# facebook/facebook360_dep

Hardware: AMD Instinct MI355X
Metric: depth Mpix/s per GPU (full pyramid, 16-cam 2048^2 rig); % HBM-read roofline (higher is better)
Workload: dtype f32+f64; 1 GPU; BASELINE config 3: 16-camera 2048x2048 synthetic rig, 8-frame sequence, full 10-level pyramid per frame, per-level temporal filter (+-2 frames); the same sequence for every --gpus N (block partition, 8 frame(s) on this rank); rig=cfg2, cameras=16, frames=8, temporal_filter=True, halo_transport=local, parallelism=frames x1

## Files before the change

### facebook360_dep_amd/csrc/derp_capi.hip

```cpp
#include <hip/hip_runtime.h>

#include <algorithm>
#include <cfloat>
#include <cmath>
#include <cstdarg>
#include <cstdio>
#include <cstdlib>
#include <cstring>
#include <map>
#include <memory>
#include <string>
#include <vector>

#include <rocprim/device/device_radix_sort.hpp>

#include "../../include/derp_hip.h"
#include "derp_host.h"
#include "derp_kernels.h"
#include "derp_mesh.h"
#include "derp_points.h"
#include "derp_render.h"

using namespace derp;

// ... 3 lines not shown

struct Span {
  derp_ctx* c;
  int stage, level;
  hipEvent_t a = nullptr, b = nullptr;
  Span(derp_ctx* ctx, int st, int lv) : c(ctx), stage(st), level(lv) {
    if (c->profiling) {
      (void)hipEventCreate(&a);
      (void)hipEventCreate(&b);
      (void)hipEventRecord(a, c->stream);
    }
  }
  ~Span() {
    if (c->profiling && a) {
      (void)hipEventRecord(b, c->stream);
      c->spans.push_back({stage, level, a, b});
    }
  }
};

void drain_spans(derp_ctx* c) {
  for (auto& s : c->spans) {
    (void)hipEventSynchronize(s.b);
    float ms = 0;
    (void)hipEventElapsedTime(&ms, s.a, s.b);
    if (s.level >= 0 && s.level < kMaxLevels) {
      c->accMs[s.stage][s.level] += ms;
      c->accLaunch[s.stage][s.level] += 1;
    }
    (void)hipEventDestroy(s.a);
    (void)hipEventDestroy(s.b);
  }
  c->spans.clear();
}

size_t npx(const derp_ctx* c, int level) {
  return (size_t)c->LW[level] * c->LH[level];
}

unsigned long long* counter_slot(derp_ctx* c, int stage, int level) {
  return c->counters.as<unsigned long long>() + ((size_t)stage * kMaxLevels + level) * 4;
}

LevelView make_view(derp_ctx* c, int stage, int dst0, int nd) {
  LevelView V;
  const int L = c->cur;
  V.W = c->LW[L];
  V.H = c->LH[L];
  V.Wd = (double)V.W;
  V.Hd = (double)V.H;
  V.S = c->S;
  V.D = nd;
  V.level = L;
  V.numLevels = c->numLevels;
  V.dst0 = dst0;
  V.hasFg = c->opt.use_foreground_masks;
  const float scale = float(V.W) / c->heightFull;
  const float scaleVar = scale * scale;
  V.varNoiseFloor = std::max(c->opt.var_noise_floor * scaleVar, kMinVar);
  V.varHighThresh = c->opt.var_high_thresh;
  V.minDepthM = c->opt.min_depth_m;
  V.maxDepthM = c->opt.max_depth_m;
  V.randomProposals = c->opt.random_proposals;
  V.partialCoverage = c->opt.partial_coverage;
  V.xcdRotate = c->xcdRotate;
  V.camsSrc = c->camsSrc.as<Cam>();
  V.camsDst = c->camsDst.as<Cam>();
  V.dst2src = c->dst2src.as<int>();
  V.srcColor = c->frame().color[L].as<ushort4>();
  V.ownBias = c->w.ownBias.as<ushort4>();
  V.srcVar = c->w.srcVar.as<float>();
  V.srcFg = c->frame().fg[L].as<uint8_t>();
  V.rayDir = c->rayDir.as<double>();
  V.behind = c->behind.as<unsigned>();
  V.rayStride = (size_t)c->D * V.W * V.H;
  V.projWarp = c->projWarp.as<float2>();
  V.projColor = c->w.projColor.as<ushort4>();
  V.projBias = c->w.projBias.as<ushort4>();
  V.projColorT = c->w.projColorT.as<ushort4>();
  V.disparity = c->w.disparity.as<float>();
  V.cost = c->w.cost.as<float>();
  V.confidence = c->w.confidence.as<float>();
  V.bgDisp = c->frame().bg[L].as<float>();
  V.fovMask = c->w.fovMask.as<uint8_t>();
  V.pairCount = c->w.pairCount.as<uint8_t>();
  V.counters = counter_slot(c, stage, L);
#if DERP_BLOCK_TRACE
  V.blockTrace = nullptr;
#endif
  return V;
}
int block_trace_attach(derp_ctx* c, LevelView& V, int which, int gridX, int gridY) {
#if DERP_BLOCK_TRACE
  DevBuf& buf = c->blockTrace[which][V.level];
  const size_t bytes = (size_t)gridX * gridY * 2 * sizeof(unsigned long long);
  ALLOC(c, buf, bytes);
  HIPCHK(c, hipMemsetAsync(buf.as<unsigned long long>(), 0, bytes, c->stream));
  V.blockTrace = buf.as<unsigned long long>();
  c->blockTraceGrid[which][V.level][0] = gridX;
  c->blockTraceGrid[which][V.level][1] = gridY;
#else
  (void)c, (void)V, (void)which, (void)gridX, (void)gridY;
#endif
  return 0;
}

const dim3 kBlurBlk(64, 4, 1);
dim3 blur_grid(int ow, int oh, int planes) {
  return dim3((ow + 63) / 64, (oh + 4 * kBlurRows - 1) / (4 * kBlurRows), planes);
}

void lanczos_coeffs(float x, float* coeffs) {
  static const double s45 = 0.70710678118654752440084436210485;
  static const double cs[][2] = {{1, 0}, {-s45, -s45}, {0, 1}, {s45, -s45}, {-1, 0}, {s45, s45}, {0, -1}, {-s45, s45}};
  if (x < 1.1920928955078125e-07f) {
    for (int i = 0; i < 8; i++) {
      coeffs[i] = 0;
    }
    coeffs[3] = 1;
    return;
  }
  float sum = 0;
  const double y0 = -(x + 3) * M_PI * 0.25, s0 = std::sin(y0), c0 = std::cos(y0);
  for (int i = 0; i < 8; i++) {
    const double y = -(x + 3 - i) * M_PI * 0.25;
    coeffs[i] = (float)((cs[i][0] * s0 + cs[i][1] * c0) / (y * y));
    sum += coeffs[i];
  }
  sum = 1.f / sum;
  for (int i = 0; i < 8; i++) {
    coeffs[i] *= sum;
  }
}

int get_lanczos(derp_ctx* c, int ssize, int dsize, LanczosTab** out) {
  auto key = std::make_pair(ssize, dsize);
  auto it = c->lanczos.find(key);
  if (it != c->lanczos.end()) {
    *out = &it->second;
    return 0;
  }
  std::vector<int> ofs(dsize);
  std::vector<float> coef((size_t)dsize * 8);
  const double scale = (double)ssize / dsize;
  for (int d = 0; d < dsize; ++d) {
    float f = (float)((d + 0.5) * scale - 0.5);
    int s = (int)f;
    s -= (s > f);
    f -= s;
    ofs[d] = s;
    lanczos_coeffs(f, &coef[(size_t)d * 8]);
  }
  LanczosTab t;
  ALLOC(c, t.ofs, ofs.size() * sizeof(int));
  ALLOC(c, t.coef, coef.size() * sizeof(float));
  HIPCHK(c, hipMemcpyAsync(t.ofs.p, ofs.data(), ofs.size() * sizeof(int), hipMemcpyHostToDevice, c->stream));
  HIPCHK(c, hipMemcpyAsync(t.coef.p, coef.data(), coef.size() * sizeof(float), hipMemcpyHostToDevice, c->stream));
  HIPCHK(c, hipStreamSynchronize(c->stream));
  *out = &(c->lanczos[key] = std::move(t));
  return 0;
}

int get_area_tab(derp_ctx* c, int ssize, int dsize, AreaTabDev** out, bool forceTable = false) {
  auto key = std::make_pair(forceTable ? -ssize : ssize, dsize);
  auto it = c->areaTabs.find(key);
  if (it != c->areaTabs.end()) {
    *out = &it->second;
// ... 93 lines not shown
      locs.push_back(make_int2(x, y));
    }
    if (x == y || ((x < 0) && (x == -y)) || ((x > 0) && (x == 1 - y))) {
      t = dx;
      dx = -dy;
      dy = t;
    }
    x += dx;
    y += dy;
  }
  return locs;
}

int ensure_spiral(derp_ctx* c, int radius) {
  if (c->spiralRadius == radius) {
    return 0;
  }
  const std::vector<int2> s = make_spiral(radius * 2 + 1);
  ALLOC(c, c->spiral, s.size() * sizeof(int2));
  HIPCHK(c, hipMemcpy(c->spiral.p, s.data(), s.size() * sizeof(int2), hipMemcpyHostToDevice));
  c->spiralN = (int)s.size();
  c->spiralRadius = radius;
  return 0;
}

int upsample_lanczos_dev(derp_ctx* c, const float* in, int sw, int sh, float* out, int dw, int dh, int planes,
                         size_t inStride, size_t outStride) {
  if (sw == dw && sh == dh) {
    return fail(c, "upsample to identical size not supported");
  }
  LanczosTab *tx, *ty;
  TRY(get_lanczos(c, sw, dw, &tx));
  TRY(get_lanczos(c, sh, dh, &ty));
  const size_t tmpStride = (size_t)dw * sh;
  ALLOC(c, c->w.lanczosTmp, tmpStride * planes * sizeof(float));
  hipLaunchKernelGGL(k_lanczos_h, grid2d(dw, sh, planes, kBlk2d), kBlk2d, 0, c->stream, in, sw, sh, dw,
                     tx->ofs.as<int>(), tx->coef.as<float>(), c->w.lanczosTmp.as<float>(), inStride, tmpStride);
  KCHECK(c);
  hipLaunchKernelGGL(k_lanczos_v, grid2d(dw, dh, planes, kBlk2d), kBlk2d, 0, c->stream, c->w.lanczosTmp.as<float>(), sh,
                     dw, dh, ty->ofs.as<int>(), ty->coef.as<float>(), out, tmpStride, outStride);
  KCHECK(c);
  return 0;
}

int upsample_masked_dev(derp_ctx* c, const float* in, const uint8_t* mask, int sw, int sh, const uint8_t* maskUp,
                        const float* bgUp, float* out, int dw, int dh, int planes = 1) {
  const float scale = float(dw) / float(sw);
  const int radius = (int)(scale * scale + 1);
  TRY(ensure_spiral(c, radius));
  ALLOC(c, c->w.lanczosTmp, (size_t)dw * dh * planes * sizeof(float));
  hipLaunchKernelGGL(k_upsample_nearest_masked, grid2d(dw, dh, planes, kBlk2d), kBlk2d, 0, c->stream, in, mask, sw, sh,
                     maskUp, dw, dh, c->w.lanczosTmp.as<float>());
  KCHECK(c);
  hipLaunchKernelGGL(k_spiral_fill, grid2d(dw, dh, planes, kBlk2d), kBlk2d, 0, c->stream, c->w.lanczosTmp.as<float>(), bgUp,
                     maskUp, dw, dh, c->spiral.as<int2>(), c->spiralN, out);
  KCHECK(c);
  return 0;
}

bool batch_needs_inverse_warps(const derp_ctx* c, int dst0, int nd) {
  std::vector<char> covered(c->S, 0);
  for (int d = dst0; d < dst0 + nd; ++d) {
    covered[c->dst2srcH[d]] = 1;
  }
  for (int s = 0; s < c->S; ++s) {
    if (!covered[s]) {
      return true;
    }
  }
  return false;
}

size_t table_bytes_per_dst(const derp_ctx* c, int W, int H, bool withInverse) {
  const size_t wp = (size_t)(W + 2 * kPadW) * (H + 2 * kPadW), cp = (size_t)(W + 2 * kPadC) * (H + 2 * kPadC);
  return (size_t)(c->S - 1) * (wp * sizeof(float2) + 2 * cp * sizeof(ushort4) + (withInverse ? (size_t)W * H * sizeof(float2) : 0) +
                               (DERP_RANDOM_TILED ? tiled_plane(W, H) * sizeof(ushort4) : 0));
}

int compute_fov_and_masks(derp_ctx* c, int level) {
  const int W = c->LW[level], H = c->LH[level];
  const size_t n = (size_t)W * H;
  {
    Span sp(c, ST_FOV, level);
    hipLaunchKernelGGL(k_fov_mask, grid2d(W, H, c->D, kBlk2d), kBlk2d, 0, c->stream, c->camsDst.as<Cam>(), W, H,
                       c->w.fovMask.as<uint8_t>());
    KCHECK(c);
    hipLaunchKernelGGL(k_and_masks, dim3(flat_grid(n), c->D), dim3(256), 0, c->stream, c->w.fovMask.as<uint8_t>(),
                       c->frame().fg[level].as<uint8_t>(), c->dst2src.as<int>(), 0, n, c->w.maskAnd.as<uint8_t>());
    KCHECK(c);
  }
  return 0;
}

int build_warp(derp_ctx* c, int dst0, int nd) {
  const int L = c->cur;
  Span sp(c, ST_PROJ_WARP, L);
  {
    const size_t n = (size_t)c->LW[L] * c->LH[L];
    ALLOC(c, c->rayDir, 3 * n * c->D * sizeof(double));
    ALLOC(c, c->behind, n * c->D * sizeof(unsigned));
  }
  LevelView V = make_view(c, ST_PROJ_WARP, dst0, nd);
  hipLaunchKernelGGL(k_proj_warp, grid2d(V.W + 2 * kPadW, V.H + 2 * kPadW, c->S, kBlk2d), kBlk2d, 0, c->stream, V,
                     c->projWarp.as<float2>());
  KCHECK(c);
  hipLaunchKernelGGL(k_pixel_rays, grid2d(V.W, V.H, nd, kBlk2d), kBlk2d, 0, c->stream, V, c->rayDir.as<double>(),
                     c->behind.as<unsigned>());
  KCHECK(c);
  c->w.colorTablesCleanLevel = -1;
  if (batch_needs_inverse_warps(c, dst0, nd)) {
    hipLaunchKernelGGL(k_proj_warp_inv, grid2d(V.W, V.H, nd, kBlk2d), kBlk2d, 0, c->stream, V, c->projWarpInv.as<float2>());
    KCHECK(c);
  }
  return 0;
}

int build_color_tables(derp_ctx* c, int dst0, int nd) {
  const int L = c->cur;
  LevelView V = make_view(c, ST_REPROJECT, dst0, nd);
  Span sp(c, ST_REPROJECT, L);
  const dim3 grid((V.W + kRbTile - 1) / kRbTile, (V.H + kRbTile - 1) / kRbTile, nd * (c->S - 1));
  ALLOC(c, c->w.tileSeen, (size_t)grid.x * grid.y * grid.z);
  const int skipBlank = c->w.colorTablesCleanLevel == L && nd == c->D && !c->noBlankSkip;
  hipLaunchKernelGGL(k_reproject_bias, grid, dim3(256), 0, c->stream, V, c->projWarpInv.as<float2>(),
                     c->w.projColor.as<ushort4>(), c->w.projBias.as<ushort4>(), c->w.projColorT.as<ushort4>(),
                     c->w.tileSeen.as<uint8_t>(), skipBlank);
  KCHECK(c);
  c->w.colorTablesCleanLevel = nd == c->D ? L : -1;
  return 0;
}

int tiles_of(int W, int H, int& tilesX) {
  constexpr int B = kTileBlock;
  tilesX = ((W + 15) / 16 + B - 1) / B * B;
  const int tilesY = ((H + 15) / 16 + B - 1) / B * B;
  return tilesX * tilesY * (256 / kCostBlock);
}
constexpr size_t kCostLdsPerSrc = (size_t)kCostBlock * sizeof(SsdPair);
struct CostGrid {
  int blocks, bands, perBlock;
};
constexpr int kCostMaxBands = 4, kCostMaxTilesPerBlock = 4;
int cost_grid_blocks(int tiles, int bands, int perBlock) {
  const int items = (tiles + perBlock - 1) / perBlock, unit = 8 * bands;
  return (items + unit - 1) / unit * unit;
}
CostGrid cost_grid(const derp_ctx* c, int tiles, int tilesX, bool spread) {
  const auto pow2_floor = [](int v, int cap) {
    int p = 1;
    while (p * 2 <= std::min(v, cap)) {
      p *= 2;
    }
    return p;
  };
  CostGrid g;
  g.perBlock = c->costTilesPerBlock > 0 ? pow2_floor(c->costTilesPerBlock, kCostMaxTilesPerBlock) : 1;
  const int rowOfSquares = tilesX * (256 / kCostBlock) * kTileBlock;
  g.bands = c->xcdBands > 0 ? pow2_floor(c->xcdBands, kCostMaxBands)
                            : spread ? pow2_floor(std::max(1, tiles / (8 * rowOfSquares)), kCostMaxBands) : 1;
  g.blocks = cost_grid_blocks(tiles, g.bands, g.perBlock);
  return g;
}
size_t lds_for_waves(size_t needed, int waves, size_t ldsPerCu, size_t fixed) {
  if (waves <= 0 || waves >= 4) {
    return needed;
  }
  const size_t perBlock = ldsPerCu / (size_t)(4 * waves + 1) + 256;
  return std::max(needed, perBlock > fixed ? perBlock - fixed : needed);
}
constexpr size_t kCostLdsStatic = sizeof(PatchWin) * (kCostBlock / 64) + kAtanLutDoubles * sizeof(double);
bool cost_four_waves(const derp_ctx* c) {
  if (const char* e = getenv("DERP_COST_WAVES")) {
    return atoi(e) >= 4;
  }
  return 16 * (kCostLdsPerSrc * (size_t)c->S + kCostLdsStatic) <= c->ldsPerCu && c->S <= 16;
}

int run_brute_force(derp_ctx* c, int dst0, int nd) {
  const int L = c->cur;
  if (L != c->numLevels - 1) {
    return 0;
  }
  Span sp(c, ST_BRUTE, L);
  LevelView V = make_view(c, ST_BRUTE, dst0, nd);
  const size_t n = (size_t)V.W * V.H;
  ALLOC(c, c->w.bruteCost, (size_t)nd * kNumDepths * n * sizeof(float));
  ALLOC(c, c->w.bruteConf, (size_t)nd * kNumDepths * n * sizeof(float));
  const int tilesX = std::max(1, (V.W - 2 + 7) / 8), tilesY = std::max(1, (V.H - 2 + 7) / 8);
  const int tiles = tilesX * tilesY;
  const size_t lds = kCostLdsPerSrc * (size_t)(c->S);
  hipLaunchKernelGGL(k_brute_costs, dim3(tiles, kNumDepths, nd), dim3(kCostBlock), lds, c->stream, V,
                     c->w.bruteCost.as<float>(), c->w.bruteConf.as<float>(), tilesX, tiles);
  KCHECK(c);
  hipLaunchKernelGGL(k_brute_select, grid2d(V.W, V.H, nd, kBlk2d), kBlk2d, 0, c->stream, V, c->w.bruteCost.as<float>(),
                     c->w.bruteConf.as<float>());
  KCHECK(c);
  hipLaunchKernelGGL(k_brute_margin, grid2d(V.W, V.H, nd, kBlk2d), kBlk2d, 0, c->stream, V);
  KCHECK(c);
  return 0;
}

int run_random_proposals(derp_ctx* c, int dst0, int nd) {
  const int L = c->cur;
  if (c->opt.random_proposals <= 0 || L == c->numLevels - 1) {
    return 0;
  }
  Span sp(c, ST_RANDOM, L);
  c->randomRanThisLevel = true;
  LevelView V = make_view(c, ST_RANDOM, dst0, nd);
  if (V.H > 2 && V.W > 2) {
    hipLaunchKernelGGL(k_row_rank, dim3(V.H - 2, nd), dim3(256), 0, c->stream, V, c->w.rank.as<int>());
    KCHECK(c);
  }
  int tilesX;
  const int tiles = tiles_of(V.W, V.H, tilesX);
  const size_t lds = lds_for_waves(kCostLdsPerSrc * (size_t)(c->S), c->randomWaves, c->ldsPerCu, kCostLdsStatic);
  const CostGrid cg = cost_grid(c, tiles, tilesX, true);
  TRY(block_trace_attach(c, V, 0, cg.blocks, nd));
  const bool four = cost_four_waves(c);
  const auto kernel = cg.perBlock > 1 ? (four ? k_random_proposals_walk : k_random_proposals_walk_w3)
                                      : (four ? k_random_proposals : k_random_proposals_w3);
  hipLaunchKernelGGL(kernel, dim3(cg.blocks, nd), dim3(kCostBlock), lds, c->stream, V, c->w.rank.as<int>(), tilesX, cg.bands, cg.perBlock);
  KCHECK(c);
  return 0;
}

int run_ping_pong(derp_ctx* c, int dst0, int nd) {
  const int L = c->cur;
  if (L == c->numLevels - 1) {
    return 0;
  }
  Span sp(c, ST_PINGPONG, L);
  LevelView V = make_view(c, ST_PINGPONG, dst0, nd);
  const size_t n = (size_t)V.W * V.H;
  HIPCHK(c, hipMemsetAsync(c->w.changed.as<uint8_t>() + (size_t)dst0 * n, 1, n * nd, c->stream));
  int tilesX;
  const int tiles = tiles_of(V.W, V.H, tilesX);
  const size_t lds = lds_for_waves(kCostLdsPerSrc * (size_t)(c->S), c->ppWaves, c->ldsPerCu, kCostLdsStatic);
  const bool four = cost_four_waves(c);
  const CostGrid cg = cost_grid(c, tiles, tilesX, false);
  const auto kernel = cg.perBlock > 1
                          ? (c->ppCompact ? (four ? k_ping_pong_walk : k_ping_pong_walk_w3) : (four ? k_ping_pong_loop_walk : k_ping_pong_loop_walk_w3))
                          : (c->ppCompact ? (four ? k_ping_pong : k_ping_pong_w3) : (four ? k_ping_pong_loop : k_ping_pong_loop_w3));
  TRY(block_trace_attach(c, V, 1, cg.blocks, nd));
  for (int it = 1; it <= c->opt.ping_pong_iterations; ++it) {
    hipLaunchKernelGGL(kernel, dim3(cg.blocks, nd), dim3(kCostBlock), lds,
                       c->stream, V, c->w.changed.as<uint8_t>(), c->w.dispRes.as<float>(), c->w.costRes.as<float>(), tilesX,
                       (int)(it == 1 && c->randomRanThisLevel && !c->noMemo), cg.bands, cg.perBlock);
    KCHECK(c);
    hipLaunchKernelGGL(k_ping_pong_commit, dim3(flat_grid(n * nd)), dim3(256), 0, c->stream,
                       c->w.disparity.as<float>() + (size_t)dst0 * n, c->w.cost.as<float>() + (size_t)dst0 * n,
                       c->w.dispRes.as<float>() + (size_t)dst0 * n, c->w.costRes.as<float>() + (size_t)dst0 * n,
                       c->w.changed.as<uint8_t>() + (size_t)dst0 * n, n * nd);
    KCHECK(c);
  }
  if (dst0 + nd >= c->D) {
    c->randomRanThisLevel = false;
  }
  return 0;
}

int run_mismatches(derp_ctx* c) {
  const int L = c->cur;
  if (L > c->opt.mismatches_start_level || L == c->numLevels - 1) {
    return 0;
  }
  if (c->D != c->S) {
    return fail(c, "Check failed: rigDst.size() == rigSrc.size()  Mismatches only valid when considering all cameras");
  }
  for (int d = 0; d < c->D; ++d) {
    if (c->dst2srcH[d] != d) {
      return fail(c, "mismatch handling needs destinations in rig order (dst %d maps to src %d)", d, c->dst2srcH[d]);
    }
  }
  Span sp(c, ST_MISMATCH, L);
  c->randomRanThisLevel = false;
  LevelView V = make_view(c, ST_MISMATCH, 0, c->D);
  const size_t n = (size_t)V.W * V.H;
  hipLaunchKernelGGL(k_mismatch, dim3((V.W + 15) / 16, (V.H + 15) / 16, c->D), dim3(256), 256 * sizeof(float) * c->S,
                     c->stream, V, c->w.dispRes.as<float>(), c->w.mismatchMask.as<uint8_t>());
  KCHECK(c);
  HIPCHK(c, hipMemcpyAsync(c->w.disparity.p, c->w.dispRes.p, n * c->D * sizeof(float), hipMemcpyDeviceToDevice, c->stream));
  return 0;
}

int bilateral_radius(int level) {
  const float scale = std::pow(0.9f, level);
  return (int)std::max(std::ceil(5 * scale), float(1));
}

size_t bilateral_lds_bytes(int radius) {
  const size_t side = 16 + 2 * (size_t)radius;
  const size_t t = ((side + 15) & ~(size_t)15) * side;
  return t * 4 * sizeof(float) + ((t + 3) & ~(size_t)3);
}

constexpr size_t kBilateralMaxLds = 64 * 1024 - 256;

int run_bilateral(derp_ctx* c) {
  const int L = c->cur;
  Span sp(c, ST_BILATERAL, L);
  c->randomRanThisLevel = false;
  const int W = c->LW[L], H = c->LH[L];
  const size_t n = (size_t)W * H;
  const int radius = bilateral_radius(L);
  hipLaunchKernelGGL(k_joint_bilateral<true>, dim3((W + 15) / 16, (H + 15) / 16, c->D), dim3(256),
                     bilateral_lds_bytes(radius), c->stream, c->w.disparity.as<float>(),
                     (const void*)c->frame().color[L].as<ushort4>(), c->w.maskAnd.as<uint8_t>(), W, H, radius, 0.005f, 0.5f,
                     1.0f, 1.0f, c->w.tmpF.as<float>(), n, n, c->dst2src.as<int>());
  KCHECK(c);
  HIPCHK(c, hipMemcpyAsync(c->w.disparity.p, c->w.tmpF.p, n * c->D * sizeof(float), hipMemcpyDeviceToDevice, c->stream));
  return 0;
}

int run_median(derp_ctx* c, bool fuseMaskFov) {
  const int L = c->cur;
  Span sp(c, ST_MEDIAN, L);
  c->randomRanThisLevel = false;
  const int W = c->LW[L], H = c->LH[L];
  const size_t n = (size_t)W * H;
  hipLaunchKernelGGL(k_masked_median, grid2d(W, H, c->D, kBlk2d), kBlk2d, 0, c->stream, c->w.disparity.as<float>(),
                     c->opt.use_foreground_masks ? c->frame().bg[L].as<float>() : (const float*)nullptr,
                     c->w.maskAnd.as<uint8_t>(), W, H, 1, c->w.tmpF.as<float>(), n,
                     fuseMaskFov ? c->w.fovMask.as<uint8_t>() : (const uint8_t*)nullptr);
  KCHECK(c);
  HIPCHK(c, hipMemcpyAsync(c->w.disparity.p, c->w.tmpF.p, n * c->D * sizeof(float), hipMemcpyDeviceToDevice, c->stream));
  return 0;
}

int run_mask_fov(derp_ctx* c) {
  const int L = c->cur;
  Span sp(c, ST_MASKFOV, L);
  const size_t n = npx(c, L) * c->D;
  hipLaunchKernelGGL(k_mask_fov, dim3(flat_grid(n)), dim3(256), 0, c->stream, c->w.disparity.as<float>(),
                     c->w.fovMask.as<uint8_t>(), n);
  KCHECK(c);
  return 0;
}

int check_level(derp_ctx* c, int level) {
  if (!c || c->numLevels == 0) {
    return fail(c, "derp_set_pyramid has not been called");
  }
  if (level < 0 || level >= c->numLevels) {
    return fail(c, "level %d out of range [0, %d)", level, c->numLevels);
  }
  if (c->LW[level] <= 0 || c->LH[level] <= 0) {
    return fail(c, "level %d was declared absent in derp_set_pyramid", level);
  }
  return 0;
}

int level_begin(derp_ctx* c, int level, bool buildAllTables) {
  TRY(check_level(c, level));
  if (c->S - 1 > kMaxSrc) {
    return fail(c, "too many source cameras (%d > %d)", c->S, kMaxSrc + 1);
  }
  c->cur = level;
  const int W = c->LW[level], H = c->LH[level];
  const size_t n = (size_t)W * H;
  if (W < 3 || H < 3) {
    return fail(c, "level %d is too small (%dx%d)", level, W, H);
  }
  TRY(compute_fov_and_masks(c, level));
  {
    Span sp(c, ST_VARIANCE, level);
    hipLaunchKernelGGL(k_variance, grid2d(W, H, c->S, kBlk2d), kBlk2d, 0, c->stream, c->frame().color[level].as<ushort4>(),
                       W, H, c->w.srcVar.as<float>());
    KCHECK(c);
  }
  {
    Span sp(c, ST_OWN_BIAS, level);
    hipLaunchKernelGGL(k_blur3_u16, blur_grid(W, H, c->S), kBlurBlk, 0, c->stream,
                       c->frame().color[level].as<ushort4>(), 0, c->w.ownBias.as<ushort4>(), 0, W, H, n, n);
    KCHECK(c);
  }
  HIPCHK(c, hipMemsetAsync(c->w.cost.p, 0, n * c->D * sizeof(float), c->stream));
  HIPCHK(c, hipMemsetAsync(c->w.confidence.p, 0, n * c->D * sizeof(float), c->stream));
  HIPCHK(c, hipMemsetAsync(c->w.mismatchMask.p, 0, n * c->D, c->stream));
  if (level < c->numLevels - 1 && !c->frame().haveDisp[level + 1] && !buildAllTables) {
    return fail(c, "Missing disparity of level %d needed to start level %d", level + 1, level);
  }
  if (level < c->numLevels - 1 && c->frame().haveDisp[level + 1]) {
    Span sp(c, ST_UPSAMPLE, level);
    const int sw = c->LW[level + 1], sh = c->LH[level + 1];
    if (!c->opt.use_foreground_masks) {
      TRY(upsample_lanczos_dev(c, c->frame().disp[level + 1].as<float>(), sw, sh, c->w.disparity.as<float>(), W, H, c->D,
                               (size_t)sw * sh, n));
    } else {
      ALLOC(c, c->w.staging, (size_t)sw * sh * c->D);
      hipLaunchKernelGGL(k_fov_mask, grid2d(sw, sh, c->D, kBlk2d), kBlk2d, 0, c->stream, c->camsDst.as<Cam>(), sw, sh,
                         c->w.staging.as<uint8_t>());
      KCHECK(c);
      hipLaunchKernelGGL(k_and_masks, dim3(flat_grid((size_t)sw * sh), c->D), dim3(256), 0, c->stream,
                         c->w.staging.as<uint8_t>(), c->frame().fg[level + 1].as<uint8_t>(), c->dst2src.as<int>(), 0,
                         (size_t)sw * sh, c->w.staging.as<uint8_t>());
      KCHECK(c);
      TRY(upsample_masked_dev(c, c->frame().disp[level + 1].as<float>(), c->w.staging.as<uint8_t>(), sw, sh,
                              c->w.maskAnd.as<uint8_t>(), c->frame().bg[level].as<float>(), c->w.disparity.as<float>(), W, H, c->D));
    }
  } else {
    HIPCHK(c, hipMemsetAsync(c->w.disparity.p, 0, n * c->D * sizeof(float), c->stream));
  }
  const bool invAll = batch_needs_inverse_warps(c, 0, c->D);
  size_t per = table_bytes_per_dst(c, W, H, invAll);
  int DB = c->D;
  bool needInv = invAll;
  {
    const size_t wpAll = (size_t)(W + 2 * kPadW) * (H + 2 * kPadW) * (c->S - 1) * c->D * sizeof(float2);
    const size_t cpAll = (size_t)(W + 2 * kPadC) * (H + 2 * kPadC) * (c->S - 1) * c->D * sizeof(ushort4);
    const size_t ipAll = (size_t)W * H * (c->S - 1) * c->D * sizeof(float2);
    const bool resident = c->projWarp.bytes >= wpAll && c->w.projColor.bytes >= cpAll && c->w.projBias.bytes >= cpAll &&
        (!invAll || c->projWarpInv.bytes >= ipAll) && !getenv("DERP_TABLE_BUDGET_GB") &&
        (!DERP_RANDOM_TILED || c->w.projColorT.bytes >= tiled_plane(W, H) * (c->S - 1) * c->D * sizeof(ushort4));
    if (!resident) {
      size_t freeB = 0, totalB = 0;
      HIPCHK(c, hipMemGetInfo(&freeB, &totalB));
      size_t budget = freeB + c->projWarp.bytes + c->w.projColor.bytes + c->w.projBias.bytes + c->projWarpInv.bytes + c->w.projColorT.bytes;
      if (const char* e = getenv("DERP_TABLE_BUDGET_GB")) {
        budget = std::min<size_t>(budget, (size_t)(atof(e) * (1ull << 30)));
      } else {
        budget = (size_t)(budget * 0.85);
      }
      DB = (int)std::min<size_t>((size_t)c->D, budget / std::max<size_t>(per, 1));
      if (DB < c->D && !needInv) {
        needInv = true;
        per = table_bytes_per_dst(c, W, H, true);
        DB = (int)std::min<size_t>((size_t)c->D, budget / std::max<size_t>(per, 1));
      }
      if (DB < 1) {
        return fail(c, "projection tables for one destination (%zu bytes) exceed the table budget (%zu bytes)", per, budget);
      }
      const int batches = (c->D + DB - 1) / DB;
      DB = (c->D + batches - 1) / batches;
    }
  }
  c->DB = DB;
  const size_t wp = (size_t)(W + 2 * kPadW) * (H + 2 * kPadW), cp = (size_t)(W + 2 * kPadC) * (H + 2 * kPadC);
  ALLOC(c, c->projWarp, (size_t)DB * (c->S - 1) * wp * sizeof(float2));
  ALLOC(c, c->w.projColor, (size_t)DB * (c->S - 1) * cp * sizeof(ushort4));
  ALLOC(c, c->w.projBias, (size_t)DB * (c->S - 1) * cp * sizeof(ushort4));
  if (needInv) {
    ALLOC(c, c->projWarpInv, (size_t)DB * (c->S - 1) * n * sizeof(float2));
  }
  if (DERP_RANDOM_TILED) {
    ALLOC(c, c->w.projColorT, (size_t)DB * (c->S - 1) * tiled_plane(W, H) * sizeof(ushort4));
  }
  c->tablesValid = false;
  c->randomRanThisLevel = false;
  if (buildAllTables) {
    if (DB < c->D) {
      return fail(c, "stage-level API needs all destinations' tables resident (batch %d < %d)", DB, c->D);
    }
    if (c->opt.rebuild_warp_tables || c->warpCachedLevel != level) {
      TRY(build_warp(c, 0, c->D));
      c->warpCachedLevel = level;
    }
  }
  return 0;
}

int level_end(derp_ctx* c) {
  const int L = c->cur;
  HIPCHK(c, hipMemcpyAsync(c->frame().disp[L].p, c->w.disparity.p, npx(c, L) * c->D * sizeof(float),
                           hipMemcpyDeviceToDevice, c->stream));
  c->frame().haveDisp[L] = 1;
  return 0;
}

int process_level(derp_ctx* c, int level) {
  TRY(level_begin(c, level, false));
  for (int d0 = 0; d0 < c->D; d0 += c->DB) {
    const int nd = std::min(c->DB, c->D - d0);
    const bool single = (c->DB == c->D);
    if (!single || c->opt.rebuild_warp_tables || c->warpCachedLevel != level) {
      TRY(build_warp(c, d0, nd));
      c->warpCachedLevel = single ? level : -1;
    }
    TRY(build_color_tables(c, d0, nd));
    TRY(run_brute_force(c, d0, nd));
    TRY(run_random_proposals(c, d0, nd));
    TRY(run_ping_pong(c, d0, nd));
  }
  TRY(run_mismatches(c));
  if (c->opt.do_bilateral_filter) {
    TRY(run_bilateral(c));
  }
  if (c->opt.do_median_filter) {
    TRY(run_median(c, true));
  } else {
    TRY(run_mask_fov(c));
  }
  TRY(level_end(c));
  return 0;
}

int need_current(derp_ctx* c, bool tables) {
  if (!c || c->cur < 0) {
    return fail(c, "derp_level_begin has not been called");
  }
  if (tables && !c->tablesValid) {
    return fail(c, "derp_stage_reproject_colors must run before this stage");
  }
  return 0;
}

template <typename T>
int upload_tmp(derp_ctx* c, DevBuf& buf, const T* host, size_t count) {
  ALLOC(c, buf, count * sizeof(T));
  HIPCHK(c, hipMemcpyAsync(buf.p, host, count * sizeof(T), hipMemcpyHostToDevice, c->stream));
  return 0;
}

int alloc_pyramid(derp_ctx* c, FramePyramid& f) {
  const int num_levels = c->numLevels;
  f.color.resize(num_levels);
  f.fg.resize(num_levels);
  f.bg.resize(num_levels);
  f.disp.resize(num_levels);
  f.haveBg.assign(num_levels, 0);
  f.haveDisp.assign(num_levels, 0);
  for (int l = 0; l < num_levels; ++l) {
    const size_t n = npx(c, l);
    if (n == 0) {
      continue;
    }
    ALLOC(c, f.color[l], n * c->S * sizeof(ushort4));
    ALLOC(c, f.fg[l], n * c->S);
    ALLOC(c, f.bg[l], n * c->D * sizeof(float));
    ALLOC(c, f.disp[l], n * c->D * sizeof(float));
    HIPCHK(c, hipMemsetAsync(f.fg[l].p, 1, n * c->S, c->stream));
    HIPCHK(c, hipMemsetAsync(f.bg[l].p, 0, n * c->D * sizeof(float), c->stream));
  }
  return 0;
}

int alloc_work_set(derp_ctx* c, WorkSet& w, size_t n) {
  ALLOC(c, w.srcVar, n * c->S * sizeof(float));
  ALLOC(c, w.ownBias, n * c->S * sizeof(ushort4));
  ALLOC(c, w.fovMask, n * c->D);
  ALLOC(c, w.maskAnd, n * c->D);
  for (DevBuf* b : {&w.disparity, &w.cost, &w.confidence, &w.dispRes, &w.costRes, &w.tmpF, &w.rank}) {
    ALLOC(c, *b, n * c->D * sizeof(float));
  }
  ALLOC(c, w.changed, n * c->D);
  ALLOC(c, w.mismatchMask, n * c->D);
  ALLOC(c, w.pairCount, n * c->D);
  return 0;
}

int select_frame(derp_ctx* c, int slot) {
  if (slot < 0 || slot >= (int)c->frames.size()) {
    return fail(c, "frame slot %d out of range [0, %d)", slot, (int)c->frames.size());
  }
  if (slot != c->curSlot) {
    c->curSlot = slot;
    c->cur = -1;
  }
  return 0;
}

void lane_swap(derp_ctx* c, int i) {
  std::swap(c->stream, c->lanes[i]->stream);
  std::swap(c->w, c->lanes[i]->w);
}

int lanes_prepare(derp_ctx* c, int count, size_t n) {
  while ((int)c->lanes.size() < count) {
    c->lanes.emplace_back(new WorkLane);
    WorkLane& l = *c->lanes.back();
    if (hipStreamCreateWithFlags(&l.stream, hipStreamNonBlocking) != hipSuccess ||
        hipEventCreateWithFlags(&l.done, hipEventDisableTiming) != hipSuccess) {
      return fail(c, "work lane: hipStreamCreate / hipEventCreate failed");
    }
  }
  if (!c->laneReady) {
    HIPCHK(c, hipEventCreateWithFlags(&c->laneReady, hipEventDisableTiming));
  }
  for (int i = 0; i < count; ++i) {
    TRY(alloc_work_set(c, c->lanes[i]->w, n));
  }
  return 0;
}

int process_level_on_lane(derp_ctx* c, int i, int slot, int level) {
  if (i < 0) {
    TRY(select_frame(c, slot));
    return process_level(c, level);
  }
  HIPCHK(c, hipStreamWaitEvent(c->lanes[i]->stream, c->laneReady, 0));
  lane_swap(c, i);
  c->activeLane = i;
  int rc = select_frame(c, slot);
  if (!rc) {
    rc = process_level(c, level);
  }
  if (!rc && hipEventRecord(c->lanes[i]->done, c->stream) != hipSuccess) {
    rc = fail(c, "work lane: hipEventRecord failed");
  }
  lane_swap(c, i);
  c->activeLane = -1;
  c->cur = -1;
  return rc;
}

int temporal_launch(derp_ctx* c, const void* const* guides, const float* const* images, const uint8_t* const* masks, int n,
                    int centre, int W, int H, int planes, float sigma, int radius, float w0, float w1, float w2,
                    float* out, const int* dst2src) {
  if (n < 1 || centre < 0 || centre >= n) {
    return fail(c, "temporal window must hold at least the centre frame");
  }
  if (n > kMaxTemporalFrames) {
    ALLOC(c, c->temporalCarry, (size_t)planes * W * H * sizeof(float2));
  }
  for (int t0 = 0; t0 < n; t0 += kMaxTemporalFrames) {
    TemporalFrames F;
    F.n = std::min(kMaxTemporalFrames, n - t0);
    for (int t = 0; t < F.n; ++t) {
      F.guides[t] = reinterpret_cast<const ushort4*>(guides[t0 + t]);
      F.images[t] = images[t0 + t];
      F.masks[t] = masks[t0 + t];
    }
    F.refGuide = reinterpret_cast<const ushort4*>(guides[centre]);
    F.refImage = images[centre];
    F.refMask = masks[centre];
    F.carry = n > kMaxTemporalFrames ? c->temporalCarry.as<float2>() : nullptr;
    F.first = t0 == 0;
    F.last = t0 + F.n >= n;
    const size_t lds = 2 * ((((size_t)(32 + 2 * radius) * (8 + 2 * radius) * 9) + 15) & ~(size_t)15);
    if (radius >= 0 && lds <= 48 * 1024 && !c->noTemporalTile) {
      hipLaunchKernelGGL(k_temporal_tiled, grid2d(W, H, planes, kBlk2d), kBlk2d, lds, c->stream, F, W, H, sigma, radius, w0,
                         w1, w2, out, dst2src);
    } else {
      hipLaunchKernelGGL(k_temporal, grid2d(W, H, planes, kBlk2d), kBlk2d, 0, c->stream, F, W, H, sigma, radius, w0, w1, w2,
                         out, dst2src);
    }
    KCHECK(c);
  }
  return 0;
}

}

extern "C" {

void derp_options_default(derp_options* o) {
  o->min_depth_m = 0.5f;
  o->max_depth_m = 1e4f;
  o->var_noise_floor = 4e-5f;
  o->var_high_thresh = 1e-3f;
  o->random_proposals = 2;
  o->ping_pong_iterations = 1;
  o->mismatches_start_level = -1;
  o->do_bilateral_filter = 1;
  o->do_median_filter = 1;
  o->use_foreground_masks = 0;
  o->partial_coverage = 0;
  o->rebuild_warp_tables = 1;
}

int derp_create(derp_ctx** out, int device, const derp_camera_desc* src, int n_src, const derp_camera_desc* dst,
                int n_dst) {
  if (!out) {
    return 1;
  }
  *out = nullptr;
  std::unique_ptr<derp_ctx> owner(new derp_ctx);
  derp_ctx* c = owner.get();
  derp_options_default(&c->opt);
  if (n_src <= 0 || n_dst <= 0) {
    return create_fail("no source / destination cameras!");
  }
  hipDeviceProp_t prop;
  TRY(open_device(device, "the depth path", &prop));
  c->device = device;
  if (prop.maxSharedMemoryPerMultiProcessor > 0) {
    c->ldsPerCu = prop.maxSharedMemoryPerMultiProcessor;
  }
  if (const char* e = getenv("DERP_XCD_ROTATE")) {
    c->xcdRotate = atoi(e);
  }
  if (const char* e = getenv("DERP_XCD_BANDS")) {
    c->xcdBands = atoi(e);
  }
  if (const char* e = getenv("DERP_COST_TILES_PER_BLOCK")) {
    c->costTilesPerBlock = atoi(e);
  }
  c->noMemo = getenv("DERP_NO_MEMO") != nullptr;
  if (const char* e = getenv("DERP_PP_COMPACT")) {
    c->ppCompact = atoi(e) != 0;
  }
  if (const char* e = getenv("DERP_RANDOM_WAVES")) {
    c->randomWaves = atoi(e);
  }
  if (const char* e = getenv("DERP_PP_WAVES")) {
    c->ppWaves = atoi(e);
  }
  c->noTemporalTile = getenv("DERP_NO_TEMPORAL_TILE") != nullptr;
  c->noBlankSkip = getenv("DERP_NO_BLANK_SKIP") != nullptr;
  c->S = n_src;
  c->D = n_dst;
  c->frames.resize(1);
  c->camsSrcH.resize(n_src);
  c->camsDstH.resize(n_dst);
  for (int i = 0; i < n_src; ++i) {
    if (const char* m = host_prepare_camera(src[i], c->camsSrcH[i])) {
      return create_fail(std::string("camera ") + src[i].id + ": " + m);
    }
  }
  c->dst2srcH.assign(n_dst, 0);
  c->descDstH.assign(dst, dst + n_dst);
  for (int i = 0; i < n_dst; ++i) {
    if (const char* m = host_prepare_camera(dst[i], c->camsDstH[i])) {
      return create_fail(std::string("camera ") + dst[i].id + ": " + m);
    }
    bool found = false;
    for (int s = 0; s < n_src; ++s) {
      if (strncmp(dst[i].id, src[s].id, sizeof dst[i].id) == 0) {
        c->dst2srcH[i] = s;
        found = true;
        break;
      }
    }
    if (!found) {
      return create_fail(std::string("destination camera ") + dst[i].id + " is not a source camera");
    }
    if (memcmp(&c->camsDstH[i], &c->camsSrcH[c->dst2srcH[i]], sizeof(Cam)) != 0) {
      return create_fail(std::string("destination camera ") + dst[i].id + " differs from the source camera of the same id "
                  "(destinations must be cameras of the source rig, as filterDestinations makes them)");
    }
  }
  if (c->camsSrc.ensure(sizeof(Cam) * n_src) || c->camsDst.ensure(sizeof(Cam) * n_dst) ||
      c->dst2src.ensure(sizeof(int) * n_dst) || c->counters.ensure(sizeof(unsigned long long) * ST_COUNT * kMaxLevels * 4)) {
    return create_fail("out of device memory");
  }
  if (hipStreamCreateWithFlags(&c->stream, hipStreamNonBlocking) != hipSuccess) {
    return create_fail("hipStreamCreate failed");
  }
  if (hipStreamCreateWithFlags(&c->copyStream, hipStreamNonBlocking) != hipSuccess) {
    (void)hipStreamDestroy(c->stream);
    return create_fail("hipStreamCreate failed");
  }
  (void)hipMemcpy(c->camsSrc.p, c->camsSrcH.data(), sizeof(Cam) * n_src, hipMemcpyHostToDevice);
  (void)hipMemcpy(c->camsDst.p, c->camsDstH.data(), sizeof(Cam) * n_dst, hipMemcpyHostToDevice);
  (void)hipMemcpy(c->dst2src.p, c->dst2srcH.data(), sizeof(int) * n_dst, hipMemcpyHostToDevice);
  (void)hipMemset(c->counters.p, 0, c->counters.bytes);
  *out = owner.release();
  return 0;
}

void derp_destroy(derp_ctx* c) {
  if (!c) {
    return;
  }
  (void)hipSetDevice(c->device);
  (void)hipStreamSynchronize(c->stream);
  for (auto& l : c->lanes) {
    (void)hipStreamSynchronize(l->stream);
  }
  drain_spans(c);
  for (auto& l : c->lanes) {
    (void)hipStreamDestroy(l->stream);
    (void)hipEventDestroy(l->done);
  }
  if (c->laneReady) {
    (void)hipEventDestroy(c->laneReady);
  }
  (void)hipStreamDestroy(c->stream);
  (void)hipStreamDestroy(c->copyStream);
  delete c;
}

const char* derp_last_error(const derp_ctx* c) {
  return c ? c->err.c_str() : g_create_error.c_str();
}

int derp_set_options(derp_ctx* c, const derp_options* o) {
  if (!c || !o) {
    return 1;
  }
  if (o->random_proposals < 0) {
    return fail(c, "Check failed: random_proposals >= 0");
  }
  c->opt = *o;
  return 0;
}

int derp_set_pyramid(derp_ctx* c, int num_levels, const int* widths, const int* heights, int width_full,
                     int height_full) {
  if (!c) {
    return 1;
  }
  if (num_levels <= 0 || num_levels > kMaxLevels) {
    return fail(c, "num_levels %d out of range (1..%d)", num_levels, kMaxLevels);
  }
  HIPCHK(c, hipSetDevice(c->device));
  c->numLevels = num_levels;
  c->widthFull = width_full;
  c->heightFull = height_full;
  c->LW.assign(widths, widths + num_levels);
  c->LH.assign(heights, heights + num_levels);
  c->frames.clear();
  c->frames.resize(1);
  c->curSlot = 0;
  TRY(alloc_pyramid(c, c->frame()));
  size_t nmax = 0;
  for (int l = 0; l < num_levels; ++l) {
    nmax = std::max(nmax, npx(c, l));
  }
  TRY(alloc_work_set(c, c->w, nmax));
  c->cur = -1;
  c->warpCachedLevel = -1;
  HIPCHK(c, hipStreamSynchronize(c->stream));
  return 0;
}

int derp_set_frame_slots(derp_ctx* c, int n_slots) {
  if (!c || c->numLevels == 0) {
    return fail(c, "derp_set_pyramid has not been called");
  }
  if (n_slots < 1 || n_slots > 4096) {
    return fail(c, "n_slots %d out of range (1..4096)", n_slots);
  }
  HIPCHK(c, hipSetDevice(c->device));
  TRY(select_frame(c, 0));
  const int had = (int)c->frames.size();
  c->frames.resize(n_slots);
  for (int k = had; k < n_slots; ++k) {
    TRY(alloc_pyramid(c, c->frames[k]));
  }
  HIPCHK(c, hipStreamSynchronize(c->stream));
  return 0;
}

int derp_select_frame(derp_ctx* c, int slot) {
  if (!c || c->numLevels == 0) {
    return fail(c, "derp_set_pyramid has not been called");
  }
  return select_frame(c, slot);
}

int derp_frame_slots(const derp_ctx* c, int* n_slots, int* selected) {
  if (!c) {
    return 1;
  }
  if (n_slots) {
    *n_slots = (int)c->frames.size();
  }
  if (selected) {
    *selected = c->curSlot;
  }
  return 0;
}

int derp_bind_thread(derp_ctx* c) {
  return use_device(c);
}
void* derp_host_alloc(size_t bytes) {
  void* p = nullptr;
  if (bytes == 0 || hipHostMalloc(&p, bytes, hipHostMallocDefault) != hipSuccess) {
    (void)hipGetLastError();
    return nullptr;
  }
  return p;
}
void derp_host_free(void* p) {
  if (p) {
    (void)hipHostFree(p);
  }
}
int derp_host_register(void* p, size_t bytes) {
  if (!p || bytes == 0 || hipHostRegister(p, bytes, hipHostRegisterDefault) != hipSuccess) {
    (void)hipGetLastError();
    return 1;
  }
  return 0;
}
void derp_host_unregister(void* p) {
  if (p && hipHostUnregister(p) != hipSuccess) {
    (void)hipGetLastError();
  }
}

int derp_upload_color(derp_ctx* c, int level, int s, const uint16_t* bgr) {
  TRY(check_level(c, level));
  if (s < 0 || s >= c->S || !bgr) {
    return fail(c, "bad source index / null image");
  }
  HIPCHK(c, hipSetDevice(c->device));
  const size_t n = npx(c, level);
  TRY(upload_tmp(c, c->w.staging, bgr, n * 3));
  hipLaunchKernelGGL(k_bgr_to_bgrx, dim3(flat_grid(n)), dim3(256), 0, c->stream, c->w.staging.as<uint16_t>(),
                     c->frame().color[level].as<ushort4>() + (size_t)s * n, n);
  KCHECK(c);
  HIPCHK(c, hipStreamSynchronize(c->stream));
// ... 170 lines not shown
  int tilesX;
  const int tiles = tiles_of(V.W, V.H, tilesX);
  const size_t lds = kCostLdsPerSrc * (size_t)(c->S);
  hipLaunchKernelGGL(k_cost_map, dim3(tiles), dim3(kCostBlock), lds, c->stream, V, d, c->w.staging.as<float>(),
                     c->w.stagingB.as<float>(), c->w.stagingB.as<float>() + n, tilesX);
  KCHECK(c);
  HIPCHK(c, hipStreamSynchronize(c->stream));
  HIPCHK(c, hipMemcpy(cost, c->w.stagingB.p, n * sizeof(float), hipMemcpyDeviceToHost));
  HIPCHK(c, hipMemcpy(confidence, c->w.stagingB.as<float>() + n, n * sizeof(float), hipMemcpyDeviceToHost));
  return 0;
}

static int build_pyramid(derp_ctx* c, int kind, int index, int count, const void* host, size_t elem, int w, int h,
                         int threshold) {
  if (!c || c->numLevels == 0) {
    return fail(c, "derp_set_pyramid has not been called");
  }
  if (index < 0 || index >= count || !host || w <= 0 || h <= 0) {
    return fail(c, "bad camera index / null image");
  }
  HIPCHK(c, hipSetDevice(c->device));
  const size_t n = (size_t)w * h;
  ALLOC(c, c->fullFrame, n * elem);
  HIPCHK(c, hipMemcpyAsync(c->fullFrame.p, host, n * elem, hipMemcpyHostToDevice, c->stream));
  for (int l = 0; l < c->numLevels; ++l) {
    const size_t nl = npx(c, l);
    if (nl == 0) {
      continue;
    }
    void* dst = kind == 0 ? (void*)(c->frame().color[l].as<ushort4>() + (size_t)index * nl)
        : kind == 1       ? (void*)(c->frame().fg[l].as<uint8_t>() + (size_t)index * nl)
                          : (void*)(c->frame().bg[l].as<float>() + (size_t)index * nl);
    TRY(resize_area_dev(c, kind, c->fullFrame.p, w, h, dst, c->LW[l], c->LH[l], threshold));
    if (kind == 2) {
      c->frame().haveBg[l] = 1;
    }
  }
  HIPCHK(c, hipStreamSynchronize(c->stream));
  return 0;
}
int derp_build_pyramid_color(derp_ctx* c, int src, const uint16_t* bgr, int w, int h) {
  return build_pyramid(c, 0, src, c ? c->S : 0, bgr, 6, w, h, -1);
}
int derp_build_pyramid_foreground_mask(derp_ctx* c, int src, const uint8_t* mask, int w, int h, int threshold) {
  return build_pyramid(c, 1, src, c ? c->S : 0, mask, 1, w, h, threshold);
}
int derp_build_pyramid_background_disparity(derp_ctx* c, int dst, const float* disp, int w, int h) {
  return build_pyramid(c, 2, dst, c ? c->D : 0, disp, 4, w, h, -1);
}
int derp_download_level_color(derp_ctx* c, int level, int src, uint16_t* bgr) {
  TRY(check_level(c, level));
  if (src < 0 || src >= c->S || !bgr) {
    return fail(c, "bad source index / null output");
  }
  const size_t n = npx(c, level);
  ALLOC(c, c->w.staging, n * 6);
  hipLaunchKernelGGL(k_bgrx_to_bgr, dim3(flat_grid(n)), dim3(256), 0, c->stream,
                     c->frame().color[level].as<ushort4>() + (size_t)src * n, c->w.staging.as<uint16_t>(), n);
  KCHECK(c);
  return download_sync(c, bgr, c->w.staging.p, n * 6);
}
int derp_download_level_mask(derp_ctx* c, int level, int src, uint8_t* mask) {
  TRY(check_level(c, level));
  if (src < 0 || src >= c->S || !mask) {
    return fail(c, "bad source index / null output");
  }
  const size_t n = npx(c, level);
  return download_sync(c, mask, c->frame().fg[level].as<uint8_t>() + (size_t)src * n, n);
}
int derp_download_level_background(derp_ctx* c, int level, int dst, float* disp) {
  TRY(check_level(c, level));
  if (dst < 0 || dst >= c->D || !disp) {
    return fail(c, "bad destination index / null output");
  }
  const size_t n = npx(c, level);
  return download_sync(c, disp, c->frame().bg[level].as<float>() + (size_t)dst * n, n * 4);
}
int derp_download_mismatch_mask(derp_ctx* c, int d, uint8_t* out) {
  TRY(need_current(c, false));
  if (d < 0 || d >= c->D || !out) {
    return fail(c, "bad destination index / null output");
  }
  const size_t n = npx(c, c->cur);
  return download_sync(c, out, c->w.mismatchMask.as<uint8_t>() + (size_t)d * n, n);
}

}

#include "derp_render_api.h"
#include "derp_rephoto_api.h"
#include "derp_points_api.h"
#include "derp_mesh_api.h"
#include "derp_filters_api.h"
#include "derp_debug_api.h"
#include "derp_sequence.h"
#include "derp_isp.h"
#include "derp_sim.h"

derp_ctx::derp_ctx() = default;
derp_ctx::~derp_ctx() = default;
```

### facebook360_dep_amd/csrc/derp_ctx.h

```cpp
#pragma once

namespace {

enum Stage {
  ST_FOV = 0,
  ST_VARIANCE,
  ST_OWN_BIAS,
  ST_UPSAMPLE,
  ST_PROJ_WARP,
  ST_REPROJECT,
  ST_PROJ_BIAS,
  ST_BRUTE,
  ST_RANDOM,
  ST_PINGPONG,
  ST_MISMATCH,
  ST_BILATERAL,
  ST_MEDIAN,
  ST_MASKFOV,
  ST_TEMPORAL,
  ST_LANES,
  ST_COUNT
};
const char* kStageNames[ST_COUNT] = {"fov_mask",  "variance",    "own_bias",         "upsample",  "proj_warp",
                                     "reproject", "proj_bias",   "brute_force",      "random_proposals",
                                     "ping_pong", "mismatches",  "bilateral",        "median",    "mask_fov",
                                     "temporal",  "lanes_wall"};
constexpr int kMaxLevels = 24;

struct TimedSpan {
  int stage, level;
  hipEvent_t a, b;
};

struct LanczosTab {
  DevBuf ofs, coef;
};

struct AreaTabDev {
  DevBuf start, si, alpha;
  int iscale = 0;
};

struct WorkSet {
  DevBuf srcVar, ownBias, fovMask, maskAnd, disparity, cost, confidence, dispRes, costRes, changed, tmpF, rank, mismatchMask, pairCount;
  DevBuf tileSeen;
  DevBuf projColor, projBias;
  DevBuf projColorT;
  DevBuf bruteCost, bruteConf, lanczosTmp, staging, stagingB;
  int colorTablesCleanLevel = -1;
};

struct FramePyramid {
  std::vector<DevBuf> color, fg, bg, disp;
  std::vector<char> haveBg, haveDisp;
};

struct WorkLane {
  hipStream_t stream = nullptr;
  hipEvent_t done = nullptr;
  WorkSet w;
};

struct SmrState; struct RephotoState; struct PointsState; struct MeshState;

}

struct derp_ctx {
  derp_ctx();
  ~derp_ctx();
  int device = 0;
  hipStream_t stream = nullptr;
  hipStream_t copyStream = nullptr;
  DevBuf copyStaging;
  std::string err;
  std::string* errSink() {
    return &err;
  }
  derp_options opt;
  int S = 0, D = 0;
  std::vector<Cam> camsSrcH, camsDstH;
  std::vector<int> dst2srcH;
  std::vector<derp_camera_desc> descDstH;
  DevBuf camsSrc, camsDst, dst2src;

  int numLevels = 0, widthFull = 0, heightFull = 0;
  std::vector<int> LW, LH;
  std::vector<FramePyramid> frames;
  int curSlot = 0;
  FramePyramid& frame() {
    return frames[curSlot];
  }
  DevBuf fullFrame;
  DevBuf devMask;

  int cur = -1;
  int DB = 0;
  WorkSet w;
  DevBuf temporalCarry;
  DevBuf projWarp, projWarpInv;
  DevBuf rayDir, behind;
  int warpCachedLevel = -1;
  bool randomRanThisLevel = false;
  bool tablesValid = false;
  std::map<std::pair<int, int>, LanczosTab> lanczos;
  std::map<std::pair<int, int>, AreaTabDev> areaTabs;
  DevBuf spiral;
  int spiralN = 0, spiralRadius = -1;
  std::vector<std::unique_ptr<WorkLane>> lanes;
  hipEvent_t laneReady = nullptr;
  int activeLane = -1;

  DevBuf counters;
  bool profiling = false;
  std::vector<TimedSpan> spans;
  double accMs[ST_COUNT][kMaxLevels] = {};
  int accLaunch[ST_COUNT][kMaxLevels] = {};
  int xcdRotate = 1;
  int xcdBands = 0, costTilesPerBlock = 0;
  DevBuf blockTrace[2][kMaxLevels];
  int blockTraceGrid[2][kMaxLevels][2] = {};
  bool noMemo = false;
  bool ppCompact = true;
  int randomWaves = 0, ppWaves = 0;
  size_t ldsPerCu = 160 * 1024;
  bool noTemporalTile = false;
  bool noBlankSkip = false;
  std::unique_ptr<SmrState> smr;
  std::unique_ptr<RephotoState> rephoto;
  std::unique_ptr<PointsState> points;
  std::unique_ptr<MeshState> mesh;
};

namespace {

int fail(derp_ctx* c, const char* fmt, ...) {
  va_list ap;
  va_start(ap, fmt);
  vfail(c ? &c->err : nullptr, fmt, ap);
  va_end(ap);
  return 1;
}

int use_device(derp_ctx* c) {
  if (!c) {
    return 1;
  }
  HIPCHK(c, hipSetDevice(c->device));
  return 0;
}

int check_camera(derp_ctx* c, int cam) {
  if (cam < 0 || cam >= c->D) {
    return fail(c, "bad camera index %d (the context has %d)", cam, c->D);
  }
  return 0;
}

}
```

### facebook360_dep_amd/csrc/derp_debug_api.h

```cpp
#pragma once

namespace {
struct HostPairs {
  SsdPair* p;
  SsdPair get(int i) const {
    return p[i];
  }
  void set(int i, const SsdPair& v) {
    p[i] = v;
  }
};
int stage_index(const char* stage) {
  for (int i = 0; i < ST_COUNT; ++i) {
    if (strcmp(stage, kStageNames[i]) == 0) {
      return i;
    }
  }
  return -1;
}
}

int derp_debug_atan2_ypos(derp_ctx* c, const double* y, const double* x, double* out, size_t n) {
  if (!c || !y || !x || !out) {
    return fail(c, "bad arguments");
  }
  ALLOC(c, c->w.staging, 3 * n * sizeof(double));
  double* d = c->w.staging.as<double>();
  HIPCHK(c, hipMemcpyAsync(d, y, n * sizeof(double), hipMemcpyHostToDevice, c->stream));
  HIPCHK(c, hipMemcpyAsync(d + n, x, n * sizeof(double), hipMemcpyHostToDevice, c->stream));
  hipLaunchKernelGGL(k_debug_atan2_ypos, dim3(flat_grid(n)), dim3(256), 0, c->stream, d, d + n, d + 2 * n, n);
  KCHECK(c);
  HIPCHK(c, hipMemcpyAsync(out, d + 2 * n, n * sizeof(double), hipMemcpyDeviceToHost, c->stream));
  HIPCHK(c, hipStreamSynchronize(c->stream));
  return 0;
}

int derp_debug_fp64(derp_ctx* c, int op, const double* a, const double* b, double* out, size_t n) {
  if (!c || !a || !out || op < 0 || op > 3 || (op >= 2 && !b)) {
    return fail(c, "bad arguments");
  }
  if (n == 0) {
    return 0;
  }
  ALLOC(c, c->w.staging, 3 * n * sizeof(double));
  double* d = c->w.staging.as<double>();
  HIPCHK(c, hipMemcpyAsync(d, a, n * sizeof(double), hipMemcpyHostToDevice, c->stream));
  HIPCHK(c, hipMemcpyAsync(d + n, op >= 2 ? b : a, n * sizeof(double), hipMemcpyHostToDevice, c->stream));
  hipLaunchKernelGGL(k_debug_fp64, dim3(flat_grid(n)), dim3(256), 0, c->stream, op, d, d + n, d + 2 * n, n);
  KCHECK(c);
  HIPCHK(c, hipMemcpyAsync(out, d + 2 * n, n * sizeof(double), hipMemcpyDeviceToHost, c->stream));
  HIPCHK(c, hipStreamSynchronize(c->stream));
  return 0;
}

int derp_debug_sees(derp_ctx* c, int src, const double* xyz, size_t n, double* out) {
  if (!c || !xyz || !out || src < 0 || src >= c->S) {
    return fail(c, "bad arguments");
  }
  if (n == 0) {
    return 0;
  }
  ALLOC(c, c->w.staging, 9 * n * sizeof(double));
  double* d = c->w.staging.as<double>();
  HIPCHK(c, hipMemcpyAsync(d, xyz, 3 * n * sizeof(double), hipMemcpyHostToDevice, c->stream));
  hipLaunchKernelGGL(k_debug_sees, dim3(flat_grid(n)), dim3(256), 0, c->stream, c->camsSrc.as<Cam>(), src, d, d + 3 * n, n);
  KCHECK(c);
  HIPCHK(c, hipMemcpyAsync(out, d + 3 * n, 6 * n * sizeof(double), hipMemcpyDeviceToHost, c->stream));
  HIPCHK(c, hipStreamSynchronize(c->stream));
  return 0;
}

int derp_debug_download(derp_ctx* c, int d, int s, int which, void* out) {
  TRY(need_current(c, false));
  const int L = c->cur;
  const int W = c->LW[L], H = c->LH[L];
  const size_t n = (size_t)W * H;
  HIPCHK(c, hipStreamSynchronize(c->stream));
  if (which == 4) {
    HIPCHK(c, hipMemcpy(out, c->w.srcVar.as<float>() + (size_t)s * n, n * sizeof(float), hipMemcpyDeviceToHost));
    return 0;
  }
  if (which == 5) {
    HIPCHK(c, hipMemcpy(out, c->w.fovMask.as<uint8_t>() + (size_t)d * n, n, hipMemcpyDeviceToHost));
    return 0;
  }
  if (d < 0 || d >= c->D || s < 0 || s >= c->S || s == c->dst2srcH[d]) {
    return fail(c, "bad (dst, src) pair");
  }
  const size_t tab = (size_t)d * (c->S - 1) + (s < c->dst2srcH[d] ? s : s - 1);
  if (which == 0) {
    const int PW = W + 2 * kPadW, PH = H + 2 * kPadW;
    std::vector<float2> tmp((size_t)PW * PH);
    HIPCHK(c, hipMemcpy(tmp.data(), c->projWarp.as<float2>() + tab * tmp.size(), tmp.size() * sizeof(float2),
                        hipMemcpyDeviceToHost));
    float2* o = reinterpret_cast<float2*>(out);
    for (int y = 0; y < H; ++y) {
      memcpy(o + (size_t)y * W, &tmp[(size_t)(y + kPadW) * PW + kPadW], (size_t)W * sizeof(float2));
    }
    return 0;
  }
  if (which == 2 || which == 3) {
    const int PW = W + 2 * kPadC, PH = H + 2 * kPadC;
    std::vector<ushort4> tmp((size_t)PW * PH);
    const ushort4* base = (which == 2 ? c->w.projColor.as<ushort4>() : c->w.projBias.as<ushort4>()) + tab * tmp.size();
    HIPCHK(c, hipMemcpy(tmp.data(), base, tmp.size() * sizeof(ushort4), hipMemcpyDeviceToHost));
    uint16_t* o = reinterpret_cast<uint16_t*>(out);
    for (int y = 0; y < H; ++y) {
      for (int x = 0; x < W; ++x) {
        const ushort4 q = tmp[(size_t)(y + kPadC) * PW + x + kPadC];
        o[((size_t)y * W + x) * 3 + 0] = q.x;
        o[((size_t)y * W + x) * 3 + 1] = q.y;
        o[((size_t)y * W + x) * 3 + 2] = q.z;
      }
    }
    return 0;
  }
  return fail(c, "unknown table id %d", which);
}

int derp_dev_disparity(derp_ctx* c, int level, int d, float** ptr, size_t* bytes) {
  TRY(check_level(c, level));
  if (d < 0 || d >= c->D || !ptr || !bytes) {
    return fail(c, "bad destination index / null output");
  }
  const size_t n = npx(c, level);
  *ptr = c->frame().disp[level].as<float>() + (size_t)d * n;
  *bytes = n * sizeof(float);
  return 0;
}
int derp_dev_color(derp_ctx* c, int level, int s, void** ptr, size_t* bytes) {
  TRY(check_level(c, level));
  if (s < 0 || s >= c->S || !ptr || !bytes) {
    return fail(c, "bad source index / null output");
  }
  const size_t n = npx(c, level);
  *ptr = c->frame().color[level].as<ushort4>() + (size_t)s * n;
  *bytes = n * sizeof(ushort4);
  return 0;
}
int derp_dev_mask(derp_ctx* c, int level, int d, uint8_t** ptr, size_t* bytes) {
  TRY(check_level(c, level));
  if (d < 0 || d >= c->D || !ptr || !bytes) {
    return fail(c, "bad destination index / null output");
  }
  HIPCHK(c, hipSetDevice(c->device));
  const int W = c->LW[level], H = c->LH[level];
  const size_t n = (size_t)W * H;
  ALLOC(c, c->devMask, n * c->D);
  hipLaunchKernelGGL(k_fov_mask, grid2d(W, H, c->D, kBlk2d), kBlk2d, 0, c->stream, c->camsDst.as<Cam>(), W, H,
                     c->devMask.as<uint8_t>());
  KCHECK(c);
  hipLaunchKernelGGL(k_and_masks, dim3(flat_grid(n), c->D), dim3(256), 0, c->stream, c->devMask.as<uint8_t>(),
                     c->frame().fg[level].as<uint8_t>(), c->dst2src.as<int>(), 0, n, c->devMask.as<uint8_t>());
  KCHECK(c);
  HIPCHK(c, hipStreamSynchronize(c->stream));
  *ptr = c->devMask.as<uint8_t>() + (size_t)d * n;
  *bytes = n;
  return 0;
}

int derp_get_counters(derp_ctx* c, uint64_t* n_cost, uint64_t* n_pair, uint64_t* insufficient) {
  if (!c) {
    return 1;
  }
  HIPCHK(c, hipStreamSynchronize(c->stream));
  std::vector<unsigned long long> h((size_t)ST_COUNT * kMaxLevels * 4);
// ... 174 lines not shown
```

### facebook360_dep_amd/csrc/derp_filters_api.h

```cpp
#pragma once

int derp_resize_area(derp_ctx* c, int kind, const void* src, int w, int h, void* dst, int dw, int dh) {
  if (!c || !src || !dst || kind < 0 || kind > 3 || w <= 0 || h <= 0 || dw <= 0 || dh <= 0) {
    return fail(c, "bad arguments");
  }
  HIPCHK(c, hipSetDevice(c->device));
  const size_t elem = kind == 0 ? 6 : kind == 1 ? 1 : kind == 3 ? 12 : 4, n = (size_t)w * h, nd = (size_t)dw * dh;
  DevBuf in, out, out3;
  TRY(upload_sync(c, in, src, n * elem));
  ALLOC(c, out, nd * (kind == 0 ? 8 : elem));
  TRY(resize_area_dev(c, kind, in.p, w, h, out.p, dw, dh, -1));
  if (kind == 0) {
    ALLOC(c, out3, nd * 6);
    hipLaunchKernelGGL(k_bgrx_to_bgr, dim3(flat_grid(nd)), dim3(256), 0, c->stream, out.as<ushort4>(),
                       out3.as<uint16_t>(), nd);
  }
  return download_sync(c, dst, kind == 0 ? out3.p : out.p, nd * elem);
}

int derp_generate_foreground_mask(derp_ctx* c, const uint16_t* template_bgr, const uint16_t* frame_bgr, int w, int h,
                                  int blur_radius, float threshold, int morph_closing_size, uint8_t* mask01) {
  if (!c || !template_bgr || !frame_bgr || !mask01 || w <= 0 || h <= 0 || blur_radius < 0 || blur_radius > 3 ||
      morph_closing_size < 0 || !(threshold >= 0)) {
    return fail(c, "bad arguments (blur_radius must be 0..3)");
// ... 16 lines not shown
    hipLaunchKernelGGL(k_gauss_u16, grid2d(w, h, 1, kBlk2d), kBlk2d, 0, c->stream, t4.as<ushort4>(), tb.as<ushort4>(), w, h, blur_radius);
    hipLaunchKernelGGL(k_gauss_u16, grid2d(w, h, 1, kBlk2d), kBlk2d, 0, c->stream, f4.as<ushort4>(), fb.as<ushort4>(), w, h, blur_radius);
    tp = tb.as<ushort4>();
    fp = fb.as<ushort4>();
  }
  hipLaunchKernelGGL(k_fg_threshold, dim3(flat_grid(n)), dim3(256), 0, c->stream, tp, fp, n, threshold, m0.as<uint8_t>());
  if (morph_closing_size > 0) {
    ALLOC(c, m1, n);
    hipLaunchKernelGGL(k_morph_rect, grid2d(w, h, 1, kBlk2d), kBlk2d, 0, c->stream, m0.as<uint8_t>(), m1.as<uint8_t>(), w, h, morph_closing_size, 1);
    hipLaunchKernelGGL(k_morph_rect, grid2d(w, h, 1, kBlk2d), kBlk2d, 0, c->stream, m1.as<uint8_t>(), m0.as<uint8_t>(), w, h, morph_closing_size, 0);
  }
  return download_sync(c, mask01, m0.p, n);
}

int derp_layer_disparities(derp_ctx* c, const float* foreground, const float* background, size_t n, uint8_t* out) {
  if (!c || !foreground || !background || !out) {
    return fail(c, "bad arguments");
  }
  HIPCHK(c, hipSetDevice(c->device));
  DevBuf f, b, o;
  TRY(upload_sync(c, f, foreground, n * 4));
  TRY(upload_sync(c, b, background, n * 4));
  ALLOC(c, o, n);
  hipLaunchKernelGGL(k_layer_disparities, dim3(flat_grid(n)), dim3(256), 0, c->stream, f.as<float>(), b.as<float>(), n,
                     o.as<uint8_t>());
  return download_sync(c, out, o.p, n);
}
int derp_fov_mask(derp_ctx* c, int d, int w, int h, uint8_t* out) {
  if (!c || !out || d < 0 || d >= c->D || w <= 0 || h <= 0) {
    return fail(c, "bad arguments");
  }
  HIPCHK(c, hipSetDevice(c->device));
  DevBuf m;
  ALLOC(c, m, (size_t)w * h);
  hipLaunchKernelGGL(k_fov_mask, grid2d(w, h, 1, kBlk2d), kBlk2d, 0, c->stream, c->camsDst.as<Cam>() + d, w, h,
                     m.as<uint8_t>());
  return download_sync(c, out, m.p, (size_t)w * h);
}

int derp_upsample_disparity(derp_ctx* c, int d, const float* disp, int w, int h, const float* bg_disp_up,
                            const uint8_t* fg_mask, const uint8_t* fg_mask_up, int w_up, int h_up, int use_fg,
                            float* out) {
  if (!c || !disp || !out || d < 0 || d >= c->D) {
    return fail(c, "bad arguments");
  }
  HIPCHK(c, hipSetDevice(c->device));
  const size_t n = (size_t)w * h, nu = (size_t)w_up * h_up;
  DevBuf in, res, m, mu, bg, fov, fovu, idx;
  TRY(upload_sync(c, in, disp, n * 4));
  ALLOC(c, res, nu * 4);
  if (!use_fg) {
    TRY(upsample_lanczos_dev(c, in.as<float>(), w, h, res.as<float>(), w_up, h_up, 1, n, nu));
    return download_sync(c, out, res.p, nu * 4);
  }
  if (!bg_disp_up || !fg_mask || !fg_mask_up) {
    return fail(c, "foreground-mask upsample needs bg_disp_up, fg_mask and fg_mask_up");
  }
  const int zero = 0;
  TRY(upload_sync(c, m, fg_mask, n));
  TRY(upload_sync(c, mu, fg_mask_up, nu));
  TRY(upload_sync(c, bg, bg_disp_up, nu * 4));
  TRY(upload_sync(c, idx, &zero, sizeof(int)));
  ALLOC(c, fov, n);
  ALLOC(c, fovu, nu);
  hipLaunchKernelGGL(k_fov_mask, grid2d(w, h, 1, kBlk2d), kBlk2d, 0, c->stream, c->camsDst.as<Cam>() + d, w, h,
                     fov.as<uint8_t>());
  hipLaunchKernelGGL(k_fov_mask, grid2d(w_up, h_up, 1, kBlk2d), kBlk2d, 0, c->stream, c->camsDst.as<Cam>() + d, w_up,
                     h_up, fovu.as<uint8_t>());
  hipLaunchKernelGGL(k_and_masks, dim3(flat_grid(n), 1), dim3(256), 0, c->stream, fov.as<uint8_t>(), m.as<uint8_t>(),
                     idx.as<int>(), 0, n, fov.as<uint8_t>());
  hipLaunchKernelGGL(k_and_masks, dim3(flat_grid(nu), 1), dim3(256), 0, c->stream, fovu.as<uint8_t>(), mu.as<uint8_t>(),
                     idx.as<int>(), 0, nu, fovu.as<uint8_t>());
  TRY(upsample_masked_dev(c, in.as<float>(), fov.as<uint8_t>(), w, h, fovu.as<uint8_t>(), bg.as<float>(), res.as<float>(),
                          w_up, h_up));
  return download_sync(c, out, res.p, nu * 4);
}

template <bool GUIDE_U16>
static void launch_joint_bilateral(derp_ctx* c, const float* image, const void* guide, const uint8_t* mask, int w, int h,
                                   int radius, float sigma, float w0, float w1, float w2, float* out) {
  const size_t n = (size_t)w * h;
  const dim3 grid((w + 15) / 16, (h + 15) / 16, 1);
  if (bilateral_lds_bytes(radius) <= kBilateralMaxLds) {
    hipLaunchKernelGGL(k_joint_bilateral<GUIDE_U16>, grid, dim3(256), bilateral_lds_bytes(radius), c->stream, image, guide,
                       mask, w, h, radius, sigma, w0, w1, w2, out, n, n, (const int*)nullptr);
  } else {
    hipLaunchKernelGGL(k_joint_bilateral_direct<GUIDE_U16>, grid, dim3(256), 0, c->stream, image, guide, mask, w, h,
                       radius, sigma, w0, w1, w2, out);
  }
}

int derp_joint_bilateral_u16(derp_ctx* c, const float* image, const uint16_t* guide, const uint8_t* mask, int w, int h,
                             int radius, float sigma, float w0, float w1, float w2, float* out) {
  if (!c || !image || !guide || !mask || !out || w <= 0 || h <= 0 || radius < 0 || radius > (1 << 30)) {
    return fail(c, "bad arguments (radius must be in [0, 2^30])");
  }
  HIPCHK(c, hipSetDevice(c->device));
  const size_t n = (size_t)w * h;
  DevBuf im, g3, g4, m, res;
  TRY(upload_sync(c, im, image, n * 4));
  TRY(upload_sync(c, g3, guide, n * 6));
  TRY(upload_sync(c, m, mask, n));
  ALLOC(c, g4, n * 8);
  ALLOC(c, res, n * 4);
  hipLaunchKernelGGL(k_bgr_to_bgrx, dim3(flat_grid(n)), dim3(256), 0, c->stream, g3.as<uint16_t>(), g4.as<ushort4>(), n);
  launch_joint_bilateral<true>(c, im.as<float>(), (const void*)g4.as<ushort4>(), m.as<uint8_t>(), w, h, radius, sigma, w0,
                               w1, w2, res.as<float>());
  return download_sync(c, out, res.p, n * 4);
}

int derp_joint_bilateral_f32(derp_ctx* c, const float* image, const float* guide, const uint8_t* mask, int w, int h,
                             int radius, float sigma, float w0, float w1, float w2, float* out) {
  if (!c || !image || !guide || !mask || !out || w <= 0 || h <= 0 || radius < 0 || radius > (1 << 30)) {
    return fail(c, "bad arguments (radius must be in [0, 2^30])");
  }
  HIPCHK(c, hipSetDevice(c->device));
  const size_t n = (size_t)w * h;
  DevBuf im, g, m, res;
  TRY(upload_sync(c, im, image, n * 4));
  TRY(upload_sync(c, g, guide, n * 12));
  TRY(upload_sync(c, m, mask, n));
  ALLOC(c, res, n * 4);
  launch_joint_bilateral<false>(c, im.as<float>(), (const void*)g.as<float>(), m.as<uint8_t>(), w, h, radius, sigma, w0, w1,
                                w2, res.as<float>());
  return download_sync(c, out, res.p, n * 4);
}

int derp_masked_median(derp_ctx* c, const float* image, const float* background, const uint8_t* mask, int w, int h,
                       int radius, float* out) {
  if (!c || !image || !mask || !out || radius < 1 || radius > 2) {
    return fail(c, "bad arguments (radius must be 1 or 2)");
  }
  HIPCHK(c, hipSetDevice(c->device));
  const size_t n = (size_t)w * h;
  DevBuf im, bg, m, res;
  TRY(upload_sync(c, im, image, n * 4));
  if (background) {
    TRY(upload_sync(c, bg, background, n * 4));
  }
  TRY(upload_sync(c, m, mask, n));
  ALLOC(c, res, n * 4);
  hipLaunchKernelGGL(k_masked_median, grid2d(w, h, 1, kBlk2d), kBlk2d, 0, c->stream, im.as<float>(),
                     background ? bg.as<float>() : (const float*)nullptr, m.as<uint8_t>(), w, h, radius,
                     res.as<float>(), n, (const uint8_t*)nullptr);
  return download_sync(c, out, res.p, n * 4);
}

int derp_temporal_filter_dev(derp_ctx* c, const void* const* guides, const float* const* disps,
                             const uint8_t* const* masks, int n_frames, int w, int h, int frame_offset, float sigma,
                             int space_radius, float w0, float w1, float w2, float* out_dev) {
  if (!c || n_frames < 1 || frame_offset < 0 || frame_offset >= n_frames) {
    return fail(c, "temporal window must hold at least one frame and contain the centre frame");
  }
  HIPCHK(c, hipSetDevice(c->device));
  return temporal_launch(c, guides, disps, masks, n_frames, frame_offset, w, h, 1, sigma, space_radius, w0, w1, w2, out_dev,
                         nullptr);
}

int derp_temporal_filter(derp_ctx* c, const uint16_t* const* guides, const float* const* disps,
                         const uint8_t* const* masks, int n_frames, int w, int h, int frame_offset, float sigma,
                         int space_radius, float w0, float w1, float w2, float* out) {
  if (!c || n_frames < 1) {
    return fail(c, "temporal window must hold at least one frame");
  }
  HIPCHK(c, hipSetDevice(c->device));
  const size_t n = (size_t)w * h;
  std::vector<DevBuf> g4(n_frames), im(n_frames), m(n_frames);
  DevBuf g3, res;
// ... 21 lines not shown
```

### facebook360_dep_amd/csrc/derp_kernels.h

```cpp
#pragma once
#include <hip/hip_runtime.h>
#include <math.h>
#include <stdint.h>

#include <type_traits>

#include "derp_camera.h"
#include "gcc_algos.h"

namespace derp {

#ifndef DERP_COST_MIN_WAVES
#define DERP_COST_MIN_WAVES 4
#endif
#ifndef DERP_RANDOM_MIN_WAVES
#define DERP_RANDOM_MIN_WAVES 4
#endif
#ifndef DERP_RANDOM_TILED
#define DERP_RANDOM_TILED 0
#endif
#ifndef DERP_MIX_HOT_ONLY
#define DERP_MIX_HOT_ONLY 0
#endif
#ifndef DERP_PHASE_TIMERS
// ... 1138 lines not shown
  if (skipBlank && !*seen) {
    return;
  }
  const int dl = tab / (V.S - 1), sl = tab - dl * (V.S - 1);
  const int own = V.dst2src[V.dst0 + dl];
  const int s = sl < own ? sl : sl + 1;
  const int x0 = blockIdx.x * kRbTile, y0 = blockIdx.y * kRbTile;
  const int OW = V.W + 2 * kPadC, OH = V.H + 2 * kPadC;
  const size_t plane = (size_t)OW * OH, n = (size_t)V.W * V.H;
  const ushort4* img = V.srcColor + (size_t)s * n;
  const float2* map = warpInv + (size_t)tab * n;
  int mapPitch = V.W;
  const int ds = batch_dst_of_source(V, s);
  if (ds >= 0) {
    mapPitch = V.W + 2 * kPadW;
    map = V.projWarp + ((size_t)ds * (V.S - 1) + slot(own, s)) * warp_plane(V) + (size_t)kPadW * mapPitch + kPadW;
  }
  int any = 0;
  for (int k = threadIdx.x; k < kRbCells; k += 256) {
    const int ty = k / kRbPitch, tx = k - ty * kRbPitch;
    const int qx = x0 - 1 + tx, qy = y0 - 1 + ty;
    if (qx >= -1 && qx <= V.W && qy >= -1 && qy <= V.H) {
      const float2 m = map[(size_t)reflect101(qy, V.H) * mapPitch + reflect101(qx, V.W)];
      const bool valid = !(m.x != m.x);
      any |= valid;
      tile[k] = valid ? remap_cubic_u16(img, V.W, V.H, m.x, m.y) : make_ushort4(0, 0, 0, 0);
    }
  }
  any = __syncthreads_or(any);
  if (!skipBlank && threadIdx.x == 0) {
    *seen = (uint8_t)(any != 0);
  }
  ushort4* pc = projColor + (size_t)tab * plane;
  ushort4* pb = projBias + (size_t)tab * plane;
  const int tilesX = tiled_tiles_x(V.W);
  ushort4* pt = projColorT ? projColorT + (size_t)tab * tiled_plane(V.W, V.H) : nullptr;
  const int lx = threadIdx.x & 31;
  const int x = x0 + lx;
  if (x >= V.W) {
    return;
  }
  const int oxa = x == 0 ? 0 : x + kPadC, oxb = x == V.W - 1 ? OW - 1 : x + kPadC;
#pragma unroll
  for (int j = 0; j < kRbTile / 8; ++j) {
    const int ly = (int)(threadIdx.x >> 5) + 8 * j;
    const int y = y0 + ly;
    if (y >= V.H) {
      break;
    }
    const ushort4* t = &tile[(ly + 1) * kRbPitch + lx + 1];
    unsigned s0 = 0, s1 = 0, s2 = 0;
#pragma unroll
    for (int v = -1; v <= 1; ++v) {
#pragma unroll
      for (int u = -1; u <= 1; ++u) {
        const ushort4 q = t[v * kRbPitch + u];
        s0 += q.x;
        s1 += q.y;
        s2 += q.z;
      }
    }
    const ushort4 col = t[0];
    const ushort4 bia = make_ushort4((unsigned short)((s0 + 4) / 9), (unsigned short)((s1 + 4) / 9),
                                     (unsigned short)((s2 + 4) / 9), 0);
    const int oya = y == 0 ? 0 : y + kPadC, oyb = y == V.H - 1 ? OH - 1 : y + kPadC;
    for (int oy = oya; oy <= oyb; ++oy) {
      for (int ox = oxa; ox <= oxb; ++ox) {
        pc[(size_t)oy * OW + ox] = col;
        pb[(size_t)oy * OW + ox] = bia;
        if (pt) {
          pt[tiled_index(tilesX, ox, oy)] = col;
        }
      }
    }
  }
}

__device__ __forceinline__ float probe_disparity(int i, float minD, float maxD) {
  const double fraction = (double)i / (double)(kNumDepths - 1);
  return (float)(fraction * (double)minD + (1 - fraction) * (double)maxD);
}

__global__ void __launch_bounds__(kCostBlock, DERP_COST_MIN_WAVES)
    k_brute_costs(LevelView V, float* __restrict__ costs, float* __restrict__ confs, int tilesX, int tilesPerDst) {
  const int i = blockIdx.y;
  const int dl = blockIdx.z;
  const int d = V.dst0 + dl;
  const int iw = V.W - 2, ih = V.H - 2;
  const int lane = threadIdx.x & 63;
  const int sx = (int)(blockIdx.x % (unsigned)tilesX), sy = (int)(blockIdx.x / (unsigned)tilesX);
  const int x = 1 + sx * 8 + (lane & 7), y = 1 + sy * 8 + (lane >> 3);
  PatchWin* win;
  LdsPairs pairs = cost_wave_prologue(V, d, x - (int)(threadIdx.x & 7), y - (int)((threadIdx.x & 63) >> 3), win);
  unsigned nCost = 0, nPair = 0;
  if (x <= iw && y <= ih) {
    const int own = V.dst2src[d];
    const size_t n = (size_t)V.W * V.H, idx = (size_t)y * V.W + x;
    const float minDisparity = 1.0f / V.maxDepthM, maxDisparity = 1.0f / V.minDepthM;
    const float disparity = probe_disparity(i, minDisparity, maxDisparity);
    const bool fov = V.fovMask[(size_t)d * n + idx], fg = V.srcFg[(size_t)own * n + idx];
    const bool closer = V.hasFg ? (V.bgDisp[(size_t)d * n + idx] < disparity) : true;
    float2 r = make_float2(__builtin_nanf(""), __builtin_nanf(""));
    if (fov && fg && closer) {
      PixCtx px;
      load_pixctx(V, d, own, x, y, win, px);
      r = compute_cost(V, dl, own, px, disparity, pairs, nPair);
      ++nCost;
    }
    const size_t o = ((size_t)dl * kNumDepths + i) * n + idx;
    costs[o] = r.x;
    confs[o] = r.y;
  }
  flush_counters(V, nCost, nPair);
}

__global__ void k_brute_select(LevelView V, const float* __restrict__ costs, const float* __restrict__ confs) {
  const int dl = blockIdx.z;
  const int d = V.dst0 + dl;
  const int x = blockIdx.x * blockDim.x + threadIdx.x, y = blockIdx.y * blockDim.y + threadIdx.y;
  if (x < 1 || y < 1 || x >= V.W - 1 || y >= V.H - 1) {
    return;
  }
  const int own = V.dst2src[d];
  const size_t n = (size_t)V.W * V.H, idx = (size_t)y * V.W + x;
  float* disp = V.disparity + (size_t)d * n;
  if (!V.fovMask[(size_t)d * n + idx]) {
    disp[idx] = __builtin_nanf("");
    return;
  }
  if (!V.srcFg[(size_t)own * n + idx]) {
    disp[idx] = V.bgDisp[(size_t)d * n + idx];
    return;
  }
  float minCost = 3.402823466e+38f, minConf = 0;
  int best = -1;
  for (int i = 0; i < kNumDepths; ++i) {
    const size_t o = ((size_t)dl * kNumDepths + i) * n + idx;
    const float c = costs[o];
    if (c < minCost) {
      minCost = c;
      minConf = confs[o];
      best = i;
    }
  }
  const float minDisparity = 1.0f / V.maxDepthM, maxDisparity = 1.0f / V.minDepthM;
  if (best == -1) {
    atomicAdd(&V.counters[2], 1ull);
    disp[idx] = minDisparity;
  } else {
    disp[idx] = probe_disparity(best, minDisparity, maxDisparity);
  }
  V.cost[(size_t)d * n + idx] = minCost;
  V.confidence[(size_t)d * n + idx] = minConf;
}

__global__ void k_brute_margin(LevelView V) {
  const int d = V.dst0 + blockIdx.z;
  const int x = blockIdx.x * blockDim.x + threadIdx.x, y = blockIdx.y * blockDim.y + threadIdx.y;
  if (x >= V.W || y >= V.H) {
    return;
  }
  if (!(x < 1 || x >= V.W - 1 || y < 1 || y >= V.H - 1)) {
    return;
  }
  const int own = V.dst2src[d];
  const size_t n = (size_t)V.W * V.H, idx = (size_t)y * V.W + x;
  if (!V.srcFg[(size_t)own * n + idx]) {
    V.disparity[(size_t)d * n + idx] = V.bgDisp[(size_t)d * n + idx];
    return;
  }
  const int yy = min(max(y, 1), V.H - 2), xx = min(max(x, 1), V.W - 2);
  const size_t src = (size_t)yy * V.W + xx;
  V.disparity[(size_t)d * n + idx] = V.disparity[(size_t)d * n + src];
  V.cost[(size_t)d * n + idx] = V.cost[(size_t)d * n + src];
  V.confidence[(size_t)d * n + idx] = V.confidence[(size_t)d * n + src];
}

__device__ __forceinline__ bool random_gate(const LevelView& V, int d, int own, size_t idx) {
  const size_t n = (size_t)V.W * V.H;
  if (!V.fovMask[(size_t)d * n + idx] || !V.srcFg[(size_t)own * n + idx]) {
    return false;
  }
  const float varHighDev = 0.1f * V.varHighThresh;
  const float thresh = fmaxf(varHighDev, V.varNoiseFloor);
  return !(V.srcVar[(size_t)own * n + idx] < thresh);
}

__global__ void __launch_bounds__(256) k_row_rank(LevelView V, int* __restrict__ rank) {
  __shared__ int partial[256];
  const int d = V.dst0 + blockIdx.y, y = blockIdx.x + 1;
  const int own = V.dst2src[d];
  const size_t n = (size_t)V.W * V.H;
  const int inner = V.W - 2;
  const int per = (inner + 255) / 256;
// ... 94 lines not shown
  atomicAdd(&V.counters[3], (unsigned long long)nSlots);
  atomicAdd(&V.counters[2], (unsigned long long)nSlotsFirst);
#endif
}

template <bool WALK>
__device__ __forceinline__ void random_proposals_body(const LevelView& V, const int* __restrict__ rank, int tilesX, int bands,
                                                      int perBlock) {
  const unsigned long long bt0 = block_trace_begin();
  const int steps = WALK ? perBlock : 1;
  const int dl = blockIdx.y;
  const int d = V.dst0 + dl;
  PatchWin* win;
  LdsPairs pairs = cost_block_prologue(win);
  bool lutReady = false;
  for (int step = 0; step < steps; ++step) {
    int x, y;
    tile_pixel(cost_block_tile(blockIdx.x, gridDim.x, V.xcdRotate ? d : 0, bands, steps, step), tilesX, x, y);
    bool go = false;
    if (x >= 1 && y >= 1 && x < V.W - 1 && y < V.H - 1) {
      const int own = V.dst2src[d];
      const size_t n = (size_t)V.W * V.H;
      const unsigned idx = (unsigned)y * (unsigned)V.W + (unsigned)x;
      if ((V.fovMask + (size_t)d * n)[idx]) {
        if (!(V.srcFg + (size_t)own * n)[idx]) {
          (V.disparity + (size_t)d * n)[idx] = (V.bgDisp + (size_t)d * n)[idx];
        } else {
          go = random_gate(V, d, own, idx);
        }
      }
    }
    if (__ballot(go) == 0ull) {
      continue;
    }
    cost_tile_prologue(V, d, x - (int)(threadIdx.x & 7), y - (int)((threadIdx.x & 63) >> 3), win, pairs, lutReady);
    random_proposals_tile(V, rank, dl, x, y, go, win, pairs);
  }
  block_trace_end(V, bt0);
}

__global__ void __launch_bounds__(kCostBlock, DERP_RANDOM_MIN_WAVES)
    k_random_proposals(LevelView V, const int* __restrict__ rank, int tilesX, int bands, int perBlock) {
  random_proposals_body<false>(V, rank, tilesX, bands, perBlock);
}
__global__ void __launch_bounds__(kCostBlock, 3)
    k_random_proposals_w3(LevelView V, const int* __restrict__ rank, int tilesX, int bands, int perBlock) {
  random_proposals_body<false>(V, rank, tilesX, bands, perBlock);
}
__global__ void __launch_bounds__(kCostBlock, DERP_RANDOM_MIN_WAVES)
    k_random_proposals_walk(LevelView V, const int* __restrict__ rank, int tilesX, int bands, int perBlock) {
  random_proposals_body<true>(V, rank, tilesX, bands, perBlock);
}
__global__ void __launch_bounds__(kCostBlock, 3)
    k_random_proposals_walk_w3(LevelView V, const int* __restrict__ rank, int tilesX, int bands, int perBlock) {
  random_proposals_body<true>(V, rank, tilesX, bands, perBlock);
}

__constant__ int kCandidates[9][2] = {{0, 0}, {-1, 0}, {1, 0}, {0, -1}, {0, 1}, {-2, -2}, {2, -2}, {-2, 2}, {2, 2}};
constexpr int kCandOff[9][2] = {{0, 0}, {-1, 0}, {1, 0}, {0, -1}, {0, 1}, {-2, -2}, {2, -2}, {-2, 2}, {2, 2}};
constexpr unsigned cand_pack(int c) {
  unsigned p = 0;
  for (int k = 0; k < 9; ++k) {
    p |= (unsigned)(kCandOff[k][c] + 2) << (3 * k);
  }
  return p;
}
constexpr unsigned kCandPackX = cand_pack(0), kCandPackY = cand_pack(1);

#ifdef DERP_COUNT_PP_FILL
__device__ __forceinline__ unsigned pp_fill_entry() {
  return __builtin_ctzll(__ballot(1)) == (int)(threadIdx.x & 63) ? 64u : 0u;
}
#endif

__device__ __forceinline__ void ping_pong_candidates_loop(const LevelView& V, const uint8_t* __restrict__ changed, int dl, int x,
                                                          int y, const PatchWin* win, LdsPairs& pairs, int useMemo, float& outDisp,
                                                          float& outCost, unsigned& counts, unsigned& fillSlots, PhaseTimers& tm) {
  const int d = V.dst0 + dl;
  const int own = V.dst2src[d];
  const size_t n = (size_t)V.W * V.H;
  const unsigned idx = (unsigned)y * (unsigned)V.W + (unsigned)x;
  const float* disp = V.disparity + (size_t)d * n;
  const uint8_t* fov = V.fovMask + (size_t)d * n;
  const uint8_t* chg = changed + (size_t)d * n;
  outDisp = disp[idx];
  const bool interior = x >= 1 && y >= 1 && x < V.W - 1 && y < V.H - 1;
  if (interior && fov[idx]) {
    if (!V.srcFg[(size_t)own * n + idx]) {
      outDisp = V.bgDisp[(size_t)d * n + idx];
    } else if (!(V.srcVar[(size_t)own * n + idx] < V.varNoiseFloor)) {
      PixCtx px;
      load_pixctx<false>(V, d, own, x, y, win, px);
      const unsigned cull = behind_sources(V, d, idx);
      float bestCost = __builtin_inff();
      float bestDisp = outDisp;
      const unsigned xy = (unsigned)x | ((unsigned)y << 16);
      for (int k = 0; k < 9; ++k) {
        unsigned q = xy;
        asm("" : "+v"(q) : "s"(k));
        const int px0 = (int)(q & 0xffffu), py0 = (int)(q >> 16);
        const unsigned pidx = (unsigned)py0 * (unsigned)V.W + (unsigned)px0;
        const int xx = min(max(px0 + kCandidates[k][0], 0), V.W - 1);
        const int yy = min(max(py0 + kCandidates[k][1], 0), V.H - 1);
        const unsigned j = (unsigned)yy * (unsigned)V.W + (unsigned)xx;
        if (fov[j]) {
          const float cand = disp[j];
          const float bg = V.hasFg ? (V.bgDisp + (size_t)d * n)[pidx] : 0.f;
          if (cand >= bg && chg[j]) {
            float2 r;
            const float memoConf = (k == 0 && useMemo) ? (V.confidence + (size_t)d * n)[pidx] : 0.0f;
            if (memoConf != 0.0f) {
              r = make_float2((V.cost + (size_t)d * n)[pidx], memoConf);
              counts += (unsigned)(V.pairCount + (size_t)d * n)[pidx] + (1u << 24);
            } else {
              unsigned np = 0;
#ifdef DERP_COUNT_PP_FILL
              fillSlots += pp_fill_entry();
#endif
              r = compute_cost<false, true>(V, dl, own, px, cand, pairs, np, cull, pidx, nullptr, &tm);
              counts += np;
            }
            counts += 1u << 16;
            if (r.x < bestCost) {
              bestCost = r.x;
              bestDisp = cand;
            }
          }
        }
      }
      outDisp = bestDisp;
      outCost = bestCost;
    }
  }
}

__device__ __forceinline__ void ping_pong_candidates_compact(const LevelView& V, const uint8_t* __restrict__ changed, int dl, int& x,
                                                             int& y, const PatchWin* win, LdsPairs& pairs, int useMemo, float& outDisp,
                                                             float& outCost, unsigned& counts, unsigned& fillSlots, PhaseTimers& tm) {
  const int d = V.dst0 + dl;
  const int own = V.dst2src[d];
  const size_t n = (size_t)V.W * V.H;
  const int lane = (int)(threadIdx.x & 63);
  const float* disp = V.disparity + (size_t)d * n;
  const uint8_t* fov = V.fovMask + (size_t)d * n;
  const uint8_t* chg = changed + (size_t)d * n;
  unsigned cmask = 0;
  bool eval = false;
  const unsigned idx = (unsigned)y * (unsigned)V.W + (unsigned)x;
  if (x < V.W && y < V.H) {
    outDisp = disp[idx];
    const bool interior = x >= 1 && y >= 1 && x < V.W - 1 && y < V.H - 1;
    if (interior && fov[idx]) {
      if (!V.srcFg[(size_t)own * n + idx]) {
        outDisp = V.bgDisp[(size_t)d * n + idx];
      } else if (!(V.srcVar[(size_t)own * n + idx] < V.varNoiseFloor)) {
        eval = true;
        const float bg = V.hasFg ? (V.bgDisp + (size_t)d * n)[idx] : 0.f;
        for (int k = 0; k < 9; ++k) {
          const int xx = min(max(x + (int)((kCandPackX >> (3 * k)) & 7u) - 2, 0), V.W - 1);
          const int yy = min(max(y + (int)((kCandPackY >> (3 * k)) & 7u) - 2, 0), V.H - 1);
          const unsigned j = (unsigned)yy * (unsigned)V.W + (unsigned)xx;
          if (fov[j]) {
            const float cand = disp[j];
            if (cand >= bg && chg[j]) {
              const float memoConf = (k == 0 && useMemo) ? (V.confidence + (size_t)d * n)[idx] : 0.0f;
              if (memoConf != 0.0f) {
                const float c = (V.cost + (size_t)d * n)[idx];
                counts += (unsigned)(V.pairCount + (size_t)d * n)[idx] + (1u << 24) + (1u << 16);
                if (c < outCost) {
                  outCost = c;
                  outDisp = cand;
                }
              } else {
                cmask |= 1u << k;
              }
            }
          }
        }
      }
    }
  }
  if (__ballot(cmask != 0u) == 0ull) {
    return;
  }
  unsigned cull = 0;
  const unsigned behind = eval ? V.behind[(size_t)d * n + idx] : ~0u;
  for (int t = 0; t < V.S - 1; ++t) {
    if (__ballot(!((behind >> t) & 1u)) == 0ull) {
      cull |= 1u << t;
    }
  }
  cull = __builtin_amdgcn_readfirstlane(cull);
  int incl = __popc(cmask);
  for (int off = 1; off < 64; off <<= 1) {
    const int v = __builtin_amdgcn_ds_bpermute((lane - off) << 2, incl);
    if (lane >= off) {
      incl += v;
    }
  }
  const int total = __builtin_amdgcn_readlane(incl, 63);
  const unsigned list = cmask | ((unsigned)incl << 16);
  const int x0 = __builtin_amdgcn_readfirstlane(x - (lane & 7)), y0 = __builtin_amdgcn_readfirstlane(y - (lane >> 3));
  extern __shared__ SsdPair ldsPairs[];
  SsdPair* const wavePairs = ldsPairs + (__builtin_amdgcn_readfirstlane(threadIdx.x) & ~63u);
  SsdPair* const stage = wavePairs + (size_t)(V.S - 1) * pairs.stride;
  for (int base = 0; base < total; base += 64) {
    int ln = lane;
    asm("" : "+v"(ln) : "s"(base));
    const int t = base + ln;
    int o = 0;
    for (int step = 32; step > 0; step >>= 1) {
      if ((int)((unsigned)__builtin_amdgcn_ds_bpermute((o + step - 1) << 2, (int)list) >> 16) <= t) {
        o += step;
      }
    }
    o = min(o, 63);
    const unsigned ol = (unsigned)__builtin_amdgcn_ds_bpermute(o << 2, (int)list);
    unsigned m = ol & 0xffffu;
    const int oStart = (int)(ol >> 16) - __popc(m);
#ifdef DERP_COUNT_PP_FILL
    fillSlots += ln == 0 ? 64u : 0u;
#endif
    if (t < total) {
      for (int r = t - oStart; r > 0; --r) {
        m &= m - 1;
      }
      const int k = __builtin_ctz(m);
      const int ox = x0 + (o & 7), oy = y0 + (o >> 3);
      const unsigned pidx = (unsigned)oy * (unsigned)V.W + (unsigned)ox;
      const int xx = min(max(ox + (int)((kCandPackX >> (3 * k)) & 7u) - 2, 0), V.W - 1);
      const int yy = min(max(oy + (int)((kCandPackY >> (3 * k)) & 7u) - 2, 0), V.H - 1);
      const float cand = disp[(unsigned)yy * (unsigned)V.W + (unsigned)xx];
      PixCtx px;
      load_pixctx<false>(V, d, own, ox, oy, win, px, o);
      LdsPairs lp{wavePairs + ln, pairs.stride, pairs.atanLut};
      unsigned np = 0;
      const float2 r = compute_cost<false, true>(V, dl, own, px, cand, lp, np, cull, pidx, nullptr, &tm);
      counts += np + (1u << 16);
      int sl = lane;
      asm("" : "+v"(sl) : "v"(r.x));
      stage[sl] = SsdPair{r.x, cand};
    }
    __builtin_amdgcn_fence(__ATOMIC_SEQ_CST, "wavefront");
    __builtin_amdgcn_wave_barrier();
    const int end = (int)(list >> 16);
    const int lo = max(end - __popc(list & 0xffffu), base), hi = min(end, base + 64);
    for (int i = lo; i < hi; ++i) {
      const SsdPair e = stage[i - base];
      if (e.first < outCost) {
        outCost = e.first;
        outDisp = e.second;
      }
    }
    __builtin_amdgcn_fence(__ATOMIC_SEQ_CST, "wavefront");
    __builtin_amdgcn_wave_barrier();
  }
  x = x0 + (lane & 7);
  y = y0 + (lane >> 3);
}

template <bool COMPACT>
__device__ __forceinline__ void ping_pong_tile(const LevelView& V, const uint8_t* __restrict__ changed, float* __restrict__ dispRes,
                                               float* __restrict__ costRes, int dl, int x, int y, const PatchWin* win, LdsPairs& pairs,
                                               int useMemo) {
  const int d = V.dst0 + dl;
  unsigned counts = 0, fillSlots = 0;
  PhaseTimers tm;
  const unsigned tk0 = phase_clock();
  float outDisp = 0.f;
  float outCost = __builtin_inff();
  if constexpr (COMPACT) {
    ping_pong_candidates_compact(V, changed, dl, x, y, win, pairs, useMemo, outDisp, outCost, counts, fillSlots, tm);
  } else if (x < V.W && y < V.H) {
    ping_pong_candidates_loop(V, changed, dl, x, y, win, pairs, useMemo, outDisp, outCost, counts, fillSlots, tm);
  }
  if (x < V.W && y < V.H) {
    const size_t n = (size_t)V.W * V.H;
    const unsigned idx = (unsigned)y * (unsigned)V.W + (unsigned)x;
    (dispRes + (size_t)d * n)[idx] = outDisp;
    (costRes + (size_t)d * n)[idx] = outCost;
  }
#if DERP_PHASE_TIMERS
  if ((threadIdx.x & 63) == 0) {
    const unsigned body = phase_clock() - tk0;
    atomicAdd(&V.counters[0], (unsigned long long)(DERP_PHASE_TIMERS == 1 ? tm.proj : body));
    atomicAdd(&V.counters[1], (unsigned long long)(DERP_PHASE_TIMERS == 1 ? tm.ssd : body - tm.inside));
    atomicAdd(&V.counters[3], (unsigned long long)(DERP_PHASE_TIMERS == 1 ? tm.select : 0u));
  }
  return;
#endif
  unsigned nMemo = counts >> 24;
#ifdef DERP_COUNT_PP_FILL
  flush_counters(V, (counts >> 16) & 0xffu, fillSlots);
#else
  (void)fillSlots;
  flush_counters(V, (counts >> 16) & 0xffu, counts & 0xffffu);
#endif
  for (int off = 32; off > 0; off >>= 1) {
    nMemo += __shfl_down(nMemo, off);
  }
  if ((threadIdx.x & 63) == 0 && nMemo) {
    atomicAdd(&V.counters[3], (unsigned long long)nMemo);
  }
}

template <bool COMPACT, bool WALK>
__device__ __forceinline__ void ping_pong_body(const LevelView& V, const uint8_t* __restrict__ changed, float* __restrict__ dispRes,
                                               float* __restrict__ costRes, int tilesX, int useMemo, int bands, int perBlock) {
  const unsigned long long bt0 = block_trace_begin();
  const int steps = WALK ? perBlock : 1;
  const int dl = blockIdx.y;
  const int d = V.dst0 + dl;
  PatchWin* win;
  LdsPairs pairs = cost_block_prologue(win);
  bool lutReady = false;
  for (int step = 0; step < steps; ++step) {
    int x, y;
    tile_pixel(cost_block_tile(blockIdx.x, gridDim.x, V.xcdRotate ? d : 0, bands, steps, step), tilesX, x, y);
    cost_tile_prologue(V, d, x - (int)(threadIdx.x & 7), y - (int)((threadIdx.x & 63) >> 3), win, pairs, lutReady);
    ping_pong_tile<COMPACT>(V, changed, dispRes, costRes, dl, x, y, win, pairs, useMemo);
  }
  block_trace_end(V, bt0);
}

#define DERP_PING_PONG_KERNEL(NAME, WAVES, COMPACT, WALK)                                                                   \
  __global__ void __launch_bounds__(kCostBlock, WAVES)                                                                      \
      NAME(LevelView V, const uint8_t* __restrict__ changed, float* __restrict__ dispRes, float* __restrict__ costRes,     \
           int tilesX, int useMemo, int bands, int perBlock) {                                                              \
    ping_pong_body<COMPACT, WALK>(V, changed, dispRes, costRes, tilesX, useMemo, bands, perBlock);                          \
  }
DERP_PING_PONG_KERNEL(k_ping_pong, DERP_COST_MIN_WAVES, true, false)
DERP_PING_PONG_KERNEL(k_ping_pong_w3, 3, true, false)
DERP_PING_PONG_KERNEL(k_ping_pong_loop, DERP_COST_MIN_WAVES, false, false)
DERP_PING_PONG_KERNEL(k_ping_pong_loop_w3, 3, false, false)
DERP_PING_PONG_KERNEL(k_ping_pong_walk, DERP_COST_MIN_WAVES, true, true)
DERP_PING_PONG_KERNEL(k_ping_pong_walk_w3, 3, true, true)
DERP_PING_PONG_KERNEL(k_ping_pong_loop_walk, DERP_COST_MIN_WAVES, false, true)
DERP_PING_PONG_KERNEL(k_ping_pong_loop_walk_w3, 3, false, true)
#undef DERP_PING_PONG_KERNEL

__global__ void k_ping_pong_commit(float* __restrict__ disp, float* __restrict__ cost, const float* __restrict__ dispRes,
                                   const float* __restrict__ costRes, uint8_t* __restrict__ changed, size_t n) {
  size_t i = (size_t)blockIdx.x * blockDim.x + threadIdx.x;
  const size_t step = (size_t)gridDim.x * blockDim.x;
  for (; i < n; i += step) {
    const float a = disp[i], b = dispRes[i];
    changed[i] = (a != b);
    disp[i] = b;
    cost[i] = costRes[i];
  }
}

__device__ __forceinline__ float clamp_fetch(const float* img, int x, int y, int W, int H) {
  return img[(size_t)min(max(y, 0), H - 1) * W + min(max(x, 0), W - 1)];
}

__global__ void __launch_bounds__(256)
    k_mismatch(LevelView V, float* __restrict__ newDisp, uint8_t* __restrict__ mismatchMask) {
  extern __shared__ float ldsMis[];
  const int d = blockIdx.z;
  const int x = blockIdx.x * 16 + (threadIdx.x & 15), y = blockIdx.y * 16 + (threadIdx.x >> 4);
  if (x >= V.W || y >= V.H) {
    return;
  }
  const size_t n = (size_t)V.W * V.H, idx = (size_t)y * V.W + x;
  if (!V.fovMask[(size_t)d * n + idx]) {
    newDisp[(size_t)d * n + idx] = __builtin_nanf("");
    return;
  }
  float* mis = ldsMis + threadIdx.x;
  const int own = V.dst2src[d];
  const float curr = V.disparity[(size_t)d * n + idx];
  int nMatch = 0, nMis = 0;
  if (V.srcFg[(size_t)own * n + idx]) {
    const Cam& cd = V.camsDst[d];
    const D3 dir = rig_direction(cd, (x + 0.5) / (double)V.W, (y + 0.5) / (double)V.H, cd.principal[0], cd.principal[1],
                                 cd.focal[0], cd.focal[1]);
    const double depth = (double)(1.0f / curr);
    const D3 pWorld = {cd.pos[0] + dir.x * depth, cd.pos[1] + dir.y * depth, cd.pos[2] + dir.z * depth};
    const float dMin = (1.0f - 0.1f) * curr, dMax = (1.0f + 0.1f) * curr;
    for (int s = 0; s < V.S; ++s) {
      if (s == own) {
        continue;
      }
      const Cam& cs = V.camsSrc[s];
      D2 pn;
      if (!sees(cs, pWorld, cs.principal[0], cs.principal[1], cs.focal[0], cs.focal[1], 1.0, 1.0, pn)) {
        continue;
      }
      const float sx = (float)(pn.x * (double)V.W), sy = (float)(pn.y * (double)V.H);
      const float xf = roundf(sx), yf = roundf(sy);
      const int xi = (int)xf, yi = (int)yf;
      const float xw = sx - xf + 0.5f, yw = sy - yf + 0.5f;
      const float* img = V.disparity + (size_t)s * n;
      const float dSrc = bilerp_f(clamp_fetch(img, xi - 1, yi - 1, V.W, V.H), clamp_fetch(img, xi, yi - 1, V.W, V.H),
                                  clamp_fetch(img, xi - 1, yi, V.W, V.H), clamp_fetch(img, xi, yi, V.W, V.H),
                                  (1 - xw) * (1 - yw), xw * (1 - yw), (1 - xw) * yw, xw * yw);
      if (dMin <= dSrc && dSrc <= dMax) {
        ++nMatch;
      } else {
        mis[(nMis++) * 256] = dSrc;
      }
    }
  }
  bool mask = false;
  float dispNew = curr;
  if (nMatch + nMis != 0) {
    const float var = V.srcVar[(size_t)own * n + idx];
    if (!(nMatch >= 1 || V.varHighThresh < var || var < V.varNoiseFloor)) {
      mask = true;
      for (int i = 1; i < nMis; ++i) {
        const float v = mis[i * 256];
        int k = i;
        while (k > 0 && mis[(k - 1) * 256] > v) {
          mis[k * 256] = mis[(k - 1) * 256];
          --k;
        }
        mis[k * 256] = v;
      }
      int closer = 0;
      for (; closer < nMis; ++closer) {
        if (mis[closer * 256] >= curr) {
          break;
        }
      }
      const float m = mis[(closer / 2) * 256];
      dispNew = (m < curr) ? m : curr;
    }
  }
  mismatchMask[(size_t)d * n + idx] = mask;
  newDisp[(size_t)d * n + idx] = dispNew;
}

__global__ void k_layer_disparities(const float* __restrict__ fg, const float* __restrict__ bg, size_t n,
                                    uint8_t* __restrict__ out) {
  size_t i = (size_t)blockIdx.x * blockDim.x + threadIdx.x;
  const size_t step = (size_t)gridDim.x * blockDim.x;
  for (; i < n; i += step) {
    const float m = fg[i] > 0.0f ? 1.0f : 0.0f;
    const float layer = fg[i] * m + bg[i] * (1 - m);
    const int r = cv_round(layer * 255.0f);
    out[i] = (uint8_t)min(max(r, 0), 255);
  }
}

__global__ void __launch_bounds__(kCostBlock, DERP_COST_MIN_WAVES)
    k_cost_map(LevelView V, int d, const float* __restrict__ dispIn, float* __restrict__ costOut,
               float* __restrict__ confOut, int tilesX) {
  const int dl = d - V.dst0;
  int x, y;
  tile_pixel(blockIdx.x, tilesX, x, y);
  PatchWin* win;
  LdsPairs pairs = cost_wave_prologue(V, d, x - (int)(threadIdx.x & 7), y - (int)((threadIdx.x & 63) >> 3), win);
  unsigned nCost = 0, nPair = 0;
  if (x >= 1 && y >= 1 && x < V.W - 1 && y < V.H - 1) {
    const int own = V.dst2src[d];
    PixCtx px;
    load_pixctx(V, d, own, x, y, win, px);
    const float2 r = compute_cost(V, dl, own, px, dispIn[(size_t)y * V.W + x], pairs, nPair);
    ++nCost;
    costOut[(size_t)y * V.W + x] = r.x;
    confOut[(size_t)y * V.W + x] = r.y;
  }
  flush_counters(V, nCost, nPair);
}

__constant__ unsigned long long kExp2fTab[32] = {
    0x3ff0000000000000ull, 0x3fefd9b0d3158574ull, 0x3fefb5586cf9890full, 0x3fef9301d0125b51ull,
    0x3fef72b83c7d517bull, 0x3fef54873168b9aaull, 0x3fef387a6e756238ull, 0x3fef1e9df51fdee1ull,
    0x3fef06fe0a31b715ull, 0x3feef1a7373aa9cbull, 0x3feedea64c123422ull, 0x3feece086061892dull,
    0x3feebfdad5362a27ull, 0x3feeb42b569d4f82ull, 0x3feeab07dd485429ull, 0x3feea47eb03a5585ull,
    0x3feea09e667f3bcdull, 0x3fee9f75e8ec5f74ull, 0x3feea11473eb0187ull, 0x3feea589994cce13ull,
    0x3feeace5422aa0dbull, 0x3feeb737b0cdc5e5ull, 0x3feec49182a3f090ull, 0x3feed503b23e255dull,
    0x3feee89f995ad3adull, 0x3feeff76f2fb5e47ull, 0x3fef199bdd85529cull, 0x3fef3720dcef9069ull,
    0x3fef5818dcfba487ull, 0x3fef7c97337b9b5full, 0x3fefa4afa2a490daull, 0x3fefd0765b6e4540ull};

__device__ __forceinline__ float div_by_const(float y, double rcp) {
  return (float)((double)y * rcp);
}

__device__ __forceinline__ float div_int_by_const(int y, double rcp) {
  return (float)((double)y * rcp);
}

__device__ __forceinline__ float expf_glibc(float x, const unsigned long long* tab) {
  const double InvLn2N = 0x1.71547652b82fep+0 * 32;
  const double C0 = 0x1.c6af84b912394p-5 / 32 / 32 / 32, C1 = 0x1.ebfce50fac4f3p-3 / 32 / 32,
               C2 = 0x1.62e42ff0c52d6p-1 / 32;
  const double SHIFT = 0x1.8p+52;
  const unsigned abstop = (__float_as_uint(x) >> 20) & 0x7ff;
  if (abstop >= (0x42b00000u >> 20)) {
    if (__float_as_uint(x) == 0xff800000u) {
      return 0.0f;
    }
    if (abstop >= (0x7f800000u >> 20)) {
      return x + x;
    }
    if (x > 0x1.62e42ep6f) {
      return __builtin_inff();
    }
    if (x < -0x1.9fe368p6f) {
      return 0.0f;
    }
  }
  const double xd = (double)x;
  double kd = __builtin_fma(InvLn2N, xd, SHIFT);
  const unsigned long long ki = (unsigned long long)__double_as_longlong(kd);
  kd -= SHIFT;
  const double r = __builtin_fma(InvLn2N, xd, -kd);
  const unsigned long long t = tab[ki & 31] + (ki << 47);
  const double sc = __longlong_as_double((long long)t);
  const double z = __builtin_fma(C0, r, C1);
  const double r2 = r * r;
  double y = __builtin_fma(C2, r, 1.0);
  y = __builtin_fma(z, r2, y);
  y = y * sc;
  return (float)y;
}

template <bool GUIDE_U16>
__device__ __forceinline__ float4 bilateral_texel(const void* __restrict__ guideV, size_t j, float value) {
  if (GUIDE_U16) {
    const ushort4 g = reinterpret_cast<const ushort4*>(guideV)[j];
    const float factor = 1 / 65535.0f;
    return make_float4(g.x * factor, g.y * factor, g.z * factor, value);
  }
  const float* g = reinterpret_cast<const float*>(guideV) + j * 3;
  const float factor = 1 / 1.0f;
  return make_float4(g[0] * factor, g[1] * factor, g[2] * factor, value);
}

__device__ __forceinline__ void bilateral_tap(float4 centre, float4 t, float weight0, float weight1, float weight2,
                                              double rcpDenom, const unsigned long long* expTab, float& sumWeight,
                                              float& weightedAvg) {
  const float d0 = centre.x - t.x, d1 = centre.y - t.y, d2 = centre.z - t.z;
  const float colorDiffSq = weight0 * (d0 * d0) + weight1 * (d1 * d1) + weight2 * (d2 * d2);
  const float weight = expf_glibc(div_by_const(div_by_const(-colorDiffSq, 1.0 / 3.0), rcpDenom), expTab);
  sumWeight += weight;
  weightedAvg += weight * t.w;
}

template <bool GUIDE_U16>
__global__ void __launch_bounds__(256)
    k_joint_bilateral(const float* __restrict__ image, const void* __restrict__ guideV,
                      const uint8_t* __restrict__ mask, int W, int H, int radius, float sigma, float weight0,
                      float weight1, float weight2, float* __restrict__ out, size_t planeStride, size_t guideStride,
                      const int* __restrict__ guideIndex) {
  extern __shared__ float ldsTile[];
  __shared__ unsigned long long expTab[32];
  if (threadIdx.x < 32) {
    expTab[threadIdx.x] = kExp2fTab[threadIdx.x];
  }
  const int p = blockIdx.z;
  const int T = 16 + 2 * radius;
  const int P = (T + 15) & ~15;
  const int n = P * T;
  float4* tTex = reinterpret_cast<float4*>(ldsTile);
  uint8_t* tMask = reinterpret_cast<uint8_t*>(ldsTile + 4 * n);
  const float* img = image + (size_t)p * planeStride;
  const uint8_t* m = mask + (size_t)p * planeStride;
  const size_t gplane = (size_t)(guideIndex ? guideIndex[p] : p) * guideStride;
  const int x0 = blockIdx.x * 16 - radius, y0 = blockIdx.y * 16 - radius;
  for (int k = threadIdx.x; k < T * T; k += 256) {
    const int ty = k / T, tx = k - ty * T;
    const int i = ty * P + tx;
    const int sx = min(max(x0 + tx, 0), W - 1), sy = min(max(y0 + ty, 0), H - 1);
    const size_t j = (size_t)sy * W + sx;
    tMask[i] = m[j];
    tTex[i] = bilateral_texel<GUIDE_U16>(guideV, gplane + j, img[j]);
  }
  __syncthreads();
  const int lx = threadIdx.x & 15, ly = threadIdx.x >> 4;
  const int x = blockIdx.x * 16 + lx, y = blockIdx.y * 16 + ly;
  if (x >= W || y >= H) {
    return;
  }
  const int c = (ly + radius) * P + lx + radius;
  const float4 centre = tTex[c];
  float result = centre.w;
  if (tMask[c]) {
    const float denom = 2.0f * (sigma * sigma);
    const double rcpDenom = 1.0 / (double)denom;
    float sumWeight = 0.f, weightedAvg = 0.f;
    for (int v = -radius; v <= radius; ++v) {
      const int row = c + v * P;
      for (int u = -radius; u <= radius; ++u) {
        const int j = row + u;
        if (!tMask[j]) {
          continue;
        }
        bilateral_tap(centre, tTex[j], weight0, weight1, weight2, rcpDenom, expTab, sumWeight, weightedAvg);
      }
    }
    if (sumWeight != 0.0f) {
      result = weightedAvg / sumWeight;
    }
  }
  out[(size_t)p * planeStride + (size_t)y * W + x] = result;
}

template <bool GUIDE_U16>
__global__ void __launch_bounds__(256)
    k_joint_bilateral_direct(const float* __restrict__ image, const void* __restrict__ guideV,
                             const uint8_t* __restrict__ mask, int W, int H, int radius, float sigma, float weight0,
                             float weight1, float weight2, float* __restrict__ out) {
  __shared__ unsigned long long expTab[32];
  if (threadIdx.x < 32) {
    expTab[threadIdx.x] = kExp2fTab[threadIdx.x];
  }
  __syncthreads();
  const int x = blockIdx.x * 16 + (threadIdx.x & 15), y = blockIdx.y * 16 + (threadIdx.x >> 4);
  if (x >= W || y >= H) {
    return;
  }
  const size_t idx = (size_t)y * W + x;
  float result = image[idx];
  if (mask[idx]) {
    const float4 centre = bilateral_texel<GUIDE_U16>(guideV, idx, result);
    const float denom = 2.0f * (sigma * sigma);
    const double rcpDenom = 1.0 / (double)denom;
    float sumWeight = 0.f, weightedAvg = 0.f;
    for (int v = -radius; v <= radius; ++v) {
      const size_t row = (size_t)min(max(y + v, 0), H - 1) * W;
      for (int u = -radius; u <= radius; ++u) {
        const size_t j = row + min(max(x + u, 0), W - 1);
        if (!mask[j]) {
          continue;
        }
        bilateral_tap(centre, bilateral_texel<GUIDE_U16>(guideV, j, image[j]), weight0, weight1, weight2, rcpDenom,
                      expTab, sumWeight, weightedAvg);
      }
    }
    if (sumWeight != 0.0f) {
      result = weightedAvg / sumWeight;
    }
  }
  out[idx] = result;
}

__device__ __forceinline__ void cswap(float& a, float& b) {
  const float lo = fminf(a, b), hi = fmaxf(a, b);
  a = lo;
  b = hi;
}

__global__ void k_masked_median(const float* __restrict__ image, const float* __restrict__ background,
                                const uint8_t* __restrict__ mask, int W, int H, int radius, float* __restrict__ out,
                                size_t planeStride, const uint8_t* __restrict__ fovForNan) {
  const int p = blockIdx.z;
  const int x = blockIdx.x * blockDim.x + threadIdx.x, y = blockIdx.y * blockDim.y + threadIdx.y;
  if (x >= W || y >= H) {
    return;
  }
  const size_t idx = (size_t)y * W + x;
  const float* img = image + (size_t)p * planeStride;
  const uint8_t* m = mask + (size_t)p * planeStride;
  float result = 0.0f;
  if (!m[idx]) {
    if (background) {
      result = background[(size_t)p * planeStride + idx];
    }
  } else if (radius == 1) {
    const float inf = __builtin_inff();
    float v[9];
    int cnt = 0;
#pragma unroll
    for (int j = 0; j < 3; ++j) {
#pragma unroll
      for (int i = 0; i < 3; ++i) {
        const int yy = y + j - 1, xx = x + i - 1;
        float t = inf;
        if (yy >= 0 && yy < H && xx >= 0 && xx < W) {
          const size_t q = (size_t)yy * W + xx;
          const float val = img[q];
          if (m[q] && !isnan(val) && val != 0) {
            t = val;
            ++cnt;
          }
        }
        v[j * 3 + i] = t;
      }
    }
    cswap(v[0], v[1]); cswap(v[3], v[4]); cswap(v[6], v[7]);
    cswap(v[1], v[2]); cswap(v[4], v[5]); cswap(v[7], v[8]);
    cswap(v[0], v[1]); cswap(v[3], v[4]); cswap(v[6], v[7]);
    cswap(v[0], v[3]); cswap(v[3], v[6]); cswap(v[0], v[3]);
    cswap(v[1], v[4]); cswap(v[4], v[7]); cswap(v[1], v[4]);
    cswap(v[2], v[5]); cswap(v[5], v[8]); cswap(v[2], v[5]);
    cswap(v[1], v[3]); cswap(v[5], v[7]); cswap(v[2], v[6]);
    cswap(v[4], v[6]); cswap(v[2], v[4]); cswap(v[2], v[3]);
    cswap(v[5], v[6]);
    if (cnt > 0) {
      const int h = cnt / 2;
      float lo = v[0], hi = v[0];
#pragma unroll
      for (int k = 0; k < 9; ++k) {
        lo = (k == h - 1) ? v[k] : lo;
        hi = (k == h) ? v[k] : hi;
      }
      result = (cnt & 1) ? hi : (float)(((double)(lo + hi)) / 2.0);
    }
  } else {
    float vals[25];
    int cnt = 0;
    for (int yy = y - radius; yy <= y + radius; ++yy) {
      for (int xx = x - radius; xx <= x + radius; ++xx) {
        if (0 > yy || yy >= H || 0 > xx || xx >= W) {
          continue;
        }
        const size_t j = (size_t)yy * W + xx;
        if (!m[j]) {
          continue;
        }
        const float v = img[j];
        if (isnan(v) || v == 0) {
          continue;
        }
        int k = cnt++;
        while (k > 0 && vals[k - 1] > v) {
          vals[k] = vals[k - 1];
          --k;
        }
        vals[k] = v;
      }
    }
    if (cnt > 0) {
      const int h = cnt / 2;
      if (cnt % 2 == 1) {
        result = vals[h];
      } else {
        result = (float)(((double)(vals[h - 1] + vals[h])) / 2.0);
      }
    }
  }
  if (fovForNan && !fovForNan[(size_t)p * planeStride + idx]) {
    result = __builtin_nanf("");
  }
  out[(size_t)p * planeStride + idx] = result;
}

__global__ void k_mask_fov(float* __restrict__ disp, const uint8_t* __restrict__ fov, size_t n) {
  size_t i = (size_t)blockIdx.x * blockDim.x + threadIdx.x;
  const size_t step = (size_t)gridDim.x * blockDim.x;
  for (; i < n; i += step) {
    if (!fov[i]) {
      disp[i] = __builtin_nanf("");
    }
  }
}

__global__ void k_and_masks(const uint8_t* fov, const uint8_t* srcFg, const int* __restrict__ dst2src, int dst0,
                            size_t n, uint8_t* out) {
  const int d = dst0 + blockIdx.y;
  size_t i = (size_t)blockIdx.x * blockDim.x + threadIdx.x;
  const size_t step = (size_t)gridDim.x * blockDim.x;
  for (; i < n; i += step) {
    out[(size_t)d * n + i] = fov[(size_t)d * n + i] & srcFg[(size_t)dst2src[d] * n + i];
  }
}

__global__ void k_lanczos_h(const float* __restrict__ in, int SW, int SH, int DW, const int* __restrict__ xofs,
                            const float* __restrict__ alpha, float* __restrict__ tmp, size_t inStride,
                            size_t tmpStride) {
  const int p = blockIdx.z;
  const int dx = blockIdx.x * blockDim.x + threadIdx.x, y = blockIdx.y * blockDim.y + threadIdx.y;
  if (dx >= DW || y >= SH) {
    return;
  }
  const float* S = in + (size_t)p * inStride + (size_t)y * SW;
  const float* a = alpha + (size_t)dx * 8;
  const int sx = xofs[dx] - 3;
  float v = 0;
#pragma unroll
  for (int j = 0; j < 8; ++j) {
    const int sxj = min(max(sx + j, 0), SW - 1);
    float sv = S[sxj];
    if (sv != sv) {
      sv = 1e-4f;
    }
    v += sv * a[j];
  }
  tmp[(size_t)p * tmpStride + (size_t)y * DW + dx] = v;
}
__global__ void k_lanczos_v(const float* __restrict__ tmp, int SH, int DW, int DH, const int* __restrict__ yofs,
                            const float* __restrict__ beta, float* __restrict__ out, size_t tmpStride,
                            size_t outStride) {
  const int p = blockIdx.z;
  const int x = blockIdx.x * blockDim.x + threadIdx.x, dy = blockIdx.y * blockDim.y + threadIdx.y;
  if (x >= DW || dy >= DH) {
    return;
  }
  const float* T = tmp + (size_t)p * tmpStride;
  const float* b = beta + (size_t)dy * 8;
  const int sy = yofs[dy] - 3;
  float r[8];
#pragma unroll
  for (int k = 0; k < 8; ++k) {
    const int syk = min(max(sy + k, 0), SH - 1);
    r[k] = T[(size_t)syk * DW + x];
  }
  out[(size_t)p * outStride + (size_t)dy * DW + x] =
      r[0] * b[0] + r[1] * b[1] + r[2] * b[2] + r[3] * b[3] + r[4] * b[4] + r[5] * b[5] + r[6] * b[6] + r[7] * b[7];
}

__global__ void k_upsample_nearest_masked(const float* __restrict__ in, const uint8_t* __restrict__ mask, int SW,
                                          int SH, const uint8_t* __restrict__ maskUp, int DW, int DH,
                                          float* __restrict__ out) {
  const int x = blockIdx.x * blockDim.x + threadIdx.x, y = blockIdx.y * blockDim.y + threadIdx.y;
  if (x >= DW || y >= DH) {
    return;
  }
  {
    const size_t ps = (size_t)blockIdx.z * SW * SH, pd = (size_t)blockIdx.z * DW * DH;
    in += ps;
    mask += ps;
    maskUp += pd;
    out += pd;
  }
  const double ifx = (double)SW / DW, ify = (double)SH / DH;
  const int sx = min((int)floor(x * ifx), SW - 1), sy = min((int)floor(y * ify), SH - 1);
  float v = in[(size_t)sy * SW + sx];
  if (!mask[(size_t)sy * SW + sx] || !maskUp[(size_t)y * DW + x]) {
    v = __builtin_nanf("");
  }
  out[(size_t)y * DW + x] = v;
}
__global__ void k_spiral_fill(const float* __restrict__ dispUp, const float* __restrict__ bgUp,
                              const uint8_t* __restrict__ maskUp, int W, int H, const int2* __restrict__ spiral,
                              int nSpiral, float* __restrict__ out) {
// ... 891 lines not shown
```

### facebook360_dep_amd/derp.py

```python
import ctypes as C
import os

import numpy as np

_HERE = os.path.dirname(os.path.abspath(__file__))
LIB_PATH = os.environ.get("DERP_LIB") or os.path.join(_HERE, "libderp_hip.so")
CAM_TYPES = {"FTHETA": 0, "RECTILINEAR": 1, "EQUISOLID": 2, "ORTHOGRAPHIC": 3}

STAGES = ["fov_mask", "variance", "own_bias", "upsample", "proj_warp", "reproject", "proj_bias", "brute_force",
          "random_proposals", "ping_pong", "mismatches", "bilateral", "median", "mask_fov", "temporal"]


class SeqOptions(C.Structure):
    _fields_ = [
        ("time_radius", C.c_int32), ("sigma", C.c_float), ("weight_b", C.c_float), ("weight_g", C.c_float),
        ("weight_r", C.c_float), ("space_radius", C.c_int32), ("use_foreground_masks", C.c_int32),
        ("partition", C.c_int32), ("do_temporal_filter", C.c_int32), ("resident_frames", C.c_int32),
    ]


class SeqTransfer(C.Structure):
    _fields_ = [("frame", C.c_int32), ("from_rank", C.c_int32), ("to_rank", C.c_int32)]


class CameraDesc(C.Structure):
    _fields_ = [
        ("type", C.c_int32), ("has_principal", C.c_int32), ("has_distortion", C.c_int32), ("has_fov", C.c_int32),
        ("origin", C.c_double * 3), ("forward", C.c_double * 3), ("up", C.c_double * 3), ("right", C.c_double * 3),
        ("resolution", C.c_double * 2), ("focal", C.c_double * 2), ("principal", C.c_double * 2),
        ("distortion", C.c_double * 3), ("fov", C.c_double), ("id", C.c_char * 64),
    ]


class Options(C.Structure):
    _fields_ = [
        ("min_depth_m", C.c_float), ("max_depth_m", C.c_float), ("var_noise_floor", C.c_float),
        ("var_high_thresh", C.c_float), ("random_proposals", C.c_int32), ("ping_pong_iterations", C.c_int32),
        ("mismatches_start_level", C.c_int32), ("do_bilateral_filter", C.c_int32), ("do_median_filter", C.c_int32),
        ("use_foreground_masks", C.c_int32), ("partial_coverage", C.c_int32), ("rebuild_warp_tables", C.c_int32),
    ]


class MeshPass(C.Structure):
    _fields_ = [("faces", C.c_longlong), ("feasible", C.c_longlong), ("winners", C.c_longlong), ("applied", C.c_longlong),
                ("deleted", C.c_longlong), ("threshold", C.c_double)]


class RenderParams(C.Structure):
    _fields_ = [
        ("kind", C.c_int32), ("width", C.c_int32), ("height", C.c_int32), ("position", C.c_double * 3),
        ("forward", C.c_double * 3), ("up", C.c_double * 3), ("horizontal_fov", C.c_double), ("ipd", C.c_float),
        ("alpha_blend", C.c_int32), ("disparity_color", C.c_int32), ("weight", C.c_int32), ("zero_nans", C.c_int32),
    ]


RENDER_KINDS = {"cube": 0, "equirect": 1, "snapshot": 2}
WEIGHTS = {"svd": 0, "minor": 1}
FORMATS = ["cubecolor", "cubedisp", "eqrcolor", "eqrdisp", "lr180", "snapcolor", "snapdisp", "tb3dof", "tbstereo"]


def render_params(kind="equirect", width=3072, height=None, position=(0, 0, 0), forward=(-1, 0, 0), up=(0, 0, 1),
                  horizontal_fov=90.0, ipd=0.0, alpha_blend=True, disparity_color=False, weight="svd", zero_nans=False):
    p = RenderParams()
    lib().derp_render_params_default(C.byref(p))
    p.kind = RENDER_KINDS[kind]
    p.width = width
    p.height = width // 2 if height is None else height
    for k, v in (("position", position), ("forward", forward), ("up", up)):
        for i in range(3):
            getattr(p, k)[i] = float(v[i])
    p.horizontal_fov = horizontal_fov
    p.ipd = ipd
    p.alpha_blend = int(bool(alpha_blend))
    p.disparity_color = int(bool(disparity_color))
    p.weight = WEIGHTS[weight]
    p.zero_nans = int(bool(zero_nans))
    return p


def render_format_size(fmt, width, height):
    w, h = C.c_int(), C.c_int()
    if lib().derp_render_format_size(fmt.encode(), width, height, C.byref(w), C.byref(h)):
        raise ValueError("Invalid format: %s" % fmt)
    return w.value, h.value


EXPORTS = [
    "derp_options_default", "derp_create", "derp_destroy", "derp_last_error", "derp_set_options", "derp_set_pyramid",
    "derp_build_pyramid_color", "derp_build_pyramid_foreground_mask", "derp_build_pyramid_background_disparity",
    "derp_download_level_color", "derp_download_level_mask", "derp_download_level_background", "derp_resize_area",
    "derp_generate_foreground_mask", "derp_image_info", "derp_image_decode", "derp_image_last_error", "derp_jpeg_encode",
    "derp_upload_color", "derp_upload_foreground_mask", "derp_upload_background_disparity", "derp_upload_disparity",
    "derp_process_level", "derp_process_pyramid", "derp_synchronize", "derp_download_disparity", "derp_download_cost",
    "derp_level_begin", "derp_stage_reproject_colors", "derp_stage_brute_force", "derp_stage_random_proposals",
    "derp_stage_ping_pong", "derp_stage_mismatches", "derp_stage_bilateral_filter", "derp_stage_median_filter", "derp_stage_mask_fov",
    "derp_level_end", "derp_set_level_disparity", "derp_get_level_disparity", "derp_cost_map", "derp_debug_download",
    "derp_debug_atan2_ypos", "derp_debug_fp64", "derp_debug_sees", "derp_debug_block_trace",
    "derp_ssim", "derp_average_score", "derp_rephotograph", "derp_rephotograph_upload", "derp_rephotograph_render", "derp_canopy_cubemap",
    "derp_render_params_default", "derp_render_upload", "derp_render", "derp_render_format_size", "derp_render_format",
    "derp_render_vertices",
    "derp_export_points", "derp_points_begin", "derp_points_splat", "derp_points_download", "derp_project_equirect_mask",
    "derp_mesh_build", "derp_mesh_counts", "derp_mesh_setup", "derp_mesh_simplify", "derp_mesh_download_f64", "derp_mesh_download",
    "derp_mesh_simplify_parallel", "derp_mesh_parallel_pass",
    "derp_mesh_setup_host", "derp_mesh_simplify_host",
    "derp_fov_mask", "derp_layer_disparities", "derp_download_mismatch_mask", "derp_upsample_disparity", "derp_joint_bilateral_u16", "derp_joint_bilateral_f32", "derp_masked_median",
    "derp_temporal_filter", "derp_temporal_filter_dev", "derp_dev_disparity", "derp_dev_color", "derp_dev_mask",
    "derp_get_counters", "derp_reset_counters", "derp_profile_enable", "derp_profile_reset", "derp_profile_query", "derp_profile_memoised",
    "derp_device_name", "derp_device_memory", "derp_host_nth_element_pairs", "derp_host_minstd_uniform", "derp_host_cost_tile_map",
    "derp_set_frame_slots", "derp_select_frame", "derp_frame_slots", "derp_host_alloc", "derp_host_free", "derp_bind_thread", "derp_host_register", "derp_host_unregister",
    "derp_seq_options_default", "derp_seq_window", "derp_seq_owner", "derp_seq_plan", "derp_seq_create", "derp_seq_destroy",
    "derp_seq_counts", "derp_seq_frames", "derp_seq_frame_slot", "derp_seq_buffer", "derp_rccl_unique_id",
    "derp_seq_attach_rccl", "derp_seq_attach_loopback", "derp_seq_attach_external", "derp_seq_selftest",
    "derp_seq_exchange_inputs", "derp_seq_level_compute", "derp_seq_level_exchange", "derp_seq_level_filter",
    "derp_seq_host_inputs", "derp_seq_buffer_copy", "derp_seq_upload_color_plane", "derp_seq_upload_disparity", "derp_seq_download_disparity", "derp_seq_exchange_inputs_level",
    "derp_seq_level_compute_frame", "derp_seq_level_provided_frame", "derp_seq_mark_exchanged", "derp_seq_level_filter_frame", "derp_seq_download_filtered",
    "derp_seq_run", "derp_seq_stats", "derp_seq_stats_reset", "derp_seq_exchange_exposed_ms",
    "derp_isp_config_default", "derp_isp_create", "derp_isp_destroy", "derp_isp_output_size", "derp_isp_process",
    "derp_isp_stage", "derp_isp_tables",
    "derp_sim_scene_create", "derp_sim_scene_destroy", "derp_sim_scene_icosahedrons", "derp_sim_scene_cubes",
    "derp_sim_scene_ground_plane", "derp_sim_scene_add_triangle", "derp_sim_bvh_build", "derp_sim_scene_counts",
    "derp_sim_scene_get", "derp_sim_perlin_table", "derp_sim_icosahedron", "derp_sim_noise", "derp_sim_trace_host", "derp_sim_create",
    "derp_sim_destroy", "derp_sim_upload", "derp_sim_render_camera", "derp_sim_render_equirect", "derp_sim_trace_rays",
    "derp_sim_stage_size", "derp_sim_stage",
]

_lib = None


def lib():
    global _lib
    if _lib is None:
        if not os.path.exists(LIB_PATH):
            raise RuntimeError(
                "libderp_hip.so is missing: build it with `python -c 'import __graft_entry__ as g; g.build()'` "
                "(hipcc --offload-arch=gfx950). There is no CPU fallback for the depth path."
            )
        try:
            import torch
        except ImportError:
            pass
        _lib = C.CDLL(LIB_PATH)
        _lib.derp_last_error.restype = C.c_char_p
        _lib.derp_last_error.argtypes = [C.c_void_p]
        _lib.derp_host_minstd_uniform.restype = C.c_float
        _lib.derp_host_minstd_uniform.argtypes = [C.c_int, C.c_uint64, C.c_float, C.c_float]
        _lib.derp_sim_scene_create.restype = C.c_void_p
        _lib.derp_sim_scene_destroy.argtypes = [C.c_void_p]
        _lib.derp_sim_scene_destroy.restype = None
    return _lib


def camera_desc(cam):
    j = CameraDesc()
    j.type = CAM_TYPES[cam["type"]]
    for k in ("origin", "forward", "up", "right", "resolution", "focal"):
        for i, v in enumerate(cam[k]):
            getattr(j, k)[i] = float(v)
    j.has_principal = int("principal" in cam)
    if "principal" in cam:
        j.principal[0], j.principal[1] = map(float, cam["principal"])
    j.has_distortion = int("distortion" in cam)
    if "distortion" in cam:
        d = list(cam["distortion"]) + [0.0] * (3 - len(cam["distortion"]))
        for i in range(3):
            j.distortion[i] = float(d[i])
    j.has_fov = int("fov" in cam)
    if "fov" in cam:
        j.fov = float(cam["fov"])
    j.id = cam["id"].encode()
    return j


def filter_destinations(cams, destinations):
    if not destinations:
        return list(cams)
    out = []
    for dest in destinations.split(","):
        for cam in cams:
            if cam["id"] == dest:
                out.append(cam)
# ... 137 lines not shown
        n, cur = C.c_int(), C.c_int()
        self._ck(lib().derp_frame_slots(self.h, C.byref(n), C.byref(cur)))
        return n.value, cur.value

    def upload_frame(self, frame):
        for level in range(len(self.sizes)):
            for s in range(self.S):
                self.upload_color(level, s, frame["color"][level][s])
                if frame.get("masks"):
                    self.upload_foreground_mask(level, s, frame["masks"][level][s])
            if frame.get("bg_disp"):
                for d in range(self.D):
                    self.upload_background_disparity(level, d, frame["bg_disp"][level][self._dst_src(d)])

    def _dst_src(self, d):
        ids = [c["id"] for c in self.cams_src]
        return ids.index(self.cams_dst[d]["id"])

    def process_level(self, level):
        self._ck(lib().derp_process_level(self.h, level))

    def process_pyramid(self, level_start=None, level_end=0):
        level_start = len(self.sizes) - 1 if level_start is None else level_start
        self._ck(lib().derp_process_pyramid(self.h, level_start, level_end))

    def synchronize(self):
        self._ck(lib().derp_synchronize(self.h))

    def download_disparity(self, level, d):
        out = np.zeros(self._shape(level), dtype=np.float32)
        self._ck(lib().derp_download_disparity(self.h, level, d, _p(out)))
        return out

    def download_cost(self, level, d):
        cost = np.zeros(self._shape(level), dtype=np.float32)
        conf = np.zeros(self._shape(level), dtype=np.float32)
        self._ck(lib().derp_download_cost(self.h, d, _p(cost), _p(conf)))
        return cost, conf

    def level_begin(self, level):
        self._cur = level
        self._ck(lib().derp_level_begin(self.h, level))

    def stage(self, name):
        fn = {
            "reproject_colors": "derp_stage_reproject_colors", "brute_force": "derp_stage_brute_force",
            "random_proposals": "derp_stage_random_proposals", "ping_pong": "derp_stage_ping_pong",
            "mismatches": "derp_stage_mismatches", "bilateral": "derp_stage_bilateral_filter", "median": "derp_stage_median_filter",
            "mask_fov": "derp_stage_mask_fov", "end": "derp_level_end",
        }[name]
        self._ck(getattr(lib(), fn)(self.h))

    def set_level_disparity(self, d, disp):
        disp = np.ascontiguousarray(disp, dtype=np.float32)
        self._ck(lib().derp_set_level_disparity(self.h, d, _p(disp)))

    def get_level_disparity(self, d):
        out = np.zeros(self._shape(self._cur), dtype=np.float32)
        self._ck(lib().derp_get_level_disparity(self.h, d, _p(out)))
        return out

    def cost_map(self, d, disp):
        disp = np.ascontiguousarray(disp, dtype=np.float32)
        cost = np.zeros(self._shape(self._cur), dtype=np.float32)
        conf = np.zeros(self._shape(self._cur), dtype=np.float32)
        self._ck(lib().derp_cost_map(self.h, d, _p(disp), _p(cost), _p(conf)))
        return cost, conf

    def debug_atan2_ypos(self, y, x):
        y = np.ascontiguousarray(y, np.float64)
        x = np.ascontiguousarray(x, np.float64)
        out = np.zeros_like(y)
        self._ck(lib().derp_debug_atan2_ypos(self.h, _p(y), _p(x), _p(out), C.c_size_t(y.size)))
        return out

    FP64_OPS = {"sqrt_lean": 0, "sqrt": 1, "div_plain": 2, "div": 3}

    def debug_fp64(self, op, a, b=None):
        a = np.ascontiguousarray(a, np.float64)
        b = None if b is None else np.ascontiguousarray(b, np.float64)
        assert b is None or b.shape == a.shape
        out = np.zeros_like(a)
        self._ck(lib().derp_debug_fp64(self.h, self.FP64_OPS[op], _p(a), _p(b), _p(out), C.c_size_t(a.size)))
        return out

    def debug_sees(self, src, xyz):
        xyz = np.ascontiguousarray(xyz, np.float64).reshape(-1, 3)
        out = np.zeros((len(xyz), 2, 3))
        self._ck(lib().derp_debug_sees(self.h, src, _p(xyz), C.c_size_t(len(xyz)), _p(out)))
        return out[:, :, 0].T != 0, np.ascontiguousarray(out[:, :, 1:].transpose(1, 0, 2))

    def debug(self, d, s, which):
        h, w = self._shape(self._cur)
        spec = {"warp": (0, (h, w, 2), np.float32), "color": (2, (h, w, 3), np.uint16),
                "bias": (3, (h, w, 3), np.uint16), "variance": (4, (h, w), np.float32),
                "fov": (5, (h, w), np.uint8)}[which]
        out = np.zeros(spec[1], dtype=spec[2])
        self._ck(lib().derp_debug_download(self.h, d, s, spec[0], _p(out)))
        return out

    def mismatch_mask(self, d):
        out = np.zeros(self._shape(self._cur), dtype=np.uint8)
        self._ck(lib().derp_download_mismatch_mask(self.h, d, _p(out)))
        return out

    def layer_disparities(self, fg, bg):
        fg = np.ascontiguousarray(fg, dtype=np.float32)
        bg = np.ascontiguousarray(bg, dtype=np.float32)
        out = np.zeros(fg.shape, dtype=np.uint8)
        self._ck(lib().derp_layer_disparities(self.h, _p(fg), _p(bg), C.c_size_t(fg.size), _p(out)))
        return out

    def ssim(self, x, y, blur_radius=1, alpha=1.0, beta=1.0, gamma=1.0):
        x = np.ascontiguousarray(x, dtype=np.float32)
        y = np.ascontiguousarray(y, dtype=np.float32)
        h, w = x.shape[:2]
        out = np.zeros((h, w, 3), dtype=np.float32)
        self._ck(lib().derp_ssim(self.h, _p(x), _p(y), w, h, blur_radius, C.c_float(alpha), C.c_float(beta),
                                 C.c_float(gamma), _p(out)))
        return out

    def rephotograph(self, target, colors, disps):
        colors = [np.ascontiguousarray(c, dtype=np.uint16) for c in colors]
        disps = [np.ascontiguousarray(d, dtype=np.float32) for d in disps]
        h, w = disps[0].shape
        cp = (C.c_void_p * len(colors))(*[c.ctypes.data for c in colors])
        dp = (C.c_void_p * len(disps))(*[d.ctypes.data for d in disps])
        out = np.zeros((h, w, 4), dtype=np.float32)
        self._ck(lib().derp_rephotograph(self.h, target, cp, dp, w, h, _p(out)))
        return out

    def rephotograph_upload(self, colors, disps):
        colors = [np.ascontiguousarray(c, dtype=np.uint16) for c in colors]
        disps = [np.ascontiguousarray(d, dtype=np.float32) for d in disps]
        h, w = disps[0].shape
        cp = (C.c_void_p * len(colors))(*[c.ctypes.data for c in colors])
        dp = (C.c_void_p * len(disps))(*[d.ctypes.data for d in disps])
        self._ck(lib().derp_rephotograph_upload(self.h, cp, dp, w, h))

    def canopy_cubemap(self, include, centre, edge):
        inc = np.ascontiguousarray(include, dtype=np.uint8)
        ctr = np.ascontiguousarray(centre, dtype=np.float64)
        out = np.zeros((6 * edge, edge, 4), dtype=np.float32)
        self._ck(lib().derp_canopy_cubemap(self.h, _p(inc), _p(ctr), edge, _p(out)))
        return out

    def render_upload(self, disps, colors=None):
        disps = [np.ascontiguousarray(d, dtype=np.float32) for d in disps]
        dp = (C.c_void_p * len(disps))(*[d.ctypes.data for d in disps])
        dw = (C.c_int * len(disps))(*[d.shape[1] for d in disps])
        dh = (C.c_int * len(disps))(*[d.shape[0] for d in disps])
        if colors is None:
            self._ck(lib().derp_render_upload(self.h, None, None, None, dp, dw, dh))
            return
        colors = [np.ascontiguousarray(c, dtype=np.float32) for c in colors]
        assert all(c.ndim == 3 and c.shape[2] == 4 for c in colors)
        cp = (C.c_void_p * len(colors))(*[c.ctypes.data for c in colors])
        cw = (C.c_int * len(colors))(*[c.shape[1] for c in colors])
        ch = (C.c_int * len(colors))(*[c.shape[0] for c in colors])
        self._ck(lib().derp_render_upload(self.h, cp, cw, ch, dp, dw, dh))

    def render(self, params, include=None):
        h = params.height
        w = {0: h, 1: 2 * h, 2: params.width}[params.kind]
        out = np.zeros((6 * h if params.kind == 0 else h, w, 4), dtype=np.float32)
        inc = None if include is None else np.ascontiguousarray(include, dtype=np.uint8)
# ... 551 lines not shown
```

### include/derp_hip.h

```cpp
#ifndef DERP_HIP_H
#define DERP_HIP_H

#include <stddef.h>
#include <stdint.h>

#ifdef __cplusplus
extern "C" {
#endif

typedef struct derp_ctx derp_ctx;

enum { DERP_FTHETA = 0, DERP_RECTILINEAR = 1, DERP_EQUISOLID = 2, DERP_ORTHOGRAPHIC = 3 };

typedef struct {
  int32_t type;
  int32_t has_principal;
  int32_t has_distortion;
  int32_t has_fov;
  double origin[3];
  double forward[3];
  double up[3];
  double right[3];
  double resolution[2];
  double focal[2];
// ... 6 lines not shown
typedef struct {
  float min_depth_m;
  float max_depth_m;
  float var_noise_floor;
  float var_high_thresh;
  int32_t random_proposals;
  int32_t ping_pong_iterations;
  int32_t mismatches_start_level;
  int32_t do_bilateral_filter;
  int32_t do_median_filter;
  int32_t use_foreground_masks;
  int32_t partial_coverage;
  int32_t rebuild_warp_tables;
} derp_options;

void derp_options_default(derp_options* o);

int derp_create(derp_ctx** out, int device, const derp_camera_desc* src, int n_src,
                const derp_camera_desc* dst, int n_dst);
void derp_destroy(derp_ctx* ctx);
const char* derp_last_error(const derp_ctx* ctx);
int derp_set_options(derp_ctx* ctx, const derp_options* o);

int derp_set_pyramid(derp_ctx* ctx, int num_levels, const int* widths, const int* heights,
                     int width_full, int height_full);

int derp_set_frame_slots(derp_ctx* ctx, int n_slots);
int derp_select_frame(derp_ctx* ctx, int slot);
int derp_frame_slots(const derp_ctx* ctx, int* n_slots, int* selected);

void* derp_host_alloc(size_t bytes);
void derp_host_free(void* p);
int derp_bind_thread(derp_ctx* ctx);
int derp_host_register(void* p, size_t bytes);
void derp_host_unregister(void* p);

int derp_upload_color(derp_ctx* ctx, int level, int src, const uint16_t* bgr);
int derp_upload_foreground_mask(derp_ctx* ctx, int level, int src, const uint8_t* mask);
int derp_upload_background_disparity(derp_ctx* ctx, int level, int dst, const float* disp);
int derp_upload_disparity(derp_ctx* ctx, int level, int dst, const float* disp);

int derp_build_pyramid_color(derp_ctx* ctx, int src, const uint16_t* bgr, int w, int h);
int derp_build_pyramid_foreground_mask(derp_ctx* ctx, int src, const uint8_t* mask, int w, int h,
                                       int threshold);
int derp_build_pyramid_background_disparity(derp_ctx* ctx, int dst, const float* disp, int w, int h);
int derp_download_level_color(derp_ctx* ctx, int level, int src, uint16_t* bgr);
int derp_download_level_mask(derp_ctx* ctx, int level, int src, uint8_t* mask01);
int derp_download_level_background(derp_ctx* ctx, int level, int dst, float* disp);
int derp_image_info(const void* bytes, size_t n, int* w, int* h, int* channels, int* bitdepth);
int derp_image_decode(const void* bytes, size_t n, void* out, size_t out_bytes);
const char* derp_image_last_error(void);
int derp_jpeg_encode(const void* pixels, int w, int h, int channels, int quality, void* out, size_t cap, size_t* size);

int derp_resize_area(derp_ctx* ctx, int kind, const void* src, int w, int h, void* dst, int dw, int dh);

int derp_generate_foreground_mask(derp_ctx* ctx, const uint16_t* template_bgr, const uint16_t* frame_bgr,
                                  int w, int h, int blur_radius, float threshold,
                                  int morph_closing_size, uint8_t* mask01);

int derp_process_level(derp_ctx* ctx, int level);
int derp_process_pyramid(derp_ctx* ctx, int level_start, int level_end);
int derp_synchronize(derp_ctx* ctx);

int derp_download_disparity(derp_ctx* ctx, int level, int dst, float* disparity);
int derp_download_cost(derp_ctx* ctx, int dst, float* cost, float* confidence);

int derp_level_begin(derp_ctx* ctx, int level);
int derp_stage_reproject_colors(derp_ctx* ctx);
int derp_stage_brute_force(derp_ctx* ctx);
int derp_stage_random_proposals(derp_ctx* ctx);
int derp_stage_ping_pong(derp_ctx* ctx);
int derp_stage_mismatches(derp_ctx* ctx);
int derp_stage_bilateral_filter(derp_ctx* ctx);
int derp_stage_median_filter(derp_ctx* ctx);
int derp_stage_mask_fov(derp_ctx* ctx);
int derp_level_end(derp_ctx* ctx);
int derp_set_level_disparity(derp_ctx* ctx, int dst, const float* disp);
int derp_get_level_disparity(derp_ctx* ctx, int dst, float* disp);
int derp_cost_map(derp_ctx* ctx, int dst, const float* disp, float* cost, float* confidence);
int derp_debug_download(derp_ctx* ctx, int dst, int src, int which, void* out);
int derp_debug_atan2_ypos(derp_ctx* ctx, const double* y, const double* x, double* out, size_t n);
int derp_debug_fp64(derp_ctx* ctx, int op, const double* a, const double* b, double* out, size_t n);
int derp_debug_sees(derp_ctx* ctx, int src, const double* xyz, size_t n, double* out);

int derp_debug_block_trace(derp_ctx* ctx, const char* stage, int level, uint64_t* out, size_t capacity, int* grid_x, int* grid_y);

int derp_download_mismatch_mask(derp_ctx* ctx, int dst, uint8_t* out);

int derp_layer_disparities(derp_ctx* ctx, const float* foreground, const float* background, size_t n,
                           uint8_t* out);
int derp_ssim(derp_ctx* ctx, const float* x_bgr, const float* y_bgr, int w, int h, int blur_radius, float alpha,
              float beta, float gamma, float* score_bgr);
int derp_average_score(const float* score_bgr, const uint8_t* mask, int w, int h, double* avg_bgr3);
int derp_rephotograph(derp_ctx* ctx, int target, const uint16_t* const* colors, const float* const* disparities,
                      int w, int h, float* out_bgra);
int derp_rephotograph_upload(derp_ctx* ctx, const uint16_t* const* colors, const float* const* disparities, int w,
                             int h);
int derp_rephotograph_render(derp_ctx* ctx, int target, float* out_bgra);
int derp_canopy_cubemap(derp_ctx* ctx, const uint8_t* include, const double* centre, int edge, float* out_bgra);
enum { DERP_RENDER_CUBE = 0, DERP_RENDER_EQUIRECT = 1, DERP_RENDER_SNAPSHOT = 2 };
enum { DERP_WEIGHT_SVD = 0, DERP_WEIGHT_MINOR = 1 };
typedef struct {
  int32_t kind;
  int32_t width, height;
  double position[3];
  double forward[3], up[3];
  double horizontal_fov;
  float ipd;
  int32_t alpha_blend;
  int32_t disparity_color;
  int32_t weight;
  int32_t zero_nans;
} derp_render_params;
void derp_render_params_default(derp_render_params* p);
int derp_render_upload(derp_ctx* ctx, const float* const* colors_bgra, const int* color_w, const int* color_h,
                       const float* const* disparities, const int* disp_w, const int* disp_h);
int derp_render(derp_ctx* ctx, const derp_render_params* p, const uint8_t* include, float* out_bgra);
int derp_render_format_size(const char* format, int width, int height, int* out_w, int* out_h);
int derp_render_format(derp_ctx* ctx, const char* format, const derp_render_params* p, const float* background,
                       const float* background_equirect, int eq_w, int eq_h, float* out_bgra);
int derp_render_vertices(derp_ctx* ctx, int cam, float ipd, float* out_xyzw);
int derp_export_points(derp_ctx* ctx, int cam, const float* disparity, int w, int h, const float* color_bgr,
                       double max_depth, int clip, int subsample, float* out_xyzrgb, size_t cap, size_t* count);
int derp_points_begin(derp_ctx* ctx, const int* widths, const int* heights);
int derp_points_splat(derp_ctx* ctx, const double* xyz, size_t n, double min_depth, double max_depth);
int derp_points_download(derp_ctx* ctx, int cam, float* disparity);
int derp_project_equirect_mask(derp_ctx* ctx, int cam, const uint8_t* eqr, int eqr_w, int eqr_h, int w, int h,
                               double depth, uint8_t* out);
enum {
  DERP_MESH_EXIT_BUDGET = 0,
  DERP_MESH_EXIT_INFINITE_THRESHOLD = 1,
  DERP_MESH_EXIT_STUCK = 2,
  DERP_MESH_EXIT_NO_CANDIDATES = 3
};
typedef struct derp_mesh_pass {
  long long faces;
  long long feasible;
  long long winners;
  long long applied;
  long long deleted;
  double threshold;
} derp_mesh_pass;
int derp_mesh_build(derp_ctx* ctx, int cam, const float* disparity, int w, int h, const double* resolution,
                    double depth_scale, const uint8_t* mask, int mask_w, int mask_h, float tear_ratio);
int derp_mesh_counts(derp_ctx* ctx, size_t* vertices, size_t* faces, size_t* faces_unmasked);
int derp_mesh_setup(derp_ctx* ctx, int equi_error, double* face_planes, double* edge_costs, double* vertex_quadrics);
int derp_mesh_simplify(derp_ctx* ctx, int num_faces_out, float strictness, int remove_boundary_edges, int equi_error,
                       int host_setup, int* stats);
int derp_mesh_simplify_parallel(derp_ctx* ctx, int num_faces_out, float strictness, int remove_boundary_edges,
                                int equi_error, int* stats);
int derp_mesh_parallel_pass(derp_ctx* ctx, int pass, derp_mesh_pass* out);
int derp_mesh_download_f64(derp_ctx* ctx, double* vertices, int32_t* faces);
int derp_mesh_download(derp_ctx* ctx, int clamp_negative_z, float* vtx, uint32_t* idx);
int derp_mesh_setup_host(const double* vertices, size_t nv, const int32_t* faces, size_t nf, int equi_error,
                         double* face_planes, double* edge_costs, double* vertex_quadrics);
int derp_mesh_simplify_host(const double* vertices, size_t nv, const int32_t* faces, size_t nf, const double* face_planes,
                            const double* edge_costs, const double* vertex_quadrics, int num_faces_out, float strictness,
                            int remove_boundary_edges, int equi_error, double* out_vertices, int32_t* out_faces,
                            size_t* out_nv, size_t* out_nf, int* stats);
int derp_fov_mask(derp_ctx* ctx, int dst, int w, int h, uint8_t* out);
int derp_upsample_disparity(derp_ctx* ctx, int dst, const float* disp, int w, int h,
                            const float* bg_disp_up, const uint8_t* fg_mask,
                            const uint8_t* fg_mask_up, int w_up, int h_up,
                            int use_foreground_masks, float* out);
int derp_joint_bilateral_u16(derp_ctx* ctx, const float* image, const uint16_t* guide_bgr,
                             const uint8_t* mask, int w, int h, int radius, float sigma,
// ... 199 lines not shown
```

Baseline: 499.0 Mpix/s.

## Cache FOV masks, batch brute-force depths, ping-pong buffer swap, fast bilateral taps

Bundles several independent optimizations. The FOV mask is now cached across frames per level. Brute-force cost computation processes a run of depths per block so the pixel context is loaded once, with behind-source culling. Ping-pong double-buffers disparity, cost and changed flags, which removes the commit kernel and the memset. Bilateral and median filters swap buffers instead of copying, and write straight into the level output. The mismatch-mask memset is skipped when the mask is unused. A fast bilateral tap path skips per-tap mask checks and the exp range checks when the whole tile is masked-in. This adds complexity and correctness risk around buffer aliasing and the cached state.

```diff
diff --git a/facebook360_dep_amd/csrc/derp_capi.hip b/facebook360_dep_amd/csrc/derp_capi.hip
--- a/facebook360_dep_amd/csrc/derp_capi.hip
+++ b/facebook360_dep_amd/csrc/derp_capi.hip
@@ -109,7 +109,7 @@
   V.cost = c->w.cost.as<float>();
   V.confidence = c->w.confidence.as<float>();
   V.bgDisp = c->frame().bg[L].as<float>();
-  V.fovMask = c->w.fovMask.as<uint8_t>();
+  V.fovMask = c->fovMask.as<uint8_t>();
   V.pairCount = c->w.pairCount.as<uint8_t>();
   V.counters = counter_slot(c, stage, L);
 #if DERP_BLOCK_TRACE
@@ -369,10 +369,13 @@
   const size_t n = (size_t)W * H;
   {
     Span sp(c, ST_FOV, level);
-    hipLaunchKernelGGL(k_fov_mask, grid2d(W, H, c->D, kBlk2d), kBlk2d, 0, c->stream, c->camsDst.as<Cam>(), W, H,
-                       c->w.fovMask.as<uint8_t>());
-    KCHECK(c);
-    hipLaunchKernelGGL(k_and_masks, dim3(flat_grid(n), c->D), dim3(256), 0, c->stream, c->w.fovMask.as<uint8_t>(),
+    if (c->opt.rebuild_warp_tables || c->fovCachedLevel != level) {
+      hipLaunchKernelGGL(k_fov_mask, grid2d(W, H, c->D, kBlk2d), kBlk2d, 0, c->stream, c->camsDst.as<Cam>(), W, H,
+                         c->fovMask.as<uint8_t>());
+      KCHECK(c);
+      c->fovCachedLevel = level;
+    }
+    hipLaunchKernelGGL(k_and_masks, dim3(flat_grid(n), c->D), dim3(256), 0, c->stream, c->fovMask.as<uint8_t>(),
                        c->frame().fg[level].as<uint8_t>(), c->dst2src.as<int>(), 0, n, c->w.maskAnd.as<uint8_t>());
     KCHECK(c);
   }
@@ -476,8 +479,9 @@
   const int tilesX = std::max(1, (V.W - 2 + 7) / 8), tilesY = std::max(1, (V.H - 2 + 7) / 8);
   const int tiles = tilesX * tilesY;
   const size_t lds = kCostLdsPerSrc * (size_t)(c->S);
-  hipLaunchKernelGGL(k_brute_costs, dim3(tiles, kNumDepths, nd), dim3(kCostBlock), lds, c->stream, V,
-                     c->w.bruteCost.as<float>(), c->w.bruteConf.as<float>(), tilesX, tiles);
+  const int run = std::min(std::max(c->bruteRun, 1), kNumDepths);
+  hipLaunchKernelGGL(k_brute_costs, dim3(tiles, (kNumDepths + run - 1) / run, nd), dim3(kCostBlock), lds, c->stream, V,
+                     c->w.bruteCost.as<float>(), c->w.bruteConf.as<float>(), tilesX, tiles, run);
   KCHECK(c);
   hipLaunchKernelGGL(k_brute_select, grid2d(V.W, V.H, nd, kBlk2d), kBlk2d, 0, c->stream, V, c->w.bruteCost.as<float>(),
                      c->w.bruteConf.as<float>());
@@ -520,7 +524,6 @@
   Span sp(c, ST_PINGPONG, L);
   LevelView V = make_view(c, ST_PINGPONG, dst0, nd);
   const size_t n = (size_t)V.W * V.H;
-  HIPCHK(c, hipMemsetAsync(c->w.changed.as<uint8_t>() + (size_t)dst0 * n, 1, n * nd, c->stream));
   int tilesX;
   const int tiles = tiles_of(V.W, V.H, tilesX);
   const size_t lds = lds_for_waves(kCostLdsPerSrc * (size_t)(c->S), c->ppWaves, c->ldsPerCu, kCostLdsStatic);
@@ -530,18 +533,24 @@
                           ? (c->ppCompact ? (four ? k_ping_pong_walk : k_ping_pong_walk_w3) : (four ? k_ping_pong_loop_walk : k_ping_pong_loop_walk_w3))
                           : (c->ppCompact ? (four ? k_ping_pong : k_ping_pong_w3) : (four ? k_ping_pong_loop : k_ping_pong_loop_w3));
   TRY(block_trace_attach(c, V, 1, cg.blocks, nd));
-  for (int it = 1; it <= c->opt.ping_pong_iterations; ++it) {
-    hipLaunchKernelGGL(kernel, dim3(cg.blocks, nd), dim3(kCostBlock), lds,
-                       c->stream, V, c->w.changed.as<uint8_t>(), c->w.dispRes.as<float>(), c->w.costRes.as<float>(), tilesX,
+  float* dispBuf[2] = {c->w.disparity.as<float>(), c->w.dispRes.as<float>()};
+  float* costBuf[2] = {c->w.cost.as<float>(), c->w.costRes.as<float>()};
+  uint8_t* chgBuf[2] = {c->w.changed.as<uint8_t>(), c->w.changed.as<uint8_t>() + n * c->D};
+  const int iterations = c->opt.ping_pong_iterations;
+  for (int it = 1; it <= iterations; ++it) {
+    const int from = (it - 1) & 1, to = it & 1;
+    V.disparity = dispBuf[from];
+    V.cost = costBuf[from];
+    hipLaunchKernelGGL(kernel, dim3(cg.blocks, nd), dim3(kCostBlock), lds, c->stream, V,
+                       it == 1 ? (const uint8_t*)nullptr : chgBuf[from], chgBuf[to], dispBuf[to], costBuf[to], tilesX,
                        (int)(it == 1 && c->randomRanThisLevel && !c->noMemo), cg.bands, cg.perBlock);
     KCHECK(c);
-    hipLaunchKernelGGL(k_ping_pong_commit, dim3(flat_grid(n * nd)), dim3(256), 0, c->stream,
-                       c->w.disparity.as<float>() + (size_t)dst0 * n, c->w.cost.as<float>() + (size_t)dst0 * n,
-                       c->w.dispRes.as<float>() + (size_t)dst0 * n, c->w.costRes.as<float>() + (size_t)dst0 * n,
-                       c->w.changed.as<uint8_t>() + (size_t)dst0 * n, n * nd);
-    KCHECK(c);
   }
   if (dst0 + nd >= c->D) {
+    if (iterations > 0 && (iterations & 1)) {
+      std::swap(c->w.disparity, c->w.dispRes);
+      std::swap(c->w.cost, c->w.costRes);
+    }
     c->randomRanThisLevel = false;
   }
   return 0;
@@ -583,6 +592,20 @@
 }
 
 constexpr size_t kBilateralMaxLds = 64 * 1024 - 256;
+
+bool bilateral_fast_tap_ok(float sigma, float w0, float w1, float w2) {
+  const float denom = 2.0f * (sigma * sigma);
+  return w1 == 1.0f && w2 == 1.0f && w0 >= 0.0f && std::isfinite(w0) && denom > 0.0f && std::isfinite(denom);
+}
+
+void launch_joint_bilateral_u16_tiled(derp_ctx* c, dim3 grid, const float* image, const void* guide, const uint8_t* mask,
+                                      int W, int H, int radius, float sigma, float w0, float w1, float w2, float* out,
+                                      size_t planeStride, size_t guideStride, const int* guideIndex) {
+  const bool fast = bilateral_fast_tap_ok(sigma, w0, w1, w2) && bilateral_lds_bytes(radius) + 256 <= kBilateralMaxLds;
+  const auto kernel = fast ? k_joint_bilateral<true, true> : k_joint_bilateral<true, false>;
+  hipLaunchKernelGGL(kernel, grid, dim3(256), bilateral_lds_bytes(radius), c->stream, image, guide, mask, W, H, radius, sigma,
+                     w0, w1, w2, out, planeStride, guideStride, guideIndex);
+}
 
 int run_bilateral(derp_ctx* c) {
   const int L = c->cur;
@@ -591,16 +614,15 @@
   const int W = c->LW[L], H = c->LH[L];
   const size_t n = (size_t)W * H;
   const int radius = bilateral_radius(L);
-  hipLaunchKernelGGL(k_joint_bilateral<true>, dim3((W + 15) / 16, (H + 15) / 16, c->D), dim3(256),
-                     bilateral_lds_bytes(radius), c->stream, c->w.disparity.as<float>(),
-                     (const void*)c->frame().color[L].as<ushort4>(), c->w.maskAnd.as<uint8_t>(), W, H, radius, 0.005f, 0.5f,
-                     1.0f, 1.0f, c->w.tmpF.as<float>(), n, n, c->dst2src.as<int>());
-  KCHECK(c);
-  HIPCHK(c, hipMemcpyAsync(c->w.disparity.p, c->w.tmpF.p, n * c->D * sizeof(float), hipMemcpyDeviceToDevice, c->stream));
-  return 0;
-}
-
-int run_median(derp_ctx* c, bool fuseMaskFov) {
+  launch_joint_bilateral_u16_tiled(c, dim3((W + 15) / 16, (H + 15) / 16, c->D), c->w.disparity.as<float>(),
+                                   (const void*)c->frame().color[L].as<ushort4>(), c->w.maskAnd.as<uint8_t>(), W, H, radius,
+                                   0.005f, 0.5f, 1.0f, 1.0f, c->w.tmpF.as<float>(), n, n, c->dst2src.as<int>());
+  KCHECK(c);
+  std::swap(c->w.disparity, c->w.tmpF);
+  return 0;
+}
+
+int run_median(derp_ctx* c, bool fuseMaskFov, float* levelOut = nullptr) {
   const int L = c->cur;
   Span sp(c, ST_MEDIAN, L);
   c->randomRanThisLevel = false;
@@ -608,19 +630,21 @@
   const size_t n = (size_t)W * H;
   hipLaunchKernelGGL(k_masked_median, grid2d(W, H, c->D, kBlk2d), kBlk2d, 0, c->stream, c->w.disparity.as<float>(),
                      c->opt.use_foreground_masks ? c->frame().bg[L].as<float>() : (const float*)nullptr,
-                     c->w.maskAnd.as<uint8_t>(), W, H, 1, c->w.tmpF.as<float>(), n,
-                     fuseMaskFov ? c->w.fovMask.as<uint8_t>() : (const uint8_t*)nullptr);
-  KCHECK(c);
-  HIPCHK(c, hipMemcpyAsync(c->w.disparity.p, c->w.tmpF.p, n * c->D * sizeof(float), hipMemcpyDeviceToDevice, c->stream));
-  return 0;
-}
-
-int run_mask_fov(derp_ctx* c) {
+                     c->w.maskAnd.as<uint8_t>(), W, H, 1, levelOut ? levelOut : c->w.tmpF.as<float>(), n,
+                     fuseMaskFov ? c->fovMask.as<uint8_t>() : (const uint8_t*)nullptr);
+  KCHECK(c);
+  if (!levelOut) {
+    std::swap(c->w.disparity, c->w.tmpF);
+  }
+  return 0;
+}
+
+int run_mask_fov(derp_ctx* c, float* levelOut = nullptr) {
   const int L = c->cur;
   Span sp(c, ST_MASKFOV, L);
   const size_t n = npx(c, L) * c->D;
   hipLaunchKernelGGL(k_mask_fov, dim3(flat_grid(n)), dim3(256), 0, c->stream, c->w.disparity.as<float>(),
-                     c->w.fovMask.as<uint8_t>(), n);
+                     c->fovMask.as<uint8_t>(), levelOut ? levelOut : c->w.disparity.as<float>(), n);
   KCHECK(c);
   return 0;
 }
@@ -664,7 +688,10 @@
   }
   HIPCHK(c, hipMemsetAsync(c->w.cost.p, 0, n * c->D * sizeof(float), c->stream));
   HIPCHK(c, hipMemsetAsync(c->w.confidence.p, 0, n * c->D * sizeof(float), c->stream));
-  HIPCHK(c, hipMemsetAsync(c->w.mismatchMask.p, 0, n * c->D, c->stream));
+  c->w.mismatchMaskHeld = level <= c->opt.mismatches_start_level && level != c->numLevels - 1;
+  if (c->w.mismatchMaskHeld) {
+    HIPCHK(c, hipMemsetAsync(c->w.mismatchMask.p, 0, n * c->D, c->stream));
+  }
   if (level < c->numLevels - 1 && !c->frame().haveDisp[level + 1] && !buildAllTables) {
     return fail(c, "Missing disparity of level %d needed to start level %d", level + 1, level);
   }
@@ -773,12 +800,13 @@
   if (c->opt.do_bilateral_filter) {
     TRY(run_bilateral(c));
   }
+  float* levelOut = c->frame().disp[level].as<float>();
   if (c->opt.do_median_filter) {
-    TRY(run_median(c, true));
+    TRY(run_median(c, true, levelOut));
   } else {
-    TRY(run_mask_fov(c));
-  }
-  TRY(level_end(c));
+    TRY(run_mask_fov(c, levelOut));
+  }
+  c->frame().haveDisp[level] = 1;
   return 0;
 }
 
@@ -825,12 +853,11 @@
 int alloc_work_set(derp_ctx* c, WorkSet& w, size_t n) {
   ALLOC(c, w.srcVar, n * c->S * sizeof(float));
   ALLOC(c, w.ownBias, n * c->S * sizeof(ushort4));
-  ALLOC(c, w.fovMask, n * c->D);
   ALLOC(c, w.maskAnd, n * c->D);
   for (DevBuf* b : {&w.disparity, &w.cost, &w.confidence, &w.dispRes, &w.costRes, &w.tmpF, &w.rank}) {
     ALLOC(c, *b, n * c->D * sizeof(float));
   }
-  ALLOC(c, w.changed, n * c->D);
+  ALLOC(c, w.changed, 2 * n * c->D);
   ALLOC(c, w.mismatchMask, n * c->D);
   ALLOC(c, w.pairCount, n * c->D);
   return 0;
@@ -974,6 +1001,9 @@
     c->costTilesPerBlock = atoi(e);
   }
   c->noMemo = getenv("DERP_NO_MEMO") != nullptr;
+  if (const char* e = getenv("DERP_BRUTE_RUN")) {
+    c->bruteRun = atoi(e);
+  }
   if (const char* e = getenv("DERP_PP_COMPACT")) {
     c->ppCompact = atoi(e) != 0;
   }
@@ -1096,8 +1126,10 @@
     nmax = std::max(nmax, npx(c, l));
   }
   TRY(alloc_work_set(c, c->w, nmax));
+  ALLOC(c, c->fovMask, nmax * c->D);
   c->cur = -1;
   c->warpCachedLevel = -1;
+  c->fovCachedLevel = -1;
   HIPCHK(c, hipStreamSynchronize(c->stream));
   return 0;
 }
@@ -1434,6 +1466,10 @@
     return fail(c, "bad destination index / null output");
   }
   const size_t n = npx(c, c->cur);
+  if (!c->w.mismatchMaskHeld) {
+    memset(out, 0, n);
+    return 0;
+  }
   return download_sync(c, out, c->w.mismatchMask.as<uint8_t>() + (size_t)d * n, n);
 }
 
diff --git a/facebook360_dep_amd/csrc/derp_ctx.h b/facebook360_dep_amd/csrc/derp_ctx.h
--- a/facebook360_dep_amd/csrc/derp_ctx.h
+++ b/facebook360_dep_amd/csrc/derp_ctx.h
@@ -42,11 +42,12 @@
 };
 
 struct WorkSet {
-  DevBuf srcVar, ownBias, fovMask, maskAnd, disparity, cost, confidence, dispRes, costRes, changed, tmpF, rank, mismatchMask, pairCount;
+  DevBuf srcVar, ownBias, maskAnd, disparity, cost, confidence, dispRes, costRes, changed, tmpF, rank, mismatchMask, pairCount;
   DevBuf tileSeen;
   DevBuf projColor, projBias;
   DevBuf projColorT;
   DevBuf bruteCost, bruteConf, lanczosTmp, staging, stagingB;
+  bool mismatchMaskHeld = false;
   int colorTablesCleanLevel = -1;
 };
 
@@ -100,6 +101,8 @@
   DevBuf projWarp, projWarpInv;
   DevBuf rayDir, behind;
   int warpCachedLevel = -1;
+  DevBuf fovMask;
+  int fovCachedLevel = -1;
   bool randomRanThisLevel = false;
   bool tablesValid = false;
   std::map<std::pair<int, int>, LanczosTab> lanczos;
@@ -120,6 +123,7 @@
   DevBuf blockTrace[2][kMaxLevels];
   int blockTraceGrid[2][kMaxLevels][2] = {};
   bool noMemo = false;
+  int bruteRun = 10;
   bool ppCompact = true;
   int randomWaves = 0, ppWaves = 0;
   size_t ldsPerCu = 160 * 1024;
diff --git a/facebook360_dep_amd/csrc/derp_debug_api.h b/facebook360_dep_amd/csrc/derp_debug_api.h
--- a/facebook360_dep_amd/csrc/derp_debug_api.h
+++ b/facebook360_dep_amd/csrc/derp_debug_api.h
@@ -53,6 +53,23 @@
   return 0;
 }
 
+int derp_debug_expf(derp_ctx* c, int mode, const float* x, float* out, size_t n) {
+  if (!c || !x || !out || mode < 0 || mode > 1) {
+    return fail(c, "bad arguments");
+  }
+  if (n == 0) {
+    return 0;
+  }
+  ALLOC(c, c->w.staging, 2 * n * sizeof(float));
+  float* d = c->w.staging.as<float>();
+  HIPCHK(c, hipMemcpyAsync(d, x, n * sizeof(float), hipMemcpyHostToDevice, c->stream));
+  hipLaunchKernelGGL(k_debug_expf, dim3(flat_grid(n)), dim3(256), 0, c->stream, mode, d, d + n, n);
+  KCHECK(c);
+  HIPCHK(c, hipMemcpyAsync(out, d + n, n * sizeof(float), hipMemcpyDeviceToHost, c->stream));
+  HIPCHK(c, hipStreamSynchronize(c->stream));
+  return 0;
+}
+
 int derp_debug_sees(derp_ctx* c, int src, const double* xyz, size_t n, double* out) {
   if (!c || !xyz || !out || src < 0 || src >= c->S) {
     return fail(c, "bad arguments");
@@ -81,7 +98,7 @@
     return 0;
   }
   if (which == 5) {
-    HIPCHK(c, hipMemcpy(out, c->w.fovMask.as<uint8_t>() + (size_t)d * n, n, hipMemcpyDeviceToHost));
+    HIPCHK(c, hipMemcpy(out, c->fovMask.as<uint8_t>() + (size_t)d * n, n, hipMemcpyDeviceToHost));
     return 0;
   }
   if (d < 0 || d >= c->D || s < 0 || s >= c->S || s == c->dst2srcH[d]) {
diff --git a/facebook360_dep_amd/csrc/derp_filters_api.h b/facebook360_dep_amd/csrc/derp_filters_api.h
--- a/facebook360_dep_amd/csrc/derp_filters_api.h
+++ b/facebook360_dep_amd/csrc/derp_filters_api.h
@@ -122,8 +122,12 @@
   const size_t n = (size_t)w * h;
   const dim3 grid((w + 15) / 16, (h + 15) / 16, 1);
   if (bilateral_lds_bytes(radius) <= kBilateralMaxLds) {
-    hipLaunchKernelGGL(k_joint_bilateral<GUIDE_U16>, grid, dim3(256), bilateral_lds_bytes(radius), c->stream, image, guide,
-                       mask, w, h, radius, sigma, w0, w1, w2, out, n, n, (const int*)nullptr);
+    if (GUIDE_U16) {
+      launch_joint_bilateral_u16_tiled(c, grid, image, guide, mask, w, h, radius, sigma, w0, w1, w2, out, n, n, nullptr);
+    } else {
+      hipLaunchKernelGGL(k_joint_bilateral<false>, grid, dim3(256), bilateral_lds_bytes(radius), c->stream, image, guide,
+                         mask, w, h, radius, sigma, w0, w1, w2, out, n, n, (const int*)nullptr);
+    }
   } else {
     hipLaunchKernelGGL(k_joint_bilateral_direct<GUIDE_U16>, grid, dim3(256), 0, c->stream, image, guide, mask, w, h,
                        radius, sigma, w0, w1, w2, out);
diff --git a/facebook360_dep_amd/csrc/derp_kernels.h b/facebook360_dep_amd/csrc/derp_kernels.h
--- a/facebook360_dep_amd/csrc/derp_kernels.h
+++ b/facebook360_dep_amd/csrc/derp_kernels.h
@@ -1244,8 +1244,8 @@
 }
 
 __global__ void __launch_bounds__(kCostBlock, DERP_COST_MIN_WAVES)
-    k_brute_costs(LevelView V, float* __restrict__ costs, float* __restrict__ confs, int tilesX, int tilesPerDst) {
-  const int i = blockIdx.y;
+    k_brute_costs(LevelView V, float* __restrict__ costs, float* __restrict__ confs, int tilesX, int tilesPerDst, int run) {
+  const int i0 = blockIdx.y * run, i1 = min(i0 + run, kNumDepths);
   const int dl = blockIdx.z;
   const int d = V.dst0 + dl;
   const int iw = V.W - 2, ih = V.H - 2;
@@ -1259,19 +1259,37 @@
     const int own = V.dst2src[d];
     const size_t n = (size_t)V.W * V.H, idx = (size_t)y * V.W + x;
     const float minDisparity = 1.0f / V.maxDepthM, maxDisparity = 1.0f / V.minDepthM;
-    const float disparity = probe_disparity(i, minDisparity, maxDisparity);
     const bool fov = V.fovMask[(size_t)d * n + idx], fg = V.srcFg[(size_t)own * n + idx];
-    const bool closer = V.hasFg ? (V.bgDisp[(size_t)d * n + idx] < disparity) : true;
-    float2 r = make_float2(__builtin_nanf(""), __builtin_nanf(""));
-    if (fov && fg && closer) {
+    const float nan = __builtin_nanf("");
+    if (fov && fg) {
       PixCtx px;
-      load_pixctx(V, d, own, x, y, win, px);
-      r = compute_cost(V, dl, own, px, disparity, pairs, nPair);
-      ++nCost;
-    }
-    const size_t o = ((size_t)dl * kNumDepths + i) * n + idx;
-    costs[o] = r.x;
-    confs[o] = r.y;
+      load_pixctx<false>(V, d, own, x, y, win, px);
+      const unsigned cull = behind_sources(V, d, idx);
+      const unsigned xy = (unsigned)x | ((unsigned)y << 16);
+      for (int i = i0; i < i1; ++i) {
+        unsigned q = xy;
+        asm("" : "+v"(q) : "s"(i));
+        const unsigned pidx = (q >> 16) * (unsigned)V.W + (q & 0xffffu);
+        const float disparity = probe_disparity(i, minDisparity, maxDisparity);
+        const bool closer = V.hasFg ? ((V.bgDisp + (size_t)d * n)[pidx] < disparity) : true;
+        float2 r = make_float2(nan, nan);
+        if (closer) {
+          unsigned np = 0;
+          r = compute_cost<false, true>(V, dl, own, px, disparity, pairs, np, cull, pidx);
+          nPair += np;
+          ++nCost;
+        }
+        const size_t o = ((size_t)dl * kNumDepths + i) * n;
+        (costs + o)[pidx] = r.x;
+        (confs + o)[pidx] = r.y;
+      }
+    } else {
+      for (int i = i0; i < i1; ++i) {
+        const size_t o = ((size_t)dl * kNumDepths + i) * n + idx;
+        costs[o] = nan;
+        confs[o] = nan;
+      }
+    }
   }
   flush_counters(V, nCost, nPair);
 }
@@ -1532,7 +1550,8 @@
   const unsigned idx = (unsigned)y * (unsigned)V.W + (unsigned)x;
   const float* disp = V.disparity + (size_t)d * n;
   const uint8_t* fov = V.fovMask + (size_t)d * n;
-  const uint8_t* chg = changed + (size_t)d * n;
+  const bool allChanged = changed == nullptr;
+  const uint8_t* chg = allChanged ? nullptr : changed + (size_t)d * n;
   outDisp = disp[idx];
   const bool interior = x >= 1 && y >= 1 && x < V.W - 1 && y < V.H - 1;
   if (interior && fov[idx]) {
@@ -1556,7 +1575,7 @@
         if (fov[j]) {
           const float cand = disp[j];
           const float bg = V.hasFg ? (V.bgDisp + (size_t)d * n)[pidx] : 0.f;
-          if (cand >= bg && chg[j]) {
+          if (cand >= bg && (allChanged || chg[j])) {
             float2 r;
             const float memoConf = (k == 0 && useMemo) ? (V.confidence + (size_t)d * n)[pidx] : 0.0f;
             if (memoConf != 0.0f) {
@@ -1593,7 +1612,8 @@
   const int lane = (int)(threadIdx.x & 63);
   const float* disp = V.disparity + (size_t)d * n;
   const uint8_t* fov = V.fovMask + (size_t)d * n;
-  const uint8_t* chg = changed + (size_t)d * n;
+  const bool allChanged = changed == nullptr;
+  const uint8_t* chg = allChanged ? nullptr : changed + (size_t)d * n;
   unsigned cmask = 0;
   bool eval = false;
   const unsigned idx = (unsigned)y * (unsigned)V.W + (unsigned)x;
@@ -1612,7 +1632,7 @@
           const unsigned j = (unsigned)yy * (unsigned)V.W + (unsigned)xx;
           if (fov[j]) {
             const float cand = disp[j];
-            if (cand >= bg && chg[j]) {
+            if (cand >= bg && (allChanged || chg[j])) {
               const float memoConf = (k == 0 && useMemo) ? (V.confidence + (size_t)d * n)[idx] : 0.0f;
               if (memoConf != 0.0f) {
                 const float c = (V.cost + (size_t)d * n)[idx];
@@ -1710,9 +1730,9 @@
 }
 
 template <bool COMPACT>
-__device__ __forceinline__ void ping_pong_tile(const LevelView& V, const uint8_t* __restrict__ changed, float* __restrict__ dispRes,
-                                               float* __restrict__ costRes, int dl, int x, int y, const PatchWin* win, LdsPairs& pairs,
-                                               int useMemo) {
+__device__ __forceinline__ void ping_pong_tile(const LevelView& V, const uint8_t* __restrict__ changed, uint8_t* __restrict__ changedNext,
+                                               float* __restrict__ dispRes, float* __restrict__ costRes, int dl, int x, int y,
+                                               const PatchWin* win, LdsPairs& pairs, int useMemo) {
   const int d = V.dst0 + dl;
   unsigned counts = 0, fillSlots = 0;
   PhaseTimers tm;
@@ -1729,6 +1749,7 @@
     const unsigned idx = (unsigned)y * (unsigned)V.W + (unsigned)x;
     (dispRes + (size_t)d * n)[idx] = outDisp;
     (costRes + (size_t)d * n)[idx] = outCost;
+    (changedNext + (size_t)d * n)[idx] = (V.disparity + (size_t)d * n)[idx] != outDisp;
   }
 #if DERP_PHASE_TIMERS
   if ((threadIdx.x & 63) == 0) {
@@ -1755,8 +1776,9 @@
 }
 
 template <bool COMPACT, bool WALK>
-__device__ __forceinline__ void ping_pong_body(const LevelView& V, const uint8_t* __restrict__ changed, float* __restrict__ dispRes,
-                                               float* __restrict__ costRes, int tilesX, int useMemo, int bands, int perBlock) {
+__device__ __forceinline__ void ping_pong_body(const LevelView& V, const uint8_t* __restrict__ changed, uint8_t* __restrict__ changedNext,
+                                               float* __restrict__ dispRes, float* __restrict__ costRes, int tilesX, int useMemo,
+                                               int bands, int perBlock) {
   const unsigned long long bt0 = block_trace_begin();
   const int steps = WALK ? perBlock : 1;
   const int dl = blockIdx.y;
@@ -1768,16 +1790,16 @@
     int x, y;
     tile_pixel(cost_block_tile(blockIdx.x, gridDim.x, V.xcdRotate ? d : 0, bands, steps, step), tilesX, x, y);
     cost_tile_prologue(V, d, x - (int)(threadIdx.x & 7), y - (int)((threadIdx.x & 63) >> 3), win, pairs, lutReady);
-    ping_pong_tile<COMPACT>(V, changed, dispRes, costRes, dl, x, y, win, pairs, useMemo);
+    ping_pong_tile<COMPACT>(V, changed, changedNext, dispRes, costRes, dl, x, y, win, pairs, useMemo);
   }
   block_trace_end(V, bt0);
 }
 
 #define DERP_PING_PONG_KERNEL(NAME, WAVES, COMPACT, WALK)                                                                   \
   __global__ void __launch_bounds__(kCostBlock, WAVES)                                                                      \
-      NAME(LevelView V, const uint8_t* __restrict__ changed, float* __restrict__ dispRes, float* __restrict__ costRes,     \
-           int tilesX, int useMemo, int bands, int perBlock) {                                                              \
-    ping_pong_body<COMPACT, WALK>(V, changed, dispRes, costRes, tilesX, useMemo, bands, perBlock);                          \
+      NAME(LevelView V, const uint8_t* __restrict__ changed, uint8_t* __restrict__ changedNext, float* __restrict__ dispRes, \
+           float* __restrict__ costRes, int tilesX, int useMemo, int bands, int perBlock) {                                 \
+    ping_pong_body<COMPACT, WALK>(V, changed, changedNext, dispRes, costRes, tilesX, useMemo, bands, perBlock);             \
   }
 DERP_PING_PONG_KERNEL(k_ping_pong, DERP_COST_MIN_WAVES, true, false)
 DERP_PING_PONG_KERNEL(k_ping_pong_w3, 3, true, false)
@@ -1788,18 +1810,6 @@
 DERP_PING_PONG_KERNEL(k_ping_pong_loop_walk, DERP_COST_MIN_WAVES, false, true)
 DERP_PING_PONG_KERNEL(k_ping_pong_loop_walk_w3, 3, false, true)
 #undef DERP_PING_PONG_KERNEL
-
-__global__ void k_ping_pong_commit(float* __restrict__ disp, float* __restrict__ cost, const float* __restrict__ dispRes,
-                                   const float* __restrict__ costRes, uint8_t* __restrict__ changed, size_t n) {
-  size_t i = (size_t)blockIdx.x * blockDim.x + threadIdx.x;
-  const size_t step = (size_t)gridDim.x * blockDim.x;
-  for (; i < n; i += step) {
-    const float a = disp[i], b = dispRes[i];
-    changed[i] = (a != b);
-    disp[i] = b;
-    cost[i] = costRes[i];
-  }
-}
 
 __device__ __forceinline__ float clamp_fetch(const float* img, int x, int y, int W, int H) {
   return img[(size_t)min(max(y, 0), H - 1) * W + min(max(x, 0), W - 1)];
@@ -1933,26 +1943,11 @@
   return (float)((double)y * rcp);
 }
 
-__device__ __forceinline__ float expf_glibc(float x, const unsigned long long* tab) {
+__device__ __forceinline__ float expf_glibc_poly(float x, const unsigned long long* tab) {
   const double InvLn2N = 0x1.71547652b82fep+0 * 32;
   const double C0 = 0x1.c6af84b912394p-5 / 32 / 32 / 32, C1 = 0x1.ebfce50fac4f3p-3 / 32 / 32,
                C2 = 0x1.62e42ff0c52d6p-1 / 32;
   const double SHIFT = 0x1.8p+52;
-  const unsigned abstop = (__float_as_uint(x) >> 20) & 0x7ff;
-  if (abstop >= (0x42b00000u >> 20)) {
-    if (__float_as_uint(x) == 0xff800000u) {
-      return 0.0f;
-    }
-    if (abstop >= (0x7f800000u >> 20)) {
-      return x + x;
-    }
-    if (x > 0x1.62e42ep6f) {
-      return __builtin_inff();
-    }
-    if (x < -0x1.9fe368p6f) {
-      return 0.0f;
-    }
-  }
   const double xd = (double)x;
   double kd = __builtin_fma(InvLn2N, xd, SHIFT);
   const unsigned long long ki = (unsigned long long)__double_as_longlong(kd);
@@ -1968,6 +1963,43 @@
   return (float)y;
 }
 
+__device__ __forceinline__ float expf_glibc(float x, const unsigned long long* tab) {
+  const unsigned abstop = (__float_as_uint(x) >> 20) & 0x7ff;
+  if (abstop >= (0x42b00000u >> 20)) {
+    if (__float_as_uint(x) == 0xff800000u) {
+      return 0.0f;
+    }
+    if (abstop >= (0x7f800000u >> 20)) {
+      return x + x;
+    }
+    if (x > 0x1.62e42ep6f) {
+      return __builtin_inff();
+    }
+    if (x < -0x1.9fe368p6f) {
+      return 0.0f;
+    }
+  }
+  return expf_glibc_poly(x, tab);
+}
+
+__device__ __forceinline__ float expf_glibc_nonpos(float x, const unsigned long long* tab) {
+  if (x < -0x1.9fe368p6f) {
+    return 0.0f;
+  }
+  return expf_glibc_poly(x, tab);
+}
+
+__global__ void __launch_bounds__(256) k_debug_expf(int mode, const float* __restrict__ x, float* __restrict__ out, size_t n) {
+  __shared__ unsigned long long expTab[32];
+  if (threadIdx.x < 32) {
+    expTab[threadIdx.x] = kExp2fTab[threadIdx.x];
+  }
+  __syncthreads();
+  for (size_t i = (size_t)blockIdx.x * blockDim.x + threadIdx.x; i < n; i += (size_t)gridDim.x * blockDim.x) {
+    out[i] = mode == 0 ? expf_glibc(x[i], expTab) : expf_glibc_nonpos(x[i], expTab);
+  }
+}
+
 template <bool GUIDE_U16>
 __device__ __forceinline__ float4 bilateral_texel(const void* __restrict__ guideV, size_t j, float value) {
   if (GUIDE_U16) {
@@ -1990,12 +2022,22 @@
   weightedAvg += weight * t.w;
 }
 
-template <bool GUIDE_U16>
+__device__ __forceinline__ void bilateral_tap_fast(float4 centre, float4 t, float weight0, double rcpDenom,
+                                                   const unsigned long long* expTab, float& sumWeight, float& weightedAvg) {
+  const float d0 = centre.x - t.x, d1 = centre.y - t.y, d2 = centre.z - t.z;
+  const float colorDiffSq = weight0 * (d0 * d0) + (d1 * d1) + (d2 * d2);
+  const float weight = expf_glibc_nonpos(div_by_const(div_by_const(-colorDiffSq, 1.0 / 3.0), rcpDenom), expTab);
+  sumWeight += weight;
+  weightedAvg += weight * t.w;
+}
+
+template <bool GUIDE_U16, bool FAST_TAP = false>
 __global__ void __launch_bounds__(256)
     k_joint_bilateral(const float* __restrict__ image, const void* __restrict__ guideV,
                       const uint8_t* __restrict__ mask, int W, int H, int radius, float sigma, float weight0,
                       float weight1, float weight2, float* __restrict__ out, size_t planeStride, size_t guideStride,
                       const int* __restrict__ guideIndex) {
+  static_assert(GUIDE_U16 || !FAST_TAP, "the fast tap's range argument needs the u16 guide");
   extern __shared__ float ldsTile[];
   __shared__ unsigned long long expTab[32];
   if (threadIdx.x < 32) {
@@ -2011,15 +2053,23 @@
   const uint8_t* m = mask + (size_t)p * planeStride;
   const size_t gplane = (size_t)(guideIndex ? guideIndex[p] : p) * guideStride;
   const int x0 = blockIdx.x * 16 - radius, y0 = blockIdx.y * 16 - radius;
+  int staged = 1;
   for (int k = threadIdx.x; k < T * T; k += 256) {
     const int ty = k / T, tx = k - ty * T;
     const int i = ty * P + tx;
     const int sx = min(max(x0 + tx, 0), W - 1), sy = min(max(y0 + ty, 0), H - 1);
     const size_t j = (size_t)sy * W + sx;
-    tMask[i] = m[j];
+    const uint8_t mk = m[j];
+    staged &= mk != 0;
+    tMask[i] = mk;
     tTex[i] = bilateral_texel<GUIDE_U16>(guideV, gplane + j, img[j]);
   }
-  __syncthreads();
+  bool fullMask = false;
+  if (FAST_TAP) {
+    fullMask = __syncthreads_and(staged) != 0;
+  } else {
+    __syncthreads();
+  }
   const int lx = threadIdx.x & 15, ly = threadIdx.x >> 4;
   const int x = blockIdx.x * 16 + lx, y = blockIdx.y * 16 + ly;
   if (x >= W || y >= H) {
@@ -2032,14 +2082,27 @@
     const float denom = 2.0f * (sigma * sigma);
     const double rcpDenom = 1.0 / (double)denom;
     float sumWeight = 0.f, weightedAvg = 0.f;
-    for (int v = -radius; v <= radius; ++v) {
-      const int row = c + v * P;
-      for (int u = -radius; u <= radius; ++u) {
-        const int j = row + u;
-        if (!tMask[j]) {
-          continue;
+    if (FAST_TAP && fullMask) {
+      for (int v = -radius; v <= radius; ++v) {
+        const int row = c + v * P;
+        for (int u = -radius; u <= radius; ++u) {
+          bilateral_tap_fast(centre, tTex[row + u], weight0, rcpDenom, expTab, sumWeight, weightedAvg);
         }
-        bilateral_tap(centre, tTex[j], weight0, weight1, weight2, rcpDenom, expTab, sumWeight, weightedAvg);
+      }
+    } else {
+      for (int v = -radius; v <= radius; ++v) {
+        const int row = c + v * P;
+        for (int u = -radius; u <= radius; ++u) {
+          const int j = row + u;
+          if (!tMask[j]) {
+            continue;
+          }
+          if (FAST_TAP) {
+            bilateral_tap_fast(centre, tTex[j], weight0, rcpDenom, expTab, sumWeight, weightedAvg);
+          } else {
+            bilateral_tap(centre, tTex[j], weight0, weight1, weight2, rcpDenom, expTab, sumWeight, weightedAvg);
+          }
+        }
       }
     }
     if (sumWeight != 0.0f) {
@@ -2189,12 +2252,15 @@
   out[(size_t)p * planeStride + idx] = result;
 }
 
-__global__ void k_mask_fov(float* __restrict__ disp, const uint8_t* __restrict__ fov, size_t n) {
+__global__ void k_mask_fov(const float* disp, const uint8_t* __restrict__ fov, float* out, size_t n) {
   size_t i = (size_t)blockIdx.x * blockDim.x + threadIdx.x;
   const size_t step = (size_t)gridDim.x * blockDim.x;
+  const bool inPlace = out == disp;
   for (; i < n; i += step) {
     if (!fov[i]) {
-      disp[i] = __builtin_nanf("");
+      out[i] = __builtin_nanf("");
+    } else if (!inPlace) {
+      out[i] = disp[i];
     }
   }
 }
diff --git a/facebook360_dep_amd/derp.py b/facebook360_dep_amd/derp.py
--- a/facebook360_dep_amd/derp.py
+++ b/facebook360_dep_amd/derp.py
@@ -95,7 +95,7 @@
     "derp_level_begin", "derp_stage_reproject_colors", "derp_stage_brute_force", "derp_stage_random_proposals",
     "derp_stage_ping_pong", "derp_stage_mismatches", "derp_stage_bilateral_filter", "derp_stage_median_filter", "derp_stage_mask_fov",
     "derp_level_end", "derp_set_level_disparity", "derp_get_level_disparity", "derp_cost_map", "derp_debug_download",
-    "derp_debug_atan2_ypos", "derp_debug_fp64", "derp_debug_sees", "derp_debug_block_trace",
+    "derp_debug_atan2_ypos", "derp_debug_fp64", "derp_debug_sees", "derp_debug_expf", "derp_debug_block_trace",
     "derp_ssim", "derp_average_score", "derp_rephotograph", "derp_rephotograph_upload", "derp_rephotograph_render", "derp_canopy_cubemap",
     "derp_render_params_default", "derp_render_upload", "derp_render", "derp_render_format_size", "derp_render_format",
     "derp_render_vertices",
@@ -399,6 +399,12 @@
         assert b is None or b.shape == a.shape
         out = np.zeros_like(a)
         self._ck(lib().derp_debug_fp64(self.h, self.FP64_OPS[op], _p(a), _p(b), _p(out), C.c_size_t(a.size)))
+        return out
+
+    def debug_expf(self, x, nonpos=False):
+        x = np.ascontiguousarray(x, np.float32)
+        out = np.zeros_like(x)
+        self._ck(lib().derp_debug_expf(self.h, int(bool(nonpos)), _p(x), _p(out), C.c_size_t(x.size)))
         return out
 
     def debug_sees(self, src, xyz):
diff --git a/include/derp_hip.h b/include/derp_hip.h
--- a/include/derp_hip.h
+++ b/include/derp_hip.h
@@ -112,6 +112,7 @@
 int derp_debug_atan2_ypos(derp_ctx* ctx, const double* y, const double* x, double* out, size_t n);
 int derp_debug_fp64(derp_ctx* ctx, int op, const double* a, const double* b, double* out, size_t n);
 int derp_debug_sees(derp_ctx* ctx, int src, const double* xyz, size_t n, double* out);
+int derp_debug_expf(derp_ctx* ctx, int mode, const float* x, float* out, size_t n);
 
 int derp_debug_block_trace(derp_ctx* ctx, const char* stage, int level, uint64_t* out, size_t capacity, int* grid_x, int* grid_y);
 
```

Measured after the change: 517.5 Mpix/s (median of 6 runs). 1.04x the previous value.
